# lukors/kanter_core

Measured on AMD Instinct MI355X. Metric: node-Mpix/s on 4096x4096 f32x4, 32-node graph, higher is better.
Workload: dtype f32

## Files before the change

### bindings/rust/kanter_core_amd_sys.rs

```rust
#![allow(non_camel_case_types, dead_code)]
use std::os::raw::{c_char, c_void};

#[repr(C)] pub struct KcPlane { _private: [u8; 0] }
#[repr(C)] pub struct KcImage { _private: [u8; 0] }
#[repr(C)] pub struct KcNodeGraph { _private: [u8; 0] }
#[repr(C)] pub struct KcLiveGraph { _private: [u8; 0] }
#[repr(C)] pub struct KcTexPro { _private: [u8; 0] }
#[repr(C)] pub struct KcPartition { _private: [u8; 0] }
#[repr(C)] pub struct KcU8Pipe { _private: [u8; 0] }

#[repr(C)] #[derive(Clone, Copy, Debug, PartialEq, Eq)]
pub struct KcPlacement { pub node_id: u32, pub rank: i32, pub component: i32, pub kind: i32 }

#[repr(C)] #[derive(Clone, Copy, Debug, PartialEq, Eq)]
pub struct KcBandRows { pub node_id: u32, pub y0: i32, pub y1: i32, pub width: u32, pub height: u32 }

#[repr(C)] #[derive(Clone, Copy, Debug, PartialEq, Eq)]
pub struct KcBandRange { pub y0: i32, pub y1: i32 }

#[repr(C)] #[derive(Clone, Copy, Debug, PartialEq, Eq)]
pub struct KcTransfer { pub node_id: u32, pub slot_id: u32, pub src_rank: i32, pub dst_rank: i32, pub level: i32 }

#[repr(C)] #[derive(Clone, Copy, Debug)]
pub struct KcDeviceImage {
// ... 13 lines not shown
pub struct KcChannelStats {
    pub channels: u32,
    pub flags: u32,
    pub pixels: u64,
    pub min: [f32; 4],
    pub max: [f32; 4],
    pub nan_count: [u64; 4],
    pub histogram: [[u64; 256]; 4],
}
pub const KC_STATS_HISTOGRAM: u32 = 1;
pub const KC_STATS_SRGB: u32 = 2;

#[repr(C)] #[derive(Clone, Copy, Debug)]
pub struct KcBcImage {
    pub ptr: *mut c_void,
    pub width: u32,
    pub height: u32,
    pub format: i32,
    pub row_pitch_bytes: usize,
}
pub const KC_BC1: i32 = 1;
pub const KC_BC3: i32 = 3;
pub const KC_BC4: i32 = 4;
pub const KC_BC5: i32 = 5;
pub const KC_BC_SRGB: u32 = 1;

#[repr(C)] #[derive(Clone, Copy, Debug, PartialEq, Eq)]
pub struct KcSize { pub width: u32, pub height: u32 }

#[repr(C)] #[derive(Clone, Copy, Debug, PartialEq, Eq)]
pub struct KcEdge { pub output_id: u32, pub input_id: u32, pub output_slot: u32, pub input_slot: u32 }

#[repr(C)]
pub struct KcNodeDesc {
    pub node_id: u32,
    pub node_type: i32,
    pub mix_type: i32,
    pub value: f32,
    pub embed_id: u32,
    pub text: *const c_char,
    pub graph: *const KcNodeGraph,
    pub resize_policy: i32,
    pub policy_slot: u32,
    pub policy_size: KcSize,
    pub resize_filter: i32,
}

pub const KC_OK: i32 = 0;
pub const KC_ERR_CANCELED: i32 = 2;
pub const KC_ERR_NO_DEVICE: i32 = 101;

#[link(name = "kanter_core_amd")]
extern "C" {
    pub fn kc_init(device_ordinal: i32) -> i32;
    pub fn kc_shutdown() -> i32;
    pub fn kc_is_initialized() -> i32;
    pub fn kc_set_stream(hip_stream: *mut c_void) -> i32;
    pub fn kc_get_stream() -> *mut c_void;
    pub fn kc_sync() -> i32;
    pub fn kc_last_error() -> *const c_char;
    pub fn kc_status_string(status: i32) -> *const c_char;
    pub fn kc_set_fusion(enabled: i32) -> i32;
    pub fn kc_get_fusion() -> i32;
    pub fn kc_set_resize_mode(mode: i32) -> i32;
    pub fn kc_get_resize_mode() -> i32;
    pub fn kc_set_cache_policy(mode: i32) -> i32;
    pub fn kc_get_cache_policy() -> i32;
    pub fn kc_set_option(name: *const c_char, value: i32) -> i32;
    pub fn kc_get_option(name: *const c_char, value: *mut i32) -> i32;
    pub fn kc_resize_upsample_plan(in_n: u32, out_n: u32, filter: i32, eligible: *mut i32, info: *mut i32, rows: *mut f32, cap: usize) -> i32;
    pub fn kc_resize_down2_plan(in_n: u32, out_n: u32, filter: i32, info: *mut i32, left_count: *mut u32, w: *mut f32, wcap: usize, vrec: *mut u32, vcap: usize, hw: *mut f32, hcap: usize) -> i32;
    pub fn kc_stats(bytes_in_use: *mut u64, bytes_cached: *mut u64, kernel_launches: *mut u64) -> i32;
    pub fn kc_stats_algorithmic_bytes(bytes: *mut u64) -> i32;
    pub fn kc_stats_counter(name: *const c_char, value: *mut u64) -> i32;
    pub fn kc_pool_trim() -> i32;
    pub fn kc_set_specialize(mode: i32, after: i32) -> i32;
    pub fn kc_get_specialize() -> i32;
    pub fn kc_specialize_wait() -> i32;
    pub fn kc_specialize_stats(kernels_compiled: *mut u64, compiles_failed: *mut u64, specialized_launches: *mut u64, compiles_pending: *mut u64) -> i32;
    pub fn kc_specialize_compile_check(words: *const u32, n_ops: u32, n_in: u32, start_src: i32, flat: i32, source: *mut c_char, cap: usize) -> i32;
    pub fn kc_specialize_compile_check_mask(words: *const u32, n_ops: u32, n_in: u32, start_src: i32, flat: i32, nt_mask: u32, source: *mut c_char, cap: usize) -> i32;
    pub fn kc_set_chain_quads(quads: i32) -> i32;
    pub fn kc_get_chain_quads() -> i32;
    pub fn kc_specialize_compile_check_upsample(words: *const u32, n_ops: u32, n_in: u32, start_src: i32, taps: u32, wide: i32, source: *mut c_char, cap: usize) -> i32;
    pub fn kc_kernel_cache_set_dir(dir: *const c_char) -> i32;
    pub fn kc_kernel_cache_stats(files_accepted: *mut u64, files_refused: *mut u64, files_written: *mut u64, kernels_loaded: *mut u64) -> i32;
    pub fn kc_kernel_cache_precompile(words: *const u32, n_ops: u32, n_in: u32, start_src: i32, flat: i32, nt_mask: u32, up_taps: u32, up_wide: i32, dir: *const c_char) -> i32;
    pub fn kc_specialize_reset() -> i32;
    pub fn kc_plane_alloc(width: u32, height: u32, out: *mut *mut KcPlane) -> i32;
    pub fn kc_plane_const(width: u32, height: u32, value: f32, out: *mut *mut KcPlane) -> i32;
    pub fn kc_plane_wrap(device_ptr: *mut c_void, width: u32, height: u32, pitch_bytes: usize, out: *mut *mut KcPlane) -> i32;
    pub fn kc_plane_retain(p: *mut KcPlane) -> i32;
    pub fn kc_plane_release(p: *mut KcPlane) -> i32;
    pub fn kc_plane_size(p: *const KcPlane, width: *mut u32, height: *mut u32) -> i32;
    pub fn kc_plane_is_const(p: *const KcPlane, is_const: *mut i32, value: *mut f32) -> i32;
    pub fn kc_plane_materialize(p: *mut KcPlane) -> i32;
    pub fn kc_plane_device_ptr(p: *mut KcPlane, device_ptr: *mut *mut c_void, pitch_bytes: *mut usize) -> i32;
    pub fn kc_plane_upload_f32(p: *mut KcPlane, host: *const f32, host_pitch_bytes: usize) -> i32;
    pub fn kc_plane_download_f32(p: *mut KcPlane, host: *mut f32, host_pitch_bytes: usize) -> i32;
    pub fn kc_image_gray(p: *mut KcPlane, out: *mut *mut KcImage) -> i32;
    pub fn kc_image_rgba(planes: *const *mut KcPlane, out: *mut *mut KcImage) -> i32;
    pub fn kc_image_retain(img: *mut KcImage) -> i32;
    pub fn kc_image_release(img: *mut KcImage) -> i32;
    pub fn kc_image_is_rgba(img: *const KcImage, is_rgba: *mut i32) -> i32;
    pub fn kc_image_size(img: *const KcImage, size: *mut KcSize) -> i32;
    pub fn kc_image_plane(img: *const KcImage, channel: i32, out: *mut *mut KcPlane) -> i32;
    pub fn kc_image_from_value(size: KcSize, value: f32, rgba: i32, out: *mut *mut KcImage) -> i32;
    pub fn kc_image_as_type(img: *const KcImage, rgba: i32, out: *mut *mut KcImage) -> i32;
    pub fn kc_image_materialize(img: *mut KcImage) -> i32;
    pub fn kc_image_from_u8(host: *const u8, width: u32, height: u32, channels: i32, out: *mut *mut KcImage) -> i32;
    pub fn kc_image_to_u8(img: *mut KcImage, srgb: i32, host_rgba8: *mut u8) -> i32;
    pub fn kc_u8_pipe_create(width: u32, height: u32, channels: i32, depth: i32, out: *mut *mut KcU8Pipe) -> i32;
    pub fn kc_u8_pipe_free(pipe: *mut KcU8Pipe) -> i32;
    pub fn kc_u8_pipe_buffers(pipe: *mut KcU8Pipe, slot: i32, host_in: *mut *mut u8, host_out: *mut *const u8) -> i32;
    pub fn kc_u8_pipe_upload(pipe: *mut KcU8Pipe, slot: i32, out: *mut *mut KcImage) -> i32;
    pub fn kc_u8_pipe_download(pipe: *mut KcU8Pipe, slot: i32, img: *mut KcImage, srgb: i32) -> i32;
    pub fn kc_u8_pipe_wait_download(pipe: *mut KcU8Pipe, slot: i32) -> i32;
    pub fn kc_image_from_f32(host_planes: *const *const f32, n_planes: i32, width: u32, height: u32, out: *mut *mut KcImage) -> i32;
    pub fn kc_image_to_f32(img: *mut KcImage, host_planes: *const *mut f32, n_planes: i32) -> i32;
    pub fn kc_device_image_validate(d: *const KcDeviceImage, extent_bytes: *mut usize) -> i32;
    pub fn kc_image_from_device(src: *const KcDeviceImage, flags: u32, hip_stream: *mut c_void, out: *mut *mut KcImage) -> i32;
    pub fn kc_image_to_device(img: *mut KcImage, dst: *const KcDeviceImage, flags: u32, hip_stream: *mut c_void) -> i32;
    pub fn kc_image_channel_stats(img: *mut KcImage, flags: u32, out: *mut KcChannelStats) -> i32;
    pub fn kc_bc_image_validate(d: *const KcBcImage, extent_bytes: *mut usize) -> i32;
    pub fn kc_image_to_bc(img: *mut KcImage, format: i32, flags: u32, host: *mut u8, host_bytes: usize) -> i32;
    pub fn kc_image_to_bc_device(img: *mut KcImage, dst: *const KcBcImage, flags: u32, hip_stream: *mut c_void) -> i32;
    pub fn kc_mip_level_count(width: u32, height: u32, levels: *mut u32) -> i32;
    pub fn kc_image_build_mips(img: *mut KcImage, flags: u32, levels: *mut *mut KcImage, cap: u32, count: *mut u32) -> i32;
    pub fn kc_bc_mip_layout(width: u32, height: u32, format: i32, levels: *mut u32, offsets: *mut usize, cap: u32, total_bytes: *mut usize) -> i32;
    pub fn kc_image_to_bc_mips(img: *mut KcImage, format: i32, flags: u32, host: *mut u8, host_bytes: usize) -> i32;
    pub fn kc_image_to_bc_mips_device(img: *mut KcImage, format: i32, flags: u32, device_ptr: *mut c_void, bytes: usize, hip_stream: *mut c_void) -> i32;
    pub fn kc_dds_header(width: u32, height: u32, format: i32, flags: u32, levels: u32, out: *mut u8, bytes: *mut usize) -> i32;
    pub fn kc_image_write_dds(img: *mut KcImage, path: *const c_char, format: i32, flags: u32, with_mips: i32) -> i32;
    pub fn kc_image_read_png(path: *const c_char, out: *mut *mut KcImage) -> i32;
    pub fn kc_image_write_png(img: *mut KcImage, path: *const c_char) -> i32;
    pub fn kc_calculate_size(policy: i32, sizes: *const KcSize, n: i32, slot_index: i32, specific: KcSize, out: *mut KcSize) -> i32;
    pub fn kc_resize_image(src: *mut KcImage, size: KcSize, filter: i32, out: *mut *mut KcImage) -> i32;
    pub fn kc_resize_buffers(images: *const *mut KcImage, keys: *const KcEdge, n: i32, edges_sorted: *const KcEdge, n_edges: i32, policy: i32, policy_slot: u32, policy_size: KcSize, filter: i32, out: *mut *mut KcImage) -> i32;
    pub fn kc_mix_process(left: *mut KcImage, right: *mut KcImage, mix_type: i32, out: *mut *mut KcImage) -> i32;
    pub fn kc_separate_rgba_process(input: *mut KcImage, out: *mut *mut KcImage) -> i32;
    pub fn kc_combine_rgba_process(inputs: *const *mut KcImage, out: *mut *mut KcImage) -> i32;
    pub fn kc_value_process(value: f32, out: *mut *mut KcImage) -> i32;
    pub fn kc_height_to_normal_process(input: *mut KcImage, out: *mut *mut KcImage) -> i32;
    pub fn kc_node_graph_new(out: *mut *mut KcNodeGraph) -> i32;
    pub fn kc_node_graph_clone(g: *const KcNodeGraph, out: *mut *mut KcNodeGraph) -> i32;
    pub fn kc_node_graph_free(g: *mut KcNodeGraph) -> i32;
    pub fn kc_node_graph_from_path(path: *const c_char, out: *mut *mut KcNodeGraph) -> i32;
    pub fn kc_node_graph_from_json(json: *const c_char, out: *mut *mut KcNodeGraph) -> i32;
    pub fn kc_node_graph_export_json(g: *const KcNodeGraph, path: *const c_char) -> i32;
    pub fn kc_node_graph_to_json(g: *const KcNodeGraph, buf: *mut c_char, cap: usize, needed: *mut usize) -> i32;
    pub fn kc_node_graph_add_node(g: *mut KcNodeGraph, node: *const KcNodeDesc, node_id: *mut u32) -> i32;
    pub fn kc_node_graph_add_node_with_id(g: *mut KcNodeGraph, node: *const KcNodeDesc) -> i32;
    pub fn kc_node_graph_connect(g: *mut KcNodeGraph, output_node: u32, input_node: u32, output_slot: u32, input_slot: u32) -> i32;
    pub fn kc_node_graph_try_connect(g: *mut KcNodeGraph, output_node: u32, input_node: u32, output_slot: u32, input_slot: u32) -> i32;
    pub fn kc_node_graph_remove_node(g: *mut KcNodeGraph, node_id: u32) -> i32;
    pub fn kc_node_graph_remove_edge(g: *mut KcNodeGraph, edge: KcEdge) -> i32;
    pub fn kc_node_graph_disconnect_slot(g: *mut KcNodeGraph, node_id: u32, side: i32, slot_id: u32) -> i32;
    pub fn kc_node_graph_node_count(g: *const KcNodeGraph, count: *mut u32) -> i32;
    pub fn kc_node_graph_node_ids(g: *const KcNodeGraph, ids: *mut u32, cap: u32, count: *mut u32) -> i32;
    pub fn kc_node_graph_edges(g: *const KcNodeGraph, edges: *mut KcEdge, cap: u32, count: *mut u32) -> i32;
    pub fn kc_node_graph_input_slot_id_with_name(g: *const KcNodeGraph, name: *const c_char, slot_id: *mut u32) -> i32;
    pub fn kc_node_graph_output_slot_id_with_name(g: *const KcNodeGraph, name: *const c_char, slot_id: *mut u32) -> i32;
    pub fn kc_node_graph_set_mix_type(g: *mut KcNodeGraph, node_id: u32, mix_type: i32) -> i32;
    pub fn kc_node_graph_set_image_node_path(g: *mut KcNodeGraph, node_id: u32, path: *const c_char) -> i32;
    pub fn kc_node_graph_rename_output_node(g: *mut KcNodeGraph, node_id: u32, new_name: *const c_char, old_name: *mut c_char, cap: usize) -> i32;
    pub fn kc_tex_pro_new(memory_threshold: u64, out: *mut *mut KcTexPro) -> i32;
    pub fn kc_tex_pro_free(tp: *mut KcTexPro) -> i32;
    pub fn kc_tex_pro_new_live_graph(tp: *mut KcTexPro, out: *mut *mut KcLiveGraph) -> i32;
    pub fn kc_live_graph_free(lg: *mut KcLiveGraph) -> i32;
    pub fn kc_live_graph_set_flags(lg: *mut KcLiveGraph, auto_update: i32, use_cache: i32) -> i32;
// ... 56 lines not shown
```

### include/kanter_core_amd.h

```cpp
#ifndef KANTER_CORE_AMD_H
#define KANTER_CORE_AMD_H

#include <stddef.h>
#include <stdint.h>

#ifdef __cplusplus
extern "C" {
#endif

#define KC_API __attribute__((visibility("default")))

typedef enum kc_status {
    KC_OK = 0,
    KC_ERR_GENERIC = 1,
    KC_ERR_CANCELED = 2,
    KC_ERR_IMAGE = 3,
    KC_ERR_INVALID_BUFFER_COUNT = 4,
    KC_ERR_INVALID_NODE_ID = 5,
    KC_ERR_INVALID_NODE_TYPE = 6,
    KC_ERR_INVALID_SLOT_ID = 7,
    KC_ERR_INVALID_SLOT_TYPE = 8,
    KC_ERR_INVALID_EDGE = 9,
    KC_ERR_NO_SLOT_DATA = 10,
    KC_ERR_SLOT_OCCUPIED = 11,
// ... 3 lines not shown
    KC_ERR_POISON = 15,
    KC_ERR_TRY_LOCK = 16,
    KC_ERR_NODE_DIRTY = 17,
    KC_ERR_IO = 18,
    KC_ERR_INVALID_NAME = 19,
    KC_ERR_HIP = 100,
    KC_ERR_NO_DEVICE = 101,
    KC_ERR_INVALID_ARG = 102,
    KC_ERR_OUT_OF_MEMORY = 103,
    KC_ERR_UNSUPPORTED = 104
} kc_status;

typedef enum kc_mix_type { KC_MIX_ADD = 0, KC_MIX_SUBTRACT = 1, KC_MIX_MULTIPLY = 2, KC_MIX_DIVIDE = 3, KC_MIX_POW = 4 } kc_mix_type;
typedef enum kc_resize_filter { KC_FILTER_NEAREST = 0, KC_FILTER_TRIANGLE = 1, KC_FILTER_CATMULLROM = 2, KC_FILTER_GAUSSIAN = 3, KC_FILTER_LANCZOS3 = 4 } kc_resize_filter;
typedef enum kc_resize_policy { KC_POLICY_MOST_PIXELS = 0, KC_POLICY_LEAST_PIXELS = 1, KC_POLICY_LARGEST_AXES = 2, KC_POLICY_SMALLEST_AXES = 3, KC_POLICY_SPECIFIC_SLOT = 4, KC_POLICY_SPECIFIC_SIZE = 5 } kc_resize_policy;
typedef enum kc_node_type {
    KC_NODE_INPUT_GRAY = 0, KC_NODE_INPUT_RGBA = 1, KC_NODE_OUTPUT_GRAY = 2, KC_NODE_OUTPUT_RGBA = 3,
    KC_NODE_GRAPH = 4, KC_NODE_IMAGE = 5, KC_NODE_EMBED = 6, KC_NODE_WRITE = 7, KC_NODE_VALUE = 8,
    KC_NODE_MIX = 9, KC_NODE_HEIGHT_TO_NORMAL = 10, KC_NODE_SEPARATE_RGBA = 11, KC_NODE_COMBINE_RGBA = 12
} kc_node_type;
typedef enum kc_node_state { KC_STATE_CLEAN = 0, KC_STATE_DIRTY = 1, KC_STATE_REQUESTED = 2, KC_STATE_PRIORITISED = 3, KC_STATE_PROCESSING = 4, KC_STATE_PROCESSING_DIRTY = 5 } kc_node_state;
typedef enum kc_side { KC_SIDE_INPUT = 0, KC_SIDE_OUTPUT = 1 } kc_side;

typedef struct kc_plane kc_plane;
typedef struct kc_image kc_image;
typedef struct kc_node_graph kc_node_graph;
typedef struct kc_live_graph kc_live_graph;
typedef struct kc_tex_pro kc_tex_pro;
typedef struct kc_partition kc_partition;
typedef struct kc_u8_pipe kc_u8_pipe;

typedef struct kc_size { uint32_t width, height; } kc_size;
typedef struct kc_edge { uint32_t output_id, input_id, output_slot, input_slot; } kc_edge;

typedef struct kc_node_desc {
    uint32_t node_id;
    int32_t node_type;
    int32_t mix_type;
    float value;
    uint32_t embed_id;
    const char *text;
    const kc_node_graph *graph;
    int32_t resize_policy;
    uint32_t policy_slot;
    kc_size policy_size;
    int32_t resize_filter;
} kc_node_desc;

KC_API int kc_init(int device_ordinal);
KC_API int kc_shutdown(void);
KC_API int kc_is_initialized(void);
KC_API int kc_set_stream(void *hip_stream);
KC_API void *kc_get_stream(void);
KC_API int kc_sync(void);
KC_API const char *kc_last_error(void);
KC_API const char *kc_status_string(int status);
KC_API int kc_set_fusion(int enabled);
KC_API int kc_get_fusion(void);
KC_API int kc_set_resize_mode(int mode);
KC_API int kc_get_resize_mode(void);
KC_API int kc_set_cache_policy(int mode);
KC_API int kc_get_cache_policy(void);
KC_API int kc_set_option(const char *name, int value);
KC_API int kc_get_option(const char *name, int *value);
KC_API int kc_resize_upsample_plan(uint32_t in_n, uint32_t out_n, int filter, int *eligible, int32_t info[5], float *rows,
                                   size_t cap);
KC_API int kc_resize_down2_plan(uint32_t in_n, uint32_t out_n, int filter, int32_t info[5], uint32_t *left_count, float *w, size_t wcap,
                                uint32_t *vrec, size_t vcap, float *hw, size_t hcap);
KC_API int kc_stats(uint64_t *bytes_in_use, uint64_t *bytes_cached, uint64_t *kernel_launches);
KC_API int kc_stats_algorithmic_bytes(uint64_t *bytes);
KC_API int kc_stats_counter(const char *name, uint64_t *value);
KC_API int kc_pool_trim(void);
KC_API int kc_set_specialize(int mode, int after);
KC_API int kc_get_specialize(void);
KC_API int kc_specialize_wait(void);
KC_API int kc_specialize_stats(uint64_t *kernels_compiled, uint64_t *compiles_failed, uint64_t *specialized_launches,
                               uint64_t *compiles_pending);
KC_API int kc_specialize_compile_check(const uint32_t *words, uint32_t n_ops, uint32_t n_in, int start_src, int flat,
                                       char *source, size_t cap);
KC_API int kc_specialize_compile_check_mask(const uint32_t *words, uint32_t n_ops, uint32_t n_in, int start_src, int flat,
                                            uint32_t nt_mask, char *source, size_t cap);
KC_API int kc_set_chain_quads(int quads);
KC_API int kc_get_chain_quads(void);
KC_API int kc_specialize_compile_check_upsample(const uint32_t *words, uint32_t n_ops, uint32_t n_in, int start_src, uint32_t taps,
                                                int wide, char *source, size_t cap);
KC_API int kc_kernel_cache_set_dir(const char *dir);
KC_API int kc_kernel_cache_stats(uint64_t *files_accepted, uint64_t *files_refused, uint64_t *files_written, uint64_t *kernels_loaded);
KC_API int kc_kernel_cache_precompile(const uint32_t *words, uint32_t n_ops, uint32_t n_in, int start_src, int flat, uint32_t nt_mask,
                                      uint32_t up_taps, int up_wide, const char *dir);
KC_API int kc_specialize_reset(void);

KC_API int kc_plane_alloc(uint32_t width, uint32_t height, kc_plane **out);
KC_API int kc_plane_const(uint32_t width, uint32_t height, float value, kc_plane **out);
KC_API int kc_plane_wrap(void *device_ptr, uint32_t width, uint32_t height, size_t pitch_bytes, kc_plane **out);
KC_API int kc_plane_retain(kc_plane *p);
KC_API int kc_plane_release(kc_plane *p);
KC_API int kc_plane_size(const kc_plane *p, uint32_t *width, uint32_t *height);
KC_API int kc_plane_is_const(const kc_plane *p, int *is_const, float *value);
KC_API int kc_plane_materialize(kc_plane *p);
KC_API int kc_plane_device_ptr(kc_plane *p, void **device_ptr, size_t *pitch_bytes);
KC_API int kc_plane_upload_f32(kc_plane *p, const float *host, size_t host_pitch_bytes);
KC_API int kc_plane_download_f32(kc_plane *p, float *host, size_t host_pitch_bytes);

KC_API int kc_image_gray(kc_plane *p, kc_image **out);
KC_API int kc_image_rgba(kc_plane *const planes[4], kc_image **out);
KC_API int kc_image_retain(kc_image *img);
KC_API int kc_image_release(kc_image *img);
KC_API int kc_image_is_rgba(const kc_image *img, int *is_rgba);
KC_API int kc_image_size(const kc_image *img, kc_size *size);
KC_API int kc_image_plane(const kc_image *img, int channel, kc_plane **out);
KC_API int kc_image_from_value(kc_size size, float value, int rgba, kc_image **out);
KC_API int kc_image_as_type(const kc_image *img, int rgba, kc_image **out);
KC_API int kc_image_materialize(kc_image *img);
KC_API int kc_image_from_u8(const uint8_t *host, uint32_t width, uint32_t height, int channels, kc_image **out);
KC_API int kc_image_to_u8(kc_image *img, int srgb, uint8_t *host_rgba8);
KC_API int kc_u8_pipe_create(uint32_t width, uint32_t height, int channels, int depth, kc_u8_pipe **out);
KC_API int kc_u8_pipe_free(kc_u8_pipe *pipe);
KC_API int kc_u8_pipe_buffers(kc_u8_pipe *pipe, int slot, uint8_t **host_in, const uint8_t **host_out);
KC_API int kc_u8_pipe_upload(kc_u8_pipe *pipe, int slot, kc_image **out);
KC_API int kc_u8_pipe_download(kc_u8_pipe *pipe, int slot, kc_image *img, int srgb);
KC_API int kc_u8_pipe_wait_download(kc_u8_pipe *pipe, int slot);
KC_API int kc_image_from_f32(const float *const host_planes[], int n_planes, uint32_t width, uint32_t height, kc_image **out);
KC_API int kc_image_to_f32(kc_image *img, float *const host_planes[], int n_planes);
typedef enum kc_dtype { KC_DTYPE_U8 = 0, KC_DTYPE_U16 = 1, KC_DTYPE_F16 = 2, KC_DTYPE_BF16 = 3, KC_DTYPE_F32 = 4 } kc_dtype;
typedef enum kc_layout { KC_LAYOUT_INTERLEAVED = 0 , KC_LAYOUT_PLANAR = 1  } kc_layout;
typedef struct kc_device_image {
    void *ptr;
    uint32_t width, height;
    int32_t channels;
    int32_t dtype, layout;
    size_t row_pitch_bytes;
    size_t channel_pitch_bytes;
} kc_device_image;
#define KC_DEVICE_SRGB 1u
#define KC_DEVICE_GRAY 2u
KC_API int kc_device_image_validate(const kc_device_image *d, size_t *extent_bytes);
KC_API int kc_image_from_device(const kc_device_image *src, uint32_t flags, void *hip_stream, kc_image **out);
KC_API int kc_image_to_device(kc_image *img, const kc_device_image *dst, uint32_t flags, void *hip_stream);
#define KC_STATS_HISTOGRAM 1u
#define KC_STATS_SRGB 2u
typedef struct kc_channel_stats {
    uint32_t channels;
    uint32_t flags;
    uint64_t pixels;
    float min[4], max[4];
    uint64_t nan_count[4];
    uint64_t histogram[4][256];
} kc_channel_stats;
KC_API int kc_image_channel_stats(kc_image *img, uint32_t flags, kc_channel_stats *out);
typedef enum kc_bc_format { KC_BC1 = 1, KC_BC3 = 3, KC_BC4 = 4, KC_BC5 = 5 } kc_bc_format;
typedef struct kc_bc_image {
    void *ptr;
    uint32_t width, height;
    int32_t format;
    size_t row_pitch_bytes;
} kc_bc_image;
#define KC_BC_SRGB 1u
KC_API int kc_bc_image_validate(const kc_bc_image *d, size_t *extent_bytes);
KC_API int kc_image_to_bc(kc_image *img, int format, uint32_t flags, uint8_t *host, size_t host_bytes);
KC_API int kc_image_to_bc_device(kc_image *img, const kc_bc_image *dst, uint32_t flags, void *hip_stream);
#define KC_MIP_PER_LEVEL 2u
KC_API int kc_mip_level_count(uint32_t width, uint32_t height, uint32_t *levels);
KC_API int kc_image_build_mips(kc_image *img, uint32_t flags, kc_image **levels, uint32_t cap, uint32_t *count);
KC_API int kc_bc_mip_layout(uint32_t width, uint32_t height, int format, uint32_t *levels, size_t *offsets, uint32_t cap,
                            size_t *total_bytes);
KC_API int kc_image_to_bc_mips(kc_image *img, int format, uint32_t flags, uint8_t *host, size_t host_bytes);
KC_API int kc_image_to_bc_mips_device(kc_image *img, int format, uint32_t flags, void *device_ptr, size_t bytes, void *hip_stream);
KC_API int kc_dds_header(uint32_t width, uint32_t height, int format, uint32_t flags, uint32_t levels, uint8_t out[148], size_t *bytes);
KC_API int kc_image_write_dds(kc_image *img, const char *path, int format, uint32_t flags, int with_mips);
KC_API int kc_image_read_png(const char *path, kc_image **out);
KC_API int kc_image_write_png(kc_image *img, const char *path);

// ... 126 lines not shown
```

### kanter_core_amd/__init__.py

```python
from .api import (Edge, EmbeddedSlotDataId, LiveGraph, MixType, Node, NodeGraph, NodeId, NodeState, NodeType,
                  ResizeFilter, ResizePolicy, Side, Size, SlotData, SlotId, SlotImage, TexProError,
                  TextureProcessor, calculate_size, combine_rgba_process, get_stream, height_to_normal_process,
                  init, is_initialized, mix_process, resize_image, separate_rgba_process, set_fusion, set_stream,
                  shutdown, stats, sync, value_process, set_specialize, get_specialize, specialize_wait,
                  specialize_stats, specialize_compile_check, Partition, PartitionPolicy, NodeKind, set_resize_mode,
                  get_resize_mode, resize_upsample_plan, resize_down2_plan, stats_counter, specialize_compile_check_upsample, specialize_compile_check_mask, set_chain_quads, get_chain_quads, set_cache_policy, get_cache_policy, set_option, get_option, comm_unique_id, comm_init,
                  comm_destroy, comm_info, comm_stats, comm_transport, comm_gather_bands, PlanKind, pool_trim, kernel_cache_set_dir, kernel_cache_stats,
                  kernel_cache_precompile, specialize_reset, U8Pipe, device_image_desc, DEVICE_SRGB, DEVICE_GRAY,
                  ChannelStats, STATS_HISTOGRAM, STATS_SRGB, BC_SRGB, BC_BLOCK_BYTES,
                  MIP_PER_LEVEL, mip_level_count, bc_mip_layout, dds_header)

__all__ = [n for n in dir() if not n.startswith("_")]
```

### kanter_core_amd/_lib.py

```python
import ctypes as C
import os

_HERE = os.path.dirname(os.path.abspath(__file__))
LIB_PATH = os.path.join(_HERE, "libkanter_core_amd.so")

c_u8p = C.POINTER(C.c_uint8)
c_u32p = C.POINTER(C.c_uint32)
c_fp = C.POINTER(C.c_float)
c_vp = C.c_void_p


class kc_size(C.Structure):
    _fields_ = [("width", C.c_uint32), ("height", C.c_uint32)]


class kc_edge(C.Structure):
    _fields_ = [("output_id", C.c_uint32), ("input_id", C.c_uint32), ("output_slot", C.c_uint32),
                ("input_slot", C.c_uint32)]


class kc_node_desc(C.Structure):
    _fields_ = [("node_id", C.c_uint32), ("node_type", C.c_int32), ("mix_type", C.c_int32), ("value", C.c_float),
                ("embed_id", C.c_uint32), ("text", C.c_char_p), ("graph", c_vp), ("resize_policy", C.c_int32),
                ("policy_slot", C.c_uint32), ("policy_size", kc_size), ("resize_filter", C.c_int32)]


class kc_placement(C.Structure):
    _fields_ = [("node_id", C.c_uint32), ("rank", C.c_int32), ("component", C.c_int32), ("kind", C.c_int32)]


class kc_transfer(C.Structure):
    _fields_ = [("node_id", C.c_uint32), ("slot_id", C.c_uint32), ("src_rank", C.c_int32), ("dst_rank", C.c_int32),
                ("level", C.c_int32)]


class kc_band_range(C.Structure):
    _fields_ = [("y0", C.c_int32), ("y1", C.c_int32)]


class kc_band_rows(C.Structure):
    _fields_ = [("node_id", C.c_uint32), ("y0", C.c_int32), ("y1", C.c_int32), ("width", C.c_uint32), ("height", C.c_uint32)]


class kc_device_image(C.Structure):
    _fields_ = [("ptr", c_vp), ("width", C.c_uint32), ("height", C.c_uint32), ("channels", C.c_int32), ("dtype", C.c_int32),
                ("layout", C.c_int32), ("row_pitch_bytes", C.c_size_t), ("channel_pitch_bytes", C.c_size_t)]


class kc_channel_stats(C.Structure):
    _fields_ = [("channels", C.c_uint32), ("flags", C.c_uint32), ("pixels", C.c_uint64), ("min", C.c_float * 4), ("max", C.c_float * 4),
                ("nan_count", C.c_uint64 * 4), ("histogram", (C.c_uint64 * 256) * 4)]


class kc_bc_image(C.Structure):
    _fields_ = [("ptr", c_vp), ("width", C.c_uint32), ("height", C.c_uint32), ("format", C.c_int32), ("row_pitch_bytes", C.c_size_t)]


SIGNATURES = {
    "kc_init": (C.c_int, [C.c_int]),
    "kc_shutdown": (C.c_int, []),
    "kc_is_initialized": (C.c_int, []),
    "kc_set_stream": (C.c_int, [c_vp]),
    "kc_get_stream": (c_vp, []),
    "kc_sync": (C.c_int, []),
    "kc_last_error": (C.c_char_p, []),
    "kc_status_string": (C.c_char_p, [C.c_int]),
    "kc_set_fusion": (C.c_int, [C.c_int]),
    "kc_set_resize_mode": (C.c_int, [C.c_int]),
    "kc_get_resize_mode": (C.c_int, []),
    "kc_set_cache_policy": (C.c_int, [C.c_int]),
    "kc_comm_unique_id": (C.c_int, [C.c_void_p]),
    "kc_comm_init": (C.c_int, [C.c_int, C.c_int, C.c_void_p]),
    "kc_comm_destroy": (C.c_int, []),
    "kc_comm_info": (C.c_int, [C.POINTER(C.c_int), C.POINTER(C.c_int)]),
    "kc_comm_stats": (C.c_int, [C.POINTER(C.c_uint64), C.POINTER(C.c_uint64), C.POINTER(C.c_uint64)]),
    "kc_live_graph_exchange": (C.c_int, [C.c_void_p, C.c_void_p, C.c_uint32]),
    "kc_comm_transport": (C.c_int, [C.c_char_p, C.c_size_t]),
    "kc_u8_pipe_create": (C.c_int, [C.c_uint32, C.c_uint32, C.c_int, C.c_int, C.POINTER(C.c_void_p)]),
    "kc_u8_pipe_free": (C.c_int, [C.c_void_p]),
    "kc_u8_pipe_buffers": (C.c_int, [C.c_void_p, C.c_int, C.POINTER(C.c_void_p), C.POINTER(C.c_void_p)]),
    "kc_u8_pipe_upload": (C.c_int, [C.c_void_p, C.c_int, C.POINTER(C.c_void_p)]),
    "kc_u8_pipe_download": (C.c_int, [C.c_void_p, C.c_int, C.c_void_p, C.c_int]),
    "kc_u8_pipe_wait_download": (C.c_int, [C.c_void_p, C.c_int]),
    "kc_kernel_cache_set_dir": (C.c_int, [C.c_char_p]),
    "kc_kernel_cache_stats": (C.c_int, [C.POINTER(C.c_uint64)] * 4),
    "kc_kernel_cache_precompile": (C.c_int, [C.POINTER(C.c_uint32), C.c_uint32, C.c_uint32, C.c_int, C.c_int, C.c_uint32, C.c_uint32, C.c_int, C.c_char_p]),
    "kc_specialize_reset": (C.c_int, []),
    "kc_comm_gather_bands": (C.c_int, [C.c_void_p, C.c_int32, C.c_uint32, C.c_int, C.POINTER(C.c_void_p)]),
    "kc_live_graph_evaluate_partitioned": (C.c_int, [C.c_void_p, C.c_void_p, C.c_uint32, C.POINTER(C.c_void_p)]),
    "kc_set_option": (C.c_int, [C.c_char_p, C.c_int]),
    "kc_get_option": (C.c_int, [C.c_char_p, C.POINTER(C.c_int)]),
    "kc_get_cache_policy": (C.c_int, []),
    "kc_stats_counter": (C.c_int, [C.c_char_p, C.POINTER(C.c_uint64)]),
    "kc_resize_down2_plan": (C.c_int, [C.c_uint32, C.c_uint32, C.c_int, C.POINTER(C.c_int32), C.POINTER(C.c_uint32), C.POINTER(C.c_float),
                                       C.c_size_t, C.POINTER(C.c_uint32), C.c_size_t, C.POINTER(C.c_float), C.c_size_t]),
    "kc_resize_upsample_plan": (C.c_int, [C.c_uint32, C.c_uint32, C.c_int, C.POINTER(C.c_int), C.POINTER(C.c_int32),
                                          C.POINTER(C.c_float), C.c_size_t]),
    "kc_get_fusion": (C.c_int, []),
    "kc_stats": (C.c_int, [C.POINTER(C.c_uint64)] * 3),
    "kc_set_specialize": (C.c_int, [C.c_int, C.c_int]),
    "kc_get_specialize": (C.c_int, []),
    "kc_specialize_wait": (C.c_int, []),
    "kc_specialize_stats": (C.c_int, [C.POINTER(C.c_uint64)] * 4),
    "kc_specialize_compile_check": (C.c_int, [c_u32p, C.c_uint32, C.c_uint32, C.c_int, C.c_int, C.c_char_p, C.c_size_t]),
    "kc_specialize_compile_check_mask": (C.c_int, [c_u32p, C.c_uint32, C.c_uint32, C.c_int, C.c_int, C.c_uint32, C.c_char_p, C.c_size_t]),
    "kc_set_chain_quads": (C.c_int, [C.c_int]),
    "kc_get_chain_quads": (C.c_int, []),
    "kc_specialize_compile_check_upsample": (C.c_int, [c_u32p, C.c_uint32, C.c_uint32, C.c_int, C.c_uint32, C.c_int, C.c_char_p,
                                                       C.c_size_t]),
    "kc_stats_algorithmic_bytes": (C.c_int, [C.POINTER(C.c_uint64)]),
    "kc_pool_trim": (C.c_int, []),
    "kc_live_graph_partition": (C.c_int, [c_vp, C.c_uint32, C.c_int, C.c_int, C.POINTER(c_vp)]),
    "kc_partition_free": (C.c_int, [c_vp]),
    "kc_partition_info": (C.c_int, [c_vp, C.POINTER(C.c_int), C.POINTER(C.c_int), C.POINTER(C.c_int)]),
    "kc_partition_nodes": (C.c_int, [c_vp, C.POINTER(kc_placement), C.c_uint32, c_u32p]),
    "kc_partition_transfers": (C.c_int, [c_vp, C.POINTER(kc_transfer), C.c_uint32, c_u32p]),
    "kc_partition_kind": (C.c_int, [c_vp, C.POINTER(C.c_int), C.POINTER(C.c_double), C.POINTER(C.c_double), C.POINTER(C.c_double)]),
    "kc_partition_bands": (C.c_int, [c_vp, C.POINTER(kc_band_range), C.c_uint32, c_u32p, c_u32p, c_u32p]),
    "kc_partition_set_gather": (C.c_int, [c_vp, C.c_int]),
    "kc_live_graph_import_slot_data": (C.c_int, [c_vp, C.c_uint32, C.c_uint32, c_vp]),
    "kc_live_graph_evaluate_band": (C.c_int, [c_vp, C.c_uint32, C.c_uint32, C.c_int32, C.c_int32, C.POINTER(c_vp)]),
    "kc_live_graph_band_source_rows": (C.c_int, [c_vp, C.c_uint32, C.c_int32, C.c_int32, C.POINTER(kc_band_rows), C.c_uint32, c_u32p]),
    "kc_live_graph_embed_slot_data_band": (C.c_int, [c_vp, c_vp, C.c_uint32, C.c_uint32, C.c_int32, C.c_uint32]),
    "kc_plane_alloc": (C.c_int, [C.c_uint32, C.c_uint32, C.POINTER(c_vp)]),
    "kc_plane_const": (C.c_int, [C.c_uint32, C.c_uint32, C.c_float, C.POINTER(c_vp)]),
    "kc_plane_wrap": (C.c_int, [c_vp, C.c_uint32, C.c_uint32, C.c_size_t, C.POINTER(c_vp)]),
    "kc_plane_retain": (C.c_int, [c_vp]),
    "kc_plane_release": (C.c_int, [c_vp]),
    "kc_plane_size": (C.c_int, [c_vp, c_u32p, c_u32p]),
    "kc_plane_is_const": (C.c_int, [c_vp, C.POINTER(C.c_int), c_fp]),
    "kc_plane_materialize": (C.c_int, [c_vp]),
    "kc_plane_device_ptr": (C.c_int, [c_vp, C.POINTER(c_vp), C.POINTER(C.c_size_t)]),
    "kc_plane_upload_f32": (C.c_int, [c_vp, c_vp, C.c_size_t]),
    "kc_plane_download_f32": (C.c_int, [c_vp, c_vp, C.c_size_t]),
    "kc_image_gray": (C.c_int, [c_vp, C.POINTER(c_vp)]),
    "kc_image_rgba": (C.c_int, [C.POINTER(c_vp), C.POINTER(c_vp)]),
    "kc_image_retain": (C.c_int, [c_vp]),
    "kc_image_release": (C.c_int, [c_vp]),
    "kc_image_is_rgba": (C.c_int, [c_vp, C.POINTER(C.c_int)]),
    "kc_image_size": (C.c_int, [c_vp, C.POINTER(kc_size)]),
    "kc_image_plane": (C.c_int, [c_vp, C.c_int, C.POINTER(c_vp)]),
    "kc_image_from_value": (C.c_int, [kc_size, C.c_float, C.c_int, C.POINTER(c_vp)]),
    "kc_image_as_type": (C.c_int, [c_vp, C.c_int, C.POINTER(c_vp)]),
    "kc_image_materialize": (C.c_int, [c_vp]),
    "kc_image_from_u8": (C.c_int, [c_vp, C.c_uint32, C.c_uint32, C.c_int, C.POINTER(c_vp)]),
    "kc_image_to_u8": (C.c_int, [c_vp, C.c_int, c_vp]),
    "kc_device_image_validate": (C.c_int, [C.POINTER(kc_device_image), C.POINTER(C.c_size_t)]),
    "kc_image_from_device": (C.c_int, [C.POINTER(kc_device_image), C.c_uint32, c_vp, C.POINTER(c_vp)]),
    "kc_image_to_device": (C.c_int, [c_vp, C.POINTER(kc_device_image), C.c_uint32, c_vp]),
    "kc_image_channel_stats": (C.c_int, [c_vp, C.c_uint32, C.POINTER(kc_channel_stats)]),
    "kc_bc_image_validate": (C.c_int, [C.POINTER(kc_bc_image), C.POINTER(C.c_size_t)]),
    "kc_image_to_bc": (C.c_int, [c_vp, C.c_int, C.c_uint32, c_vp, C.c_size_t]),
    "kc_image_to_bc_device": (C.c_int, [c_vp, C.POINTER(kc_bc_image), C.c_uint32, c_vp]),
    "kc_mip_level_count": (C.c_int, [C.c_uint32, C.c_uint32, C.POINTER(C.c_uint32)]),
    "kc_image_build_mips": (C.c_int, [c_vp, C.c_uint32, C.POINTER(c_vp), C.c_uint32, C.POINTER(C.c_uint32)]),
    "kc_bc_mip_layout": (C.c_int, [C.c_uint32, C.c_uint32, C.c_int, C.POINTER(C.c_uint32), C.POINTER(C.c_size_t), C.c_uint32,
                                   C.POINTER(C.c_size_t)]),
    "kc_image_to_bc_mips": (C.c_int, [c_vp, C.c_int, C.c_uint32, c_vp, C.c_size_t]),
    "kc_image_to_bc_mips_device": (C.c_int, [c_vp, C.c_int, C.c_uint32, c_vp, C.c_size_t, c_vp]),
    "kc_dds_header": (C.c_int, [C.c_uint32, C.c_uint32, C.c_int, C.c_uint32, C.c_uint32, c_vp, C.POINTER(C.c_size_t)]),
    "kc_image_write_dds": (C.c_int, [c_vp, C.c_char_p, C.c_int, C.c_uint32, C.c_int]),
    "kc_image_from_f32": (C.c_int, [C.POINTER(c_vp), C.c_int, C.c_uint32, C.c_uint32, C.POINTER(c_vp)]),
    "kc_image_to_f32": (C.c_int, [c_vp, C.POINTER(c_vp), C.c_int]),
    "kc_image_read_png": (C.c_int, [C.c_char_p, C.POINTER(c_vp)]),
    "kc_image_write_png": (C.c_int, [c_vp, C.c_char_p]),
    "kc_calculate_size": (C.c_int, [C.c_int, C.POINTER(kc_size), C.c_int, C.c_int, kc_size, C.POINTER(kc_size)]),
    "kc_resize_image": (C.c_int, [c_vp, kc_size, C.c_int, C.POINTER(c_vp)]),
    "kc_resize_buffers": (C.c_int, [C.POINTER(c_vp), C.POINTER(kc_edge), C.c_int, C.POINTER(kc_edge), C.c_int, C.c_int,
                                    C.c_uint32, kc_size, C.c_int, C.POINTER(c_vp)]),
    "kc_mix_process": (C.c_int, [c_vp, c_vp, C.c_int, C.POINTER(c_vp)]),
    "kc_separate_rgba_process": (C.c_int, [c_vp, C.POINTER(c_vp)]),
    "kc_combine_rgba_process": (C.c_int, [C.POINTER(c_vp), C.POINTER(c_vp)]),
    "kc_value_process": (C.c_int, [C.c_float, C.POINTER(c_vp)]),
    "kc_height_to_normal_process": (C.c_int, [c_vp, C.POINTER(c_vp)]),
    "kc_node_graph_new": (C.c_int, [C.POINTER(c_vp)]),
    "kc_node_graph_clone": (C.c_int, [c_vp, C.POINTER(c_vp)]),
    "kc_node_graph_free": (C.c_int, [c_vp]),
    "kc_node_graph_from_path": (C.c_int, [C.c_char_p, C.POINTER(c_vp)]),
    "kc_node_graph_from_json": (C.c_int, [C.c_char_p, C.POINTER(c_vp)]),
    "kc_node_graph_export_json": (C.c_int, [c_vp, C.c_char_p]),
    "kc_node_graph_to_json": (C.c_int, [c_vp, C.c_char_p, C.c_size_t, C.POINTER(C.c_size_t)]),
    "kc_node_graph_add_node": (C.c_int, [c_vp, C.POINTER(kc_node_desc), c_u32p]),
    "kc_node_graph_add_node_with_id": (C.c_int, [c_vp, C.POINTER(kc_node_desc)]),
    "kc_node_graph_connect": (C.c_int, [c_vp] + [C.c_uint32] * 4),
    "kc_node_graph_try_connect": (C.c_int, [c_vp] + [C.c_uint32] * 4),
    "kc_node_graph_remove_node": (C.c_int, [c_vp, C.c_uint32]),
    "kc_node_graph_remove_edge": (C.c_int, [c_vp, kc_edge]),
    "kc_node_graph_disconnect_slot": (C.c_int, [c_vp, C.c_uint32, C.c_int, C.c_uint32]),
    "kc_node_graph_node_count": (C.c_int, [c_vp, c_u32p]),
    "kc_node_graph_node_ids": (C.c_int, [c_vp, c_u32p, C.c_uint32, c_u32p]),
# ... 87 lines not shown
```

### kanter_core_amd/api.py

```python
import collections
import ctypes as C
import os

import numpy as np

from . import _lib
from ._lib import kc_edge, kc_node_desc, kc_size

_ERROR_NAMES = {
    1: "Generic", 2: "Canceled", 3: "Image", 4: "InvalidBufferCount", 5: "InvalidNodeId", 6: "InvalidNodeType",
    7: "InvalidSlotId", 8: "InvalidSlotType", 9: "InvalidEdge", 10: "NoSlotData", 11: "SlotOccupied",
    12: "SlotNotOccupied", 13: "UnableToLock", 14: "NodeProcessing", 15: "PoisonError", 16: "TryLockError",
    17: "NodeDirty", 18: "Io", 19: "InvalidName", 100: "Hip", 101: "NoDevice", 102: "InvalidArgument",
    103: "OutOfMemory", 104: "Unsupported",
}


class TexProError(Exception):

    def __init__(self, code, detail=""):
        self.code = code
        self.kind = _ERROR_NAMES.get(code, "Unknown")
        L = _lib.load()
        msg = L.kc_status_string(code).decode()
# ... 107 lines not shown


def get_option(name):
    v = C.c_int()
    _check(_lib.load().kc_get_option(name.encode(), C.byref(v)))
    return v.value


def resize_upsample_plan(in_n, out_n, filter=None):
    import numpy as np
    L = _lib.load()
    f = ResizeFilter.default() if filter is None else filter
    ok = C.c_int(0)
    info = (C.c_int32 * 5)()
    _check(L.kc_resize_upsample_plan(int(in_n), int(out_n), int(f), C.byref(ok), info, None, 0))
    if not ok.value:
        return None
    ratio, taps, off, b_lo, b_hi = (int(v) for v in info)
    rows = np.zeros(((ratio + b_lo + b_hi), taps), np.float32)
    _check(L.kc_resize_upsample_plan(int(in_n), int(out_n), int(f), C.byref(ok), info,
                                     rows.ctypes.data_as(C.POINTER(C.c_float)), rows.size))
    return dict(ratio=ratio, taps=taps, off=off, b_lo=b_lo, b_hi=b_hi, rows=rows)


def resize_down2_plan(in_n, out_n, filter=None):
    import numpy as np
    L = _lib.load()
    f = ResizeFilter.default() if filter is None else filter
    info = (C.c_int32 * 5)()
    _check(L.kc_resize_down2_plan(int(in_n), int(out_n), int(f), info, None, None, 0, None, 0, None, 0))
    stride, nc, hstride, tile_w, min_count = (int(v) for v in info)
    groups = (out_n + 3) // 4
    lc = np.zeros(2 * out_n, np.uint32)
    w = np.zeros((out_n, stride), np.float32)
    vrec = np.zeros((groups, max(nc, 1), 72), np.uint32)
    hw = np.zeros((out_n, max(hstride, 1)), np.float32)
    _check(L.kc_resize_down2_plan(int(in_n), int(out_n), int(f), info, lc.ctypes.data_as(C.POINTER(C.c_uint32)),
                                  w.ctypes.data_as(C.POINTER(C.c_float)), w.size,
                                  vrec.ctypes.data_as(C.POINTER(C.c_uint32)), vrec.size if nc else 0,
                                  hw.ctypes.data_as(C.POINTER(C.c_float)), hw.size if hstride else 0))
    return dict(stride=stride, nc=nc, hstride=hstride, tile_w=tile_w, min_count=min_count, left=lc[:out_n].copy(),
                count=lc[out_n:].copy(), w=w, vrec=vrec if nc else None, hw=hw if hstride else None)


def set_specialize(mode, after=0):
    _check(_lib.load().kc_set_specialize(int(mode), int(after)))


def get_specialize():
    return _lib.load().kc_get_specialize()


def specialize_wait():
    _check(_lib.load().kc_specialize_wait())


def specialize_stats():
    v = [C.c_uint64() for _ in range(4)]
    _check(_lib.load().kc_specialize_stats(*[C.byref(x) for x in v]))
    return dict(zip(("kernels_compiled", "compiles_failed", "specialized_launches", "compiles_pending"), [x.value for x in v]))


def specialize_compile_check(words, n_in, start_src=0, flat=True):
    arr = (C.c_uint32 * len(words))(*words)
    buf = C.create_string_buffer(1 << 16)
    _check(_lib.load().kc_specialize_compile_check(arr, len(words), int(n_in), int(start_src), int(bool(flat)), buf, len(buf)))
    return buf.value.decode()


def specialize_compile_check_mask(words, n_in, nt_mask, start_src=0, flat=True):
    arr = (C.c_uint32 * len(words))(*words)
    buf = C.create_string_buffer(1 << 17)
    _check(_lib.load().kc_specialize_compile_check_mask(arr, len(words), int(n_in), int(start_src), int(bool(flat)), int(nt_mask),
                                                        buf, len(buf)))
    return buf.value.decode()


def set_chain_quads(quads):
    _check(_lib.load().kc_set_chain_quads(int(quads)))


def get_chain_quads():
    return _lib.load().kc_get_chain_quads()


def specialize_compile_check_upsample(words, n_in, start_src=0, taps=3, wide=True):
    arr = (C.c_uint32 * len(words))(*words)
    buf = C.create_string_buffer(1 << 17)
    _check(_lib.load().kc_specialize_compile_check_upsample(arr, len(words), int(n_in), int(start_src), int(taps), int(bool(wide)),
                                                            buf, len(buf)))
    return buf.value.decode()


def stats():
    a, b, c = C.c_uint64(), C.c_uint64(), C.c_uint64()
    _check(_lib.load().kc_stats(C.byref(a), C.byref(b), C.byref(c)))
    d = C.c_uint64()
    _check(_lib.load().kc_stats_algorithmic_bytes(C.byref(d)))
    return {"bytes_in_use": a.value, "bytes_cached": b.value, "kernel_launches": c.value, "algorithmic_bytes": d.value}


def kernel_cache_set_dir(path):
    _check(_lib.load().kc_kernel_cache_set_dir(None if path is None else str(path).encode()))


def kernel_cache_stats():
    v = [C.c_uint64() for _ in range(4)]
    _check(_lib.load().kc_kernel_cache_stats(*[C.byref(x) for x in v]))
    return dict(zip(("files_accepted", "files_refused", "files_written", "kernels_loaded"), (x.value for x in v)))


def kernel_cache_precompile(words, n_in, start_src, flat, nt_mask, directory, up_taps=0, up_wide=False):
    arr = (C.c_uint32 * len(words))(*words)
    _check(_lib.load().kc_kernel_cache_precompile(arr, len(words), int(n_in), int(start_src), int(bool(flat)), int(nt_mask),
                                                  int(up_taps), int(bool(up_wide)), str(directory).encode()))


def specialize_reset():
    _check(_lib.load().kc_specialize_reset())


def pool_trim():
    _check(_lib.load().kc_pool_trim())


def stats_counter(name):
    v = C.c_uint64()
    _check(_lib.load().kc_stats_counter(name.encode(), C.byref(v)))
    return v.value


class NodeId(int):
    """NodeId(u32), src/node_graph.rs:592-607"""


class SlotId(int):
    """SlotId(u32), src/node_graph.rs:609-624"""


class EmbeddedSlotDataId(int):
    """src/node/embed.rs:13-14"""


class Size:

    def __init__(self, width, height):
        self.width, self.height = int(width), int(height)

    def pixel_count(self):
        return (self.width * self.height) & 0xFFFFFFFF

    def __eq__(self, o):
        if isinstance(o, tuple):
            return (self.width, self.height) == o
        return isinstance(o, Size) and (self.width, self.height) == (o.width, o.height)

    def __hash__(self):
        return hash((self.width, self.height))

    def __iter__(self):
        return iter((self.width, self.height))

    def __repr__(self):
        return "%dx%d" % (self.width, self.height)

    def _c(self):
# ... 1040 lines not shown
```

### kanter_core_amd/build.py

```python
import os
import subprocess
import sys
from concurrent.futures import ThreadPoolExecutor

HERE = os.path.dirname(os.path.abspath(__file__))
CSRC = os.path.join(HERE, "csrc")
OBJ = os.path.join(HERE, "csrc", "build")
LIB = os.path.join(HERE, "libkanter_core_amd.so")
SOURCES = ["chain.hip", "upsample.hip", "resize_tile.hip", "resize_down.hip", "h2n.hip", "u8.hip", "chain1.hip", "down2.hip", "runtime.cpp",
           "ops.cpp", "resize.cpp", "graph.cpp", "json.cpp", "png.cpp", "specialize.cpp", "partition.cpp", "bands.cpp", "comm.cpp", "replay.cpp",
           "u8pipe.cpp", "devimage.hip", "devimage.cpp", "stats.hip", "stats.cpp", "bc.hip", "bc.cpp", "mip.hip", "mip.cpp",
           "c_api.cpp"]
HEADERS = ["kc_internal.hpp", "kc_runtime.hpp", "chain_program.h", os.path.join("..", "..", "include", "kanter_core_amd.h"), "pow_positive.inc",
           "srgb_thresholds.inc", "streaming.h", "upsample.h", "upsample_chain.inc", "chain_apply.inc", "chain_interp.inc", "resample.inc"]
JIT_TEXTS = [("kJitChainProgramH", "chain_program.h"), ("kJitPowPositiveInc", "pow_positive.inc"), ("kJitUpsampleH", "upsample.h"),
             ("kJitUpsampleChainInc", "upsample_chain.inc")]

FLAGS = ["--offload-arch=gfx950", "-O3", "-std=c++17", "-fPIC", "-fvisibility=hidden", "-fno-fast-math",
         "-ffp-contract=off", "-fhip-fp32-correctly-rounded-divide-sqrt", "-Wall", "-Wno-unused-result"]
DEVICE_FLAGS = ["-mllvm", "-structurizecfg-skip-uniform-regions=1"]
if os.environ.get("KC_HOST_PROFILE"):
    FLAGS = FLAGS + ["-DKC_HOST_PROFILE"]
if os.environ.get("KC_HOST_SAMPLE"):
    FLAGS = FLAGS + ["-DKC_HOST_SAMPLE", "-fno-omit-frame-pointer"]


def _hipcc():
    for cand in (os.environ.get("HIPCC"), "/opt/rocm/bin/hipcc", "hipcc"):
        if cand and (os.path.isabs(cand) and os.path.exists(cand) or not os.path.isabs(cand)):
            return cand
    return "hipcc"


def _stale(target, deps):
    if not os.path.exists(target):
        return True
    t = os.path.getmtime(target)
    return any(os.path.getmtime(d) > t for d in deps)


def object_name(src):
    stem = os.path.splitext(src)[0]
    if src.endswith(".hip") and stem + ".cpp" in SOURCES:
        stem += "_kernels"
    return stem + ".o"


def _write_jit_texts():
    out = os.path.join(OBJ, "jit_texts.cpp")
    parts = ["// generated by kanter_core_amd/build.py from csrc/chain_program.h and csrc/pow_positive.inc -- do not edit\n",
             "namespace kc {\n"]
    for name, fn in JIT_TEXTS:
        with open(os.path.join(CSRC, fn)) as f:
            text = f.read()
        assert ')KCJIT"' not in text
        parts.append('extern const char %s[];\nconst char %s[] = R"KCJIT(\n%s)KCJIT";\n' % (name, name, text))
    parts.append("}  // namespace kc\n")
    new = "".join(parts)
    old = open(out).read() if os.path.exists(out) else None
    if new != old:
        with open(out, "w") as f:
            f.write(new)
    return out


def build(force=False, verbose=False):
    os.makedirs(OBJ, exist_ok=True)
    hipcc = _hipcc()
    hdrs = [os.path.join(CSRC, h) for h in HEADERS]
    jobs = []
    objs = []
    jit = _write_jit_texts()
    jit_o = os.path.join(OBJ, "jit_texts.o")
    objs.append(jit_o)
    if force or _stale(jit_o, [jit]):
        jobs.append([hipcc] + FLAGS + ["-c", jit, "-o", jit_o])
    for src in SOURCES:
        s = os.path.join(CSRC, src)
        o = os.path.join(OBJ, object_name(src))
        objs.append(o)
        if force or _stale(o, [s] + hdrs):
            cmd = [hipcc] + FLAGS + (DEVICE_FLAGS + ["-x", "hip"] if src.endswith(".hip") else []) + ["-c", s, "-o", o]
            jobs.append(cmd)

    def run(cmd):
        if verbose:
            print(" ".join(cmd), flush=True)
        r = subprocess.run(cmd, stdout=subprocess.PIPE, stderr=subprocess.STDOUT, text=True)
        if r.returncode != 0:
            raise RuntimeError("hipcc failed:\n%s\n%s" % (" ".join(cmd), r.stdout))
        return r.stdout

    with ThreadPoolExecutor(max_workers=4) as ex:
        for out in ex.map(run, jobs):
            if verbose and out.strip():
                print(out)
    if force or jobs or _stale(LIB, objs):
        run([hipcc, "--offload-arch=gfx950", "-shared", "-fPIC", "-o", LIB] + objs + ["-lz", "-ldl"])
    populate_kernel_cache(verbose=verbose)
    return LIB


MANIFEST = os.path.join(HERE, "baseline_programs.jsonl")
KERNEL_CACHE = os.path.join(HERE, "kernel_cache")


def populate_kernel_cache(force=False, verbose=False):
    import ctypes as C
    import hashlib
    import json
    if not os.path.exists(MANIFEST) or not os.path.exists(LIB):
        return 0
    with open(MANIFEST) as f:
        text = f.read()
    entries = [json.loads(line) for line in text.splitlines() if line.strip()]
    st = os.stat(LIB)
    stamp = hashlib.sha256(("%s|%d|%d" % (text, st.st_mtime_ns, st.st_size)).encode()).hexdigest()
    stamp_file = os.path.join(KERNEL_CACHE, ".stamp")
    if not force and os.path.exists(stamp_file) and open(stamp_file).read() == stamp:
        return len(entries)
    os.makedirs(KERNEL_CACHE, exist_ok=True)
    for old in os.listdir(KERNEL_CACHE):
        if old.endswith(".kcco"):
            os.remove(os.path.join(KERNEL_CACHE, old))
    L = C.CDLL(LIB)
    L.kc_kernel_cache_precompile.argtypes = [C.POINTER(C.c_uint32), C.c_uint32, C.c_uint32, C.c_int, C.c_int, C.c_uint32, C.c_uint32,
                                             C.c_int, C.c_char_p]
    L.kc_kernel_cache_precompile.restype = C.c_int
    L.kc_last_error.restype = C.c_char_p

    def one(e):
        words = (C.c_uint32 * len(e["words"]))(*e["words"])
        rc = L.kc_kernel_cache_precompile(words, len(e["words"]), e["n_in"], e["start_src"], e["flat"], e["nt_mask"], e["up_taps"],
                                          e["up_wide"], KERNEL_CACHE.encode())
        if rc != 0:
            raise RuntimeError("pre-compiling %s failed (%d): %s" % (e.get("name"), rc, (L.kc_last_error() or b"").decode(errors="replace")))
        if verbose:
            print("pre-compiled", e.get("name"), flush=True)

    with ThreadPoolExecutor(max_workers=4) as ex:
        list(ex.map(one, entries))
    with open(stamp_file, "w") as f:
        f.write(stamp)
    return len(entries)


if __name__ == "__main__":
    print(build(force="--force" in sys.argv, verbose=True))
```

### kanter_core_amd/csrc/c_api.cpp

```cpp
#include <algorithm>
#include <cctype>
#include <climits>
#include <cstdio>
#include <cstdlib>
#include <cstring>
#include <fstream>
#include <sstream>

#include "kc_runtime.hpp"

namespace kc {
const std::string &last_error();
}
using namespace kc;

#define KC_ARG(cond)                                         \
    do {                                                     \
        if (!(cond)) {                                       \
            set_error("invalid argument: " #cond);           \
            return KC_ERR_INVALID_ARG;                       \
        }                                                    \
    } while (0)

typedef std::lock_guard<std::recursive_mutex> Lock;
// ... 310 lines not shown

int kc_specialize_stats(uint64_t *compiled, uint64_t *failed, uint64_t *launches, uint64_t *pending)
try {
    specialize_stats(compiled, failed, launches, pending);
    return KC_OK;
}
KC_CATCH

int kc_specialize_compile_check(const uint32_t *words, uint32_t n_ops, uint32_t n_in, int start_src, int flat, char *source,
                                size_t cap)
try {
    KC_ARG(words && n_ops >= 1 && n_ops <= (uint32_t)KC_CHAIN_MAX_OPS && n_in <= (uint32_t)KC_CHAIN_MAX_IN);
    KC_ARG(start_src >= -1 && start_src < (int)n_in);
    ChainProgram P;
    std::memset(&P, 0, sizeof P);
    P.n_ops = n_ops;
    P.n_in = n_in;
    P.start_src = start_src;
    P.rows = flat ? 1u : 2u;
    P.row_units = 1;
    for (uint32_t i = 0; i < n_ops; ++i) {
        const uint32_t from = (words[i] >> 8) & 0xffu, level = words[i] >> 16;
        KC_ARG((words[i] & 0xffu) <= CH_SAVE_LOAD && (from <= n_in || (from == (uint32_t)KC_CHAIN_SRC_SAVED && (words[i] & 0xffu) != CH_SAVE_LOAD)));
        KC_ARG(level < (uint32_t)KC_CHAIN_MAX_SAVED && (level == 0 || from == (uint32_t)KC_CHAIN_SRC_SAVED || (words[i] & 0xffu) == CH_SAVE_LOAD));
        ((i & 1u) ? P.step[0][i / 2].b : P.step[0][i / 2].a).word = words[i];
    }
    if (source && cap) {
        const std::string src = specialize_source(P);
        std::snprintf(source, cap, "%s", src.c_str());
    }
    std::string log;
    int s = specialize_compile_only(P, &log);
    if (s != KC_OK) set_error("specialised chain kernel did not compile: " + log);
    return s;
}
KC_CATCH

int kc_specialize_compile_check_mask(const uint32_t *words, uint32_t n_ops, uint32_t n_in, int start_src, int flat, uint32_t nt_mask,
                                     char *source, size_t cap)
try {
    KC_ARG(words && n_ops >= 1 && n_ops <= (uint32_t)KC_CHAIN_MAX_OPS && n_in <= (uint32_t)KC_CHAIN_MAX_IN);
    KC_ARG(start_src >= -1 && start_src < (int)n_in);
    ChainProgram P;
    std::memset(&P, 0, sizeof P);
    P.n_ops = n_ops;
    P.n_in = n_in;
    P.start_src = start_src;
    P.rows = flat ? 1u : 2u;
    P.row_units = 1;
    P.nt_mask = nt_mask;
    for (uint32_t i = 0; i < n_ops; ++i) {
        const uint32_t from = (words[i] >> 8) & 0xffu, level = words[i] >> 16;
        KC_ARG((words[i] & 0xffu) <= CH_SAVE_LOAD && (from <= n_in || (from == (uint32_t)KC_CHAIN_SRC_SAVED && (words[i] & 0xffu) != CH_SAVE_LOAD)));
        KC_ARG(level < (uint32_t)KC_CHAIN_MAX_SAVED && (level == 0 || from == (uint32_t)KC_CHAIN_SRC_SAVED || (words[i] & 0xffu) == CH_SAVE_LOAD));
        ((i & 1u) ? P.step[0][i / 2].b : P.step[0][i / 2].a).word = words[i];
    }
    if (source && cap) {
        const std::string src = specialize_source(P);
        std::snprintf(source, cap, "%s", src.c_str());
    }
    std::string log;
    int s = specialize_compile_only(P, &log);
    if (s != KC_OK) set_error("specialised chain kernel did not compile: " + log);
    return s;
}
KC_CATCH

int kc_set_chain_quads(int quads)
try {
    const int s = specialize_set_chain_quads(quads);
    if (s != KC_OK) set_error("kc_set_chain_quads accepts 0, 1, 2 or 4");
    return s;
}
KC_CATCH

int kc_get_chain_quads(void)
try {
    return specialize_get_chain_quads();
}
catch (...) {
    return 0;
}

int kc_kernel_cache_set_dir(const char *dir)
try {
    Lock lk(ctx().mu);
    return kernel_cache_set_dir(dir);
}
KC_CATCH

int kc_kernel_cache_stats(uint64_t *hits, uint64_t *rejected, uint64_t *written, uint64_t *kernels_loaded)
try {
    kernel_cache_stats(hits, rejected, written, kernels_loaded);
    return KC_OK;
}
KC_CATCH

int kc_kernel_cache_precompile(const uint32_t *words, uint32_t n_ops, uint32_t n_in, int start_src, int flat, uint32_t nt_mask,
                               uint32_t up_taps, int up_wide, const char *dir)
try {
    KC_ARG(words && dir);
    std::string log;
    const int s = kernel_cache_precompile(words, n_ops, n_in, start_src, flat != 0, nt_mask, up_taps, up_wide != 0, dir, &log);
    if (s != KC_OK) set_error("kernel cache: " + log);
    return s;
}
KC_CATCH

int kc_specialize_reset(void)
try {
    Lock lk(ctx().mu);
    if (ctx().stream) (void)hipStreamSynchronize(ctx().stream);
    const int mode = specialize_get_mode();
    specialize_shutdown();
    (void)mode;
    return KC_OK;
}
KC_CATCH

int kc_specialize_compile_check_upsample(const uint32_t *words, uint32_t n_ops, uint32_t n_in, int start_src, uint32_t taps, int wide,
                                         char *source, size_t cap)
try {
    KC_ARG(words && n_ops >= 1 && n_ops <= (uint32_t)KC_CHAIN_MAX_OPS && n_in >= 1 && n_in <= (uint32_t)KC_CHAIN_INTERP_IN);
    KC_ARG(start_src >= -1 && start_src < (int)n_in && (taps == 1 || taps == 3));
    ChainProgram P;
    std::memset(&P, 0, sizeof P);
    P.n_ops = n_ops;
    P.n_in = n_in;
    P.start_src = start_src;
    for (uint32_t i = 0; i < n_ops; ++i) {
        const uint32_t from = words[i] >> 8, code = words[i] & 0xffu;
        KC_ARG(code <= CH_MUL_INV && from <= n_in && code != CH_DIV_L && code != CH_DIV_R && code != CH_POW_L && code != CH_POW_R);
        ((i & 1u) ? P.step[0][i / 2].b : P.step[0][i / 2].a).word = words[i];
    }
    UpsampleArgs U{};
    U.H.taps = U.V.taps = taps;
    U.tile_w = wide ? 1024u : 256u;
    if (source && cap) {
        const std::string src = specialize_source(P, &U);
        std::snprintf(source, cap, "%s", src.c_str());
    }
    std::string log;
    int s = specialize_compile_only(P, &log, &U);
    if (s != KC_OK) set_error("specialised up-sampling kernel did not compile: " + log);
    return s;
}
KC_CATCH

int kc_stats(uint64_t *in_use, uint64_t *cached, uint64_t *launches)
try {
    Context &c = ctx();
    Lock lk(c.mu);
    if (in_use) *in_use = c.bytes_in_use;
    if (cached) *cached = c.bytes_cached;
    if (launches) *launches = c.launches;
    return KC_OK;
}
KC_CATCH

int kc_stats_counter(const char *name, uint64_t *value)
try {
    KC_ARG(name && value);
    Context &c = ctx();
    Lock lk(c.mu);
    auto it = c.counters.find(name);
    *value = it == c.counters.end() ? 0 : it->second;
// ... 1307 lines not shown
```

### kanter_core_amd/csrc/kc_runtime.hpp

```cpp
#pragma once

#include <cstring>
#include <deque>
#include <set>
#include <tuple>
#include <type_traits>
#include <unordered_map>
#include <unordered_set>

#include "kc_internal.hpp"

namespace kc {
struct Chain;
struct ChainLink;
}

namespace kc {
#if defined(__SANITIZE_ADDRESS__) || defined(__SANITIZE_THREAD__)
#define KC_NO_OBJECT_POOL 1
#elif defined(__has_feature)
#if __has_feature(address_sanitizer) || __has_feature(thread_sanitizer)
#define KC_NO_OBJECT_POOL 1
#endif
#endif
template <class T> struct Pooled {
#ifndef KC_NO_OBJECT_POOL
    struct FreeList {
        struct Block { Block *next; };
        static constexpr size_t kMaxFree = 1u << 14;
        Block *head = nullptr;
        size_t n = 0;
        bool closed = false;
        ~FreeList()
        {
            closed = true;
            while (head) {
                Block *b = head;
                head = b->next;
                ::operator delete(b);
            }
            n = 0;
        }
    };
    static FreeList &list()
    {
        static FreeList fl;
        return fl;
    }
    static void *operator new(size_t bytes)
    {
        FreeList &fl = list();
        if (bytes == sizeof(T) && fl.head) {
            typename FreeList::Block *b = fl.head;
            fl.head = b->next;
            --fl.n;
            return b;
        }
        return ::operator new(bytes < sizeof(typename FreeList::Block) ? sizeof(typename FreeList::Block) : bytes);
    }
    static void operator delete(void *q, size_t bytes)
    {
        FreeList &fl = list();
        if (bytes == sizeof(T) && fl.n < FreeList::kMaxFree && !fl.closed) {
            typename FreeList::Block *b = static_cast<typename FreeList::Block *>(q);
            b->next = fl.head;
            fl.head = b;
            ++fl.n;
            return;
        }
        ::operator delete(q);
    }
#endif
};
}

struct kc_plane : kc::Pooled<kc_plane> {
    enum Kind { MEM = 0, CONST = 1, LAZY = 2, RESIZE = 3 };
    int refs = 1;
    uint32_t w = 0, h = 0;
    Kind kind = MEM;
    float *dptr = nullptr;
    size_t pitch = 0;
    size_t bytes = 0;
    bool owned = false;
    float cval = 0.0f;
    kc::ChainLink *link = nullptr;
    kc::Chain *chain = nullptr;
    kc_plane *view_of = nullptr;
    kc_plane *rz_src = nullptr;
    int rz_filter = 0;
};

struct kc_image : kc::Pooled<kc_image> {
    int refs = 1;
    int n = 0;
    kc_plane *planes[4] = { nullptr, nullptr, nullptr, nullptr };
    bool is_rgba() const { return n == 4; }
    uint32_t w() const { return planes[0]->w; }
    uint32_t h() const { return planes[0]->h; }
};

namespace kc {

struct ChainStep {
    uint8_t code;
    kc_plane *operand;
    uint8_t level = 0;
};
kc_plane *saved_value_marker();

struct Chain : Pooled<Chain> {
    kc_plane *start = nullptr;
    std::vector<ChainStep> steps;
    std::vector<kc_plane *> joined;
    ~Chain();
};

struct ChainLink : Pooled<ChainLink> {
    kc_plane *prev = nullptr;
    kc_plane *start = nullptr;
    ChainStep step{};
    uint32_t length = 1;
    bool fused = false;
    uint8_t saved = 0;
    int n_in = 0;
    struct InKey {
        const void *p = nullptr;
        size_t q = 0;
        bool operator==(const InKey &o) const { return p == o.p && q == o.q; }
    };
    InKey ins[KC_CHAIN_MAX_IN + 1];
    ~ChainLink();
};

struct TapsHost {
    std::vector<uint32_t> left, count;
    std::vector<float> w;
    uint32_t stride = 1;
    uint32_t min_count = 1;
    uint32_t reg_a = 0, reg_b = 0, reg_ages = 0, reg_ratio = 0;
    bool up_ok = false;
    UpAxis up{};
    std::vector<float> up_rows, up_qrows;
    std::vector<uint32_t> d2_vrec, d2_strips;
    std::vector<float> d2_hw;
    bool d2_want = false;
    uint32_t d2_nc = 0, d2_hstride = 0, d2_tile_w = 0;
    uint32_t p2_tile_w = 0;
    const uint32_t *d2_vrec_dev = nullptr, *d2_strips_dev = nullptr;
    const float *d2_hw_dev = nullptr;
};

struct TapsEntry {
    uint64_t last_use = 0;
    TapsHost host;
    void *dev_block = nullptr;
    size_t dev_bytes = 0;
    TapsDev dev{};
};

struct ReplayLaunch {
    ChainProgram prog;
    int batch = 0, mode = 0;
    uint32_t in_refs[KC_CHAIN_MAX_IN] = {};
    uint32_t w = 0, h = 0;
    kc_plane *planes[KC_CHAIN_MAX_BATCH] = { nullptr, nullptr, nullptr, nullptr };
    int in_from[KC_CHAIN_MAX_BATCH][KC_CHAIN_MAX_IN];
    int in_ch[KC_CHAIN_MAX_BATCH][KC_CHAIN_MAX_IN];
};
struct ReplayCapture {
    bool ok = true;
    std::vector<ReplayLaunch> launches;
};
// ... 65 lines not shown
#endif

#define KC_HIP(call)                                           \
    do {                                                       \
        hipError_t _e = (call);                                \
        if (_e != hipSuccess) return kc::hip_fail(_e, #call);  \
    } while (0)
#define KC_TRY(expr)                   \
    do {                               \
        int _s = (expr);               \
        if (_s != KC_OK) return _s;    \
    } while (0)

int pool_alloc(size_t bytes, void **out);
void pool_free(void *p, size_t bytes);
int pool_trim();

int plane_new_mem(uint32_t w, uint32_t h, kc_plane **out);
kc_plane *plane_new_const(uint32_t w, uint32_t h, float v);
inline void plane_retain(kc_plane *p)
{
    if (p) ++p->refs;
}
void plane_release(kc_plane *p);
int plane_force(kc_plane *p);
int planes_force(kc_plane *const *planes, int n);
int plane_materialize(kc_plane *p);
int plane_mix(int mix_type, kc_plane *l, kc_plane *r, kc_plane **out);
int planes_mix_prepare(kc_plane *const *ls, kc_plane *const *rs, int n);
Operand plane_operand(const kc_plane *p);

kc_image *image_new(int n, kc_plane *const *planes);
inline void image_retain(kc_image *img)
{
    if (img) ++img->refs;
}
void image_release(kc_image *img);
int image_force(kc_image *img);

int image_from_value(kc_size size, float v, bool rgba, kc_image **out);
int image_as_type(kc_image *img, bool rgba, kc_image **out);
int image_from_u8(const uint8_t *host, uint32_t w, uint32_t h, int channels, kc_image **out);
int image_to_u8(kc_image *img, bool srgb, uint8_t *host);
int device_image_validate(const kc_device_image *d, size_t *extent_bytes);
int image_from_device(const kc_device_image *src, uint32_t flags, void *hip_stream, kc_image **out);
int image_to_device(kc_image *img, const kc_device_image *dst, uint32_t flags, void *hip_stream);
int device_extent_check(const void *ptr, size_t ext, const char *who);
int stream_edge(hipStream_t from, hipStream_t to);
int bc_image_validate(const kc_bc_image *d, size_t *extent_bytes);
int image_to_bc(kc_image *img, int format, uint32_t flags, uint8_t *host, size_t host_bytes);
int image_to_bc_device(kc_image *img, const kc_bc_image *dst, uint32_t flags, void *hip_stream);
size_t bc_block_bytes(int format);
int bc_encode(kc_image *img, int format, bool srgb, char *dst, size_t row_pitch, hipStream_t s);
int mip_level_count(uint32_t w, uint32_t h, uint32_t *levels);
float mip_const_fold(float c);
int image_build_mips(kc_image *img, uint32_t flags, kc_image **levels, uint32_t cap, uint32_t *count);
int bc_mip_layout(uint32_t w, uint32_t h, int format, uint32_t *levels, size_t *offsets, uint32_t cap, size_t *total_bytes);
int image_to_bc_mips(kc_image *img, int format, uint32_t flags, uint8_t *host, size_t host_bytes);
int image_to_bc_mips_device(kc_image *img, int format, uint32_t flags, void *device_ptr, size_t bytes, void *hip_stream);
int dds_header(uint32_t w, uint32_t h, int format, uint32_t flags, uint32_t levels, uint8_t *out, size_t *bytes);
int image_write_dds(kc_image *img, const char *path, int format, uint32_t flags, int with_mips);
int image_channel_stats(kc_image *img, uint32_t flags, kc_channel_stats *out);
void channel_stats_release();
int calculate_size(int policy, const kc_size *sizes, int n, int slot_index, kc_size specific, kc_size *out);
int mix_process(kc_image *left, kc_image *right, int mix_type, kc_image **out);
int separate_process(kc_image *in, kc_image *out[4]);
int combine_process(kc_image *const in[4], kc_image **out);
int value_process(float v, kc_image **out);
int height_to_normal_process(kc_image *in, kc_image **out);
int height_to_normal_band(kc_image *in_with_halo, uint32_t full_h, kc_image **out);

int build_taps_host(uint32_t in_n, uint32_t out_n, int filter, TapsHost &t);
int resize_image(kc_image *src, kc_size size, int filter, kc_image **out);
int resize_force(kc_plane *p);
int resize_planes_band(kc_plane *const *srcs, int n, int32_t src_y0, uint32_t src_h_full, kc_size dst_full, int32_t a, int32_t b,
                       int filter, kc_plane **outs);
int resize_force_many(kc_plane *const *planes, int n);
int chain_resize_launch(const ChainProgram &P, int batch, int mode, kc_plane *const *sampled, bool *launched);

hipError_t launch_chain_specialized(const ChainProgram &P, int batch, hipStream_t s, bool *launched, uint32_t *nt_mask, uint32_t *quads = nullptr);
uint32_t cache_policy_mask(uint64_t in_bytes, uint64_t out_bytes, uint32_t n_resident, const Options &o = options());
uint32_t chain_cache_policy(const uint32_t *refs, uint32_t n, uint64_t stream_bytes, uint64_t out_bytes);
hipError_t chain_dispatch(ChainProgram &P, int batch, int mode, uint32_t w, uint32_t h, size_t out_pitch_bytes);
hipError_t launch_upsample_chain_specialized(const ChainProgram &P, int batch, const UpsampleArgs &U, hipStream_t s, bool *launched);
int specialize_set_mode(int mode, int after);
int specialize_get_mode();
int specialize_set_chain_quads(int quads);
int specialize_get_chain_quads();
void specialize_wait();
void specialize_stats(uint64_t *compiled, uint64_t *failed, uint64_t *launches, uint64_t *pending);
std::string specialize_last_log();
void specialize_shutdown();
std::string specialize_source(const ChainProgram &P, const UpsampleArgs *U = nullptr);
int specialize_compile_only(const ChainProgram &P, std::string *log, const UpsampleArgs *U = nullptr);
int kernel_cache_set_dir(const char *dir);
void kernel_cache_stats(uint64_t *hits, uint64_t *rejected, uint64_t *written, uint64_t *kernels_loaded);
bool kernel_cache_populated();
int kernel_cache_precompile(const uint32_t *words, uint32_t n_ops, uint32_t n_in, int32_t start_src, bool flat, uint32_t nt_mask,
                            uint32_t up_taps, bool up_wide, const char *dir, std::string *log);

int u8_pipe_create(uint32_t w, uint32_t h, int channels, int depth, kc_u8_pipe **out);
int u8_pipe_free(kc_u8_pipe *p);
int u8_pipe_buffers(kc_u8_pipe *p, int slot, uint8_t **host_in, const uint8_t **host_out);
int u8_pipe_upload(kc_u8_pipe *p, int slot, kc_image **out);
int u8_pipe_download(kc_u8_pipe *p, int slot, kc_image *img, bool srgb);
int u8_pipe_wait_download(kc_u8_pipe *p, int slot);

int png_read(const std::string &path, std::vector<uint8_t> &px, uint32_t &w, uint32_t &h, int &channels);
int png_write_rgba8(const std::string &path, const uint8_t *px, uint32_t w, uint32_t h);

struct NodeGraph;

struct Node {
    uint32_t node_id = 0;
    int type = KC_NODE_VALUE;
    int mix_type = KC_MIX_ADD;
    float value = 0.0f;
    uint32_t embed_id = 0;
    std::string text;
    std::shared_ptr<NodeGraph> graph;
    int policy = KC_POLICY_MOST_PIXELS;
    uint32_t policy_slot = 0;
    kc_size policy_size{ 0, 0 };
    int filter = KC_FILTER_TRIANGLE;

    bool is_input() const { return type == KC_NODE_INPUT_GRAY || type == KC_NODE_INPUT_RGBA; }
    bool is_output() const { return type == KC_NODE_OUTPUT_GRAY || type == KC_NODE_OUTPUT_RGBA; }
    bool is_source() const { return type == KC_NODE_EMBED || type == KC_NODE_IMAGE || is_input(); }
};

enum SlotType { SLOT_GRAY = 0, SLOT_RGBA = 1, SLOT_GRAY_OR_RGBA = 2 };
struct Slot {
    std::string name;
    uint32_t slot_id;
    int slot_type;
};

struct GraphIndex {
    uint64_t version = ~0ull;
    size_t n_nodes = 0, n_edges = 0;
    std::unordered_map<uint32_t, uint32_t> node_pos;
    std::unordered_map<uint32_t, std::vector<kc_edge>> in_edges;
    std::unordered_map<uint32_t, std::vector<kc_edge>> out_edges;
};

struct NodeGraph {
    std::vector<Node> nodes;
    std::vector<kc_edge> edges;
    uint32_t node_id_counter = 0;
    uint64_t version = 0;
    mutable GraphIndex idx;

    void touch() { ++version; }
    const GraphIndex &index() const;
    bool index_is_current() const;
    void appended_node(bool index_was_current);
    void appended_edge(bool index_was_current);
    void erased_edge(const kc_edge &e, bool index_was_current);
    const std::vector<kc_edge> &edges_into(uint32_t id) const;
    const std::vector<kc_edge> &edges_out_of(uint32_t id) const;

    const Node *find(uint32_t id) const;
    Node *find(uint32_t id);
    uint32_t new_id();
    int add_node(Node n, uint32_t *id);
    int add_node_with_id(Node n);
    int connect(uint32_t on, uint32_t in, uint32_t os, uint32_t is);
    int try_connect(uint32_t on, uint32_t in, uint32_t os, uint32_t is);
    int remove_edge(kc_edge e);
    int remove_node(uint32_t id, std::vector<kc_edge> *removed);
    int disconnect_slot(uint32_t id, int side, uint32_t slot, std::vector<kc_edge> *removed);
    std::vector<uint32_t> get_children(uint32_t id) const;
    std::vector<uint32_t> get_children_recursive(uint32_t id) const;
    std::vector<uint32_t> get_parents(uint32_t id) const;
    std::vector<uint32_t> output_ids() const;
    int rename_output_node(uint32_t id, const std::string &new_name, std::string *old_name);
    std::vector<Slot> input_slots_of_graph() const;
    std::vector<Slot> output_slots_of_graph() const;
};

std::vector<Slot> node_input_slots(const Node &n, bool *unimplemented = nullptr);
std::vector<Slot> node_output_slots(const Node &n, bool *unimplemented = nullptr);
Node node_from_desc(const kc_node_desc &d);
int ancestors_topological(const NodeGraph &g, uint32_t root, std::vector<uint32_t> &topo);
int root_output_slot(const NodeGraph &g, uint32_t root, uint32_t *slot);

int graph_from_json(const std::string &text, NodeGraph &g);
std::string graph_to_json(const NodeGraph &g);

// ... 175 lines not shown
```

### kanter_core_amd/csrc/runtime.cpp

```cpp
#include <cmath>
#include <cstdlib>
#include <cstdio>
#include <cstring>

#include <algorithm>

#ifdef KC_HOST_SAMPLE
#include <dlfcn.h>
#include <new>
#include <signal.h>
#include <sys/time.h>
#include <ucontext.h>
#endif

#include "kc_runtime.hpp"

namespace kc {

static const int KC_RETRY_CHAIN = -1000;

static thread_local std::string g_last_error;

Context &ctx()
{
// ... 130 lines not shown
        e = hipMalloc(out, bytes);
    }
    if (e == hipErrorOutOfMemory) {
        (void)hipGetLastError();
        set_error("out of HBM");
        return KC_ERR_OUT_OF_MEMORY;
    }
    if (e != hipSuccess) return hip_fail(e, "hipMalloc");
    c.bytes_in_use += bytes;
    return KC_OK;
}

void pool_free(void *p, size_t bytes)
{
    if (!p) return;
    Context &c = ctx();
    std::lock_guard<std::recursive_mutex> lk(c.mu);
    if (!c.inited) return;
    c.free_blocks.emplace(bytes, p);
    c.bytes_in_use -= bytes;
    c.bytes_cached += bytes;
}

int pool_trim()
{
    Context &c = ctx();
    std::lock_guard<std::recursive_mutex> lk(c.mu);
    if (c.stream) (void)hipStreamSynchronize(c.stream);
    for (auto &kv : c.free_blocks) (void)hipFree(kv.second);
    if (!c.free_blocks.empty()) comm_blocks_freed();
    c.free_blocks.clear();
    c.bytes_cached = 0;
    return KC_OK;
}

static size_t pitch_for(uint32_t w)
{
    size_t row = (size_t)w * sizeof(float);
    return (row + 255) / 256 * 256;
}

int plane_new_mem(uint32_t w, uint32_t h, kc_plane **out)
{
    KC_TRY(need_init());
    if (w == 0 || h == 0) {
        set_error("plane with zero extent");
        return KC_ERR_INVALID_ARG;
    }
    kc_plane *p = new kc_plane();
    p->w = w;
    p->h = h;
    p->kind = kc_plane::MEM;
    p->pitch = pitch_for(w);
    p->bytes = p->pitch * h;
    p->owned = true;
    void *d = nullptr;
    int s = pool_alloc(p->bytes, &d);
    if (s != KC_OK) {
        delete p;
        return s;
    }
    p->dptr = (float *)d;
    *out = p;
    return KC_OK;
}

kc_plane *plane_new_const(uint32_t w, uint32_t h, float v)
{
    kc_plane *p = new kc_plane();
    p->w = w;
    p->h = h;
    p->kind = kc_plane::CONST;
    p->cval = v;
    return p;
}

void plane_release(kc_plane *p)
{
    if (!p) return;
    if (--p->refs == 0) {
        if (p->chain) delete p->chain;
        if (p->link) delete p->link;
        if (p->rz_src) plane_release(p->rz_src);
        if (p->view_of) plane_release(p->view_of);
        if (p->owned && p->dptr) pool_free(p->dptr, p->bytes);
        delete p;
    }
}

Chain::~Chain()
{
    plane_release(start);
    for (auto &s : steps) plane_release(s.operand);
    for (auto *j : joined) plane_release(j);
}

kc_plane *saved_value_marker()
{
    static kc_plane *m = [] {
        kc_plane *p = new kc_plane();
        p->kind = kc_plane::CONST;
        p->refs = 1 << 30;
        return p;
    }();
    return m;
}

ChainLink::~ChainLink()
{
    plane_release(start);
    plane_release(step.operand);
    kc_plane *q = prev;
    prev = nullptr;
    while (q) {
        if (--q->refs != 0) break;
        kc_plane *next = nullptr;
        if (q->link) {
            next = q->link->prev;
            q->link->prev = nullptr;
        }
        q->refs = 1;
        plane_release(q);
        q = next;
    }
}

static int chain_in_limit()
{
    const Context &c = ctx();
    return (c.opt.wide && c.opt.fusion && !c.plain_chains && specialize_get_mode() != 0) ? KC_CHAIN_MAX_IN : KC_CHAIN_INTERP_IN;
}

static void link_add_input(ChainLink &L, const kc_plane *q)
{
    ChainLink::InKey k;
    if (q->kind == kc_plane::MEM)
        k = { q->dptr, q->pitch };
    else if (q->kind == kc_plane::RESIZE)
        k = { q, ~(size_t)0 };
    else
        return;
    for (int i = 0; i < L.n_in && i <= KC_CHAIN_MAX_IN; ++i)
        if (L.ins[i] == k) return;
    if (L.n_in <= KC_CHAIN_MAX_IN) L.ins[L.n_in] = k;
    L.n_in++;
}

static int input_index(std::vector<const kc_plane *> &ins, const kc_plane *p);

static int chain_distinct_inputs(const Chain &ch)
{
    std::vector<const kc_plane *> ins;
    auto counts = [](const kc_plane *q) { return q->kind == kc_plane::MEM || q->kind == kc_plane::RESIZE; };
    if (counts(ch.start)) input_index(ins, ch.start);
    for (auto &s : ch.steps)
        if (counts(s.operand)) input_index(ins, s.operand);
    return (int)ins.size();
}

static size_t chain_record_count(const Chain &ch)
{
    size_t r = 0;
    for (size_t i = 0; i < ch.steps.size(); ++i, ++r) {
        const ChainStep &st = ch.steps[i];
        uint8_t code = st.code == CH_ADD_R ? (uint8_t)CH_ADD : st.code == CH_MUL_R ? (uint8_t)CH_MUL : st.code;
        const bool plane = st.operand == saved_value_marker() || st.operand->kind != kc_plane::CONST;
        if (plane && code <= CH_MUL && i + 1 < ch.steps.size() && ch.steps[i + 1].code == CH_SUB_R &&
            ch.steps[i + 1].operand->kind == kc_plane::CONST && ch.steps[i + 1].operand != saved_value_marker())
            ++i;
    }
    return r;
}

static void chain_flatten(kc_plane *p)
{
    KC_PROF("chain_flatten");
    if (p->chain) return;
    Chain *c = new Chain();
    c->steps.reserve(p->link->length);
    kc_plane *q = p;
    for (;;) {
        ChainLink *L = q->link;
        kc_plane *opnd = L->step.operand;
        if (opnd->kind == kc_plane::LAZY) {
            chain_flatten(opnd);
            const Chain &sub = *opnd->chain;
            uint8_t code = L->step.code;
            switch (code) {
            case CH_SUB_L: code = CH_SUB_R; break;
            case CH_SUB_R: code = CH_SUB_L; break;
            case CH_DIV_L: code = CH_DIV_R; break;
            case CH_DIV_R: code = CH_DIV_L; break;
            case CH_POW_L: code = CH_POW_R; break;
            case CH_POW_R: code = CH_POW_L; break;
            default: break;
            }
            c->steps.push_back({ code, saved_value_marker(), 0 });
            for (size_t i = sub.steps.size(); i-- > 0;) {
                ChainStep st = sub.steps[i];
                if (st.code == CH_SAVE_LOAD || st.operand == saved_value_marker()) st.level++;
                c->steps.push_back(st);
            }
            c->steps.push_back({ (uint8_t)CH_SAVE_LOAD, sub.start, 0 });
            c->joined.push_back(opnd);
            plane_retain(opnd);
        } else {
            c->steps.push_back(L->step);
        }
        if (L->prev && L->prev->kind == kc_plane::LAZY) {
            q = L->prev;
            continue;
        }
        c->start = L->prev ? L->prev : L->start;
        break;
    }
    std::reverse(c->steps.begin(), c->steps.end());
    plane_retain(c->start);
    for (auto &s : c->steps) plane_retain(s.operand);
    p->chain = c;
}

Operand plane_operand(const kc_plane *p)
{
    Operand o;
    if (p->kind == kc_plane::CONST) {
        o.ptr = nullptr;
        o.pitch = 0;
        o.c = p->cval;
    } else {
        o.ptr = p->dptr;
        o.pitch = (uint32_t)(p->pitch / sizeof(float));
        o.c = 0.0f;
    }
    return o;
}

struct BuiltChain {
    ChainProgram prog;
    uint32_t in_refs[KC_CHAIN_MAX_IN] = {};
    int mode = 0;
    kc_plane *sampled[KC_CHAIN_MAX_BATCH] = { nullptr, nullptr, nullptr, nullptr };
    bool joins = false;
};

static int input_index(std::vector<const kc_plane *> &ins, const kc_plane *p)
{
    for (size_t i = 0; i < ins.size(); ++i)
        if (ins[i] == p || (p->kind == kc_plane::MEM && ins[i]->kind == kc_plane::MEM && ins[i]->dptr == p->dptr &&
                            ins[i]->pitch == p->pitch))
            return (int)i;
    ins.push_back(p);
    return (int)ins.size() - 1;
}

static bool chain_fill(BuiltChain &bc, int b, const kc_plane *p)
{
    KC_PROF("chain_fill");
    const Chain &ch = *p->chain;
    ChainProgram &P = bc.prog;
    std::vector<const kc_plane *> ins;
    kc_plane *samp = nullptr;
    if (ch.start->kind == kc_plane::MEM) input_index(ins, ch.start);
    for (auto &st : ch.steps)
        if (st.operand->kind == kc_plane::MEM) input_index(ins, st.operand);
    auto slot = [&](kc_plane *q, float *c) -> int {
        if (q == saved_value_marker()) return KC_CHAIN_SRC_SAVED - 1;
        if (q->kind == kc_plane::MEM) return input_index(ins, q);
        if (q->kind == kc_plane::RESIZE) {
            samp = q;
            return -2;
        }
        *c = q->cval;
        return -1;
    };
    const int km = (int)ins.size();
    if (km > KC_CHAIN_MAX_IN) return false;
    float c0 = 0.0f;
    int start_src = slot(ch.start, &c0);
    if (start_src == -2) start_src = km;
    if (b == 0) {
        std::memset(&P, 0, sizeof(P));
        P.start_src = start_src;
    } else if (P.start_src != start_src) {
        return false;
    }
    P.start_c[b] = c0;
    size_t r = 0;
    for (size_t i = 0; i < ch.steps.size(); ++i, ++r) {
        const ChainStep &st = ch.steps[i];
        float c = 0.0f;
        int src = slot(st.operand, &c);
        if (src == -2) src = km;
        uint8_t code = st.code;
        if (code == CH_ADD_R) code = CH_ADD;
        if (code == CH_MUL_R) code = CH_MUL;
        if (code == CH_SAVE_LOAD) bc.joins = true;
        if (src >= 0 && code <= CH_MUL && i + 1 < ch.steps.size() && ch.steps[i + 1].code == CH_SUB_R &&
            ch.steps[i + 1].operand->kind == kc_plane::CONST && ch.steps[i + 1].operand != saved_value_marker()) {
            static const uint8_t inv[4] = { CH_ADD_INV, CH_SUBL_INV, CH_SUBR_INV, CH_MUL_INV };
            code = inv[code];
            c = ch.steps[i + 1].operand->cval;
            ++i;
        }
        uint32_t word = chain_op_word(code, src);
        if (st.code == CH_SAVE_LOAD || st.operand == saved_value_marker()) word |= (uint32_t)st.level << 16;
        auto rec = [&](int ch_) -> ChainStepRec & { return (r & 1) ? P.step[ch_][r / 2].b : P.step[ch_][r / 2].a; };
        if (b == 0) {
            rec(0).word = word;
            if (code == CH_DIV_L || code == CH_DIV_R) bc.mode = bc.mode < 1 ? 1 : bc.mode;
            if (code == CH_POW_L || code == CH_POW_R) bc.mode = 2;
        } else if (r >= P.n_ops || rec(0).word != word) {
            return false;
        }
        rec(b).word = word;
        rec(b).c = c;
    }
    if (b == 0)
        P.n_ops = (uint32_t)r;
    else if (P.n_ops != r)
        return false;
    const uint32_t n_in = (uint32_t)km + (samp ? 1u : 0u);
    if (b == 0)
        P.n_in = n_in;
    else if (P.n_in != n_in || (samp != nullptr) != (bc.sampled[0] != nullptr))
        return false;
    if (samp && b > 0) {
        const kc_plane *s0 = bc.sampled[0];
        if (samp->rz_filter != s0->rz_filter || samp->rz_src->w != s0->rz_src->w || samp->rz_src->h != s0->rz_src->h)
            return false;
    }
    bc.sampled[b] = samp;
    for (int k = 0; k < km; ++k) {
        P.in[b][k] = ins[k]->dptr;
        P.in_pitch[b][k] = (uint32_t)(ins[k]->pitch / 16);
        if (b == 0) bc.in_refs[k] = (uint32_t)ins[k]->refs;
    }
    if (samp) {
        P.samp_src[b] = samp->rz_src->dptr;
        P.samp_pitch[b] = (uint32_t)(samp->rz_src->pitch / 4);
    }
    return true;
}

static int chain_prepare(kc_plane *p)
{
    Chain &ch = *p->chain;
    kc_plane *first = nullptr;
    auto visit = [&](kc_plane *q) -> int {
        if (q->kind != kc_plane::RESIZE) return KC_OK;
        if (!first) {
            first = q;
            return KC_OK;
        }
        return q == first ? KC_OK : resize_force(q);
    };
    KC_TRY(visit(ch.start));
    for (auto &st : ch.steps) KC_TRY(visit(st.operand));
    return KC_OK;
}

uint32_t chain_cache_policy(const uint32_t *refs, uint32_t n, uint64_t stream_bytes, uint64_t out_bytes)
{
    const Options &o = options();
    if (!o.cache_policy) return 0;
    uint32_t all = 0;
    for (uint32_t k = 0; k < n; ++k) all |= KC_CHAIN_NT_BIT(k);
    if (o.nt_force >= 0) return (uint32_t)o.nt_force & (all | 0x100u);
    const uint64_t budget = (uint64_t)o.cache_budget_mb << 20;
    if (n * stream_bytes + out_bytes <= budget) return 0;
    uint32_t mask = all;
    uint64_t used = 0;
    for (;;) {
        int best = -1;
        for (uint32_t k = 0; k < n; ++k)
            if ((mask & KC_CHAIN_NT_BIT(k)) && refs[k] >= 2 && (best < 0 || refs[k] > refs[best])) best = (int)k;
        if (best < 0 || used + stream_bytes > budget) break;
        used += stream_bytes;
        mask &= ~KC_CHAIN_NT_BIT(best);
    }
    if (used + out_bytes > budget) mask |= 0x100u;
    return mask;
}

uint32_t cache_policy_mask(uint64_t in_bytes, uint64_t out_bytes, uint32_t n_resident, const Options &o)
{
    if (!o.cache_policy) return 0;
    if (o.nt_force >= 0) return (uint32_t)o.nt_force & (((1u << n_resident) - 1u) | 0x100u);
    const uint64_t budget = (uint64_t)o.cache_budget_mb << 20;
    if (in_bytes + out_bytes <= budget) return 0;
    uint32_t mask = (1u << n_resident) - 1u;
    if (out_bytes > budget) mask |= 0x100u;
    return mask;
}

namespace {
struct ChainCounterNames {
    std::string interp[5][9][3][2];
    std::string k0[3];
    std::string chain1[8];
    std::string spec[0x200], spec_q2[0x200], spec_q4[0x200];
    ChainCounterNames()
    {
        char buf[64];
        for (int k = 1; k <= 4; ++k)
            for (int u : { 1, 2, 4, 6, 8 })
                for (int m = 0; m < 3; ++m)
                    for (int nt = 0; nt < 2; ++nt) {
                        std::snprintf(buf, sizeof buf, "chain_interp_k%d_u%d_m%d%s", k, u, m, nt ? "_nt" : "");
                        interp[k][u][m][nt] = buf;
                    }
        for (int m = 0; m < 3; ++m) k0[m] = "chain_k0_m" + std::to_string(m);
        for (int b = 0; b < 8; ++b) chain1[b] = "chain1_nt" + std::to_string(b);
        for (int b = 0; b < 0x200; ++b) {
            std::snprintf(buf, sizeof buf, "specialized_nt_%03x", b);
            spec[b] = buf;
            spec_q2[b] = spec[b] + "_q2";
            spec_q4[b] = spec[b] + "_q4";
        }
    }
};
const ChainCounterNames &chain_counter_names()
{
    static const ChainCounterNames n;
    return n;
}
}

hipError_t chain_dispatch(ChainProgram &P, int batch, int mode, uint32_t w, uint32_t h, size_t out_pitch_bytes)
{
    Context &c = ctx();
    const uint32_t row_units = (w + 3) / 4;
    bool launched = false;
    bool dense = (size_t)row_units * 16 == out_pitch_bytes;
    for (int b = 0; b < batch && dense; ++b)
        for (uint32_t k = 0; k < P.n_in; ++k)
            if (P.in_pitch[b][k] != row_units) dense = false;
    if (dense) {
        P.rows = 1;
        P.row_units = row_units * h;
    } else {
// ... 104 lines not shown
        }
        if (e != hipSuccess) {
            for (auto *o : outs) plane_release(o);
            return hip_fail(e, "launch_chain");
        }
        if (bc.joins) c.counters["join_launches"]++;
        if (P.n_in > (uint32_t)KC_CHAIN_INTERP_IN) c.counters["wide_launches"]++;
    }
    c.launches++;
    {
        uint64_t px = (uint64_t)p0->w * p0->h, bytes = 0;
        for (int b = 0; b < batch; ++b) {
            const uint32_t resident = P.n_in - (bc.sampled[b] ? 1u : 0u);
            bytes += 4 * px * (resident + 1);
            if (bc.sampled[b]) bytes += 4 * (uint64_t)bc.sampled[b]->rz_src->w * bc.sampled[b]->rz_src->h;
        }
        c.alg_bytes += bytes;
    }
    if (c.capture) {
        ReplayCapture &cap = *c.capture;
        if (bc.sampled[0] || cap.launches.size() >= 32) cap.ok = false;
        else {
            cap.launches.emplace_back();
            ReplayLaunch &L = cap.launches.back();
            L.prog = P;
            L.batch = batch;
            L.mode = bc.mode;
            std::memcpy(L.in_refs, bc.in_refs, sizeof L.in_refs);
            L.w = p0->w;
            L.h = p0->h;
            for (int b = 0; b < batch; ++b) L.planes[b] = planes[b];
        }
    }
    for (int b = 0; b < batch; ++b) {
        kc_plane *p = planes[b];
        Chain *old = p->chain;
        ChainLink *old_link = p->link;
        p->chain = nullptr;
        p->link = nullptr;
        p->kind = kc_plane::MEM;
        p->dptr = outs[b]->dptr;
        p->pitch = outs[b]->pitch;
        p->bytes = outs[b]->bytes;
        p->owned = true;
        outs[b]->owned = false;
        outs[b]->dptr = nullptr;
        plane_release(outs[b]);
        delete old;
        delete old_link;
    }
    return KC_OK;
}

static int chain_flatten_to_fit(kc_plane *p, int limit)
{
    chain_flatten(p);
    while (chain_distinct_inputs(*p->chain) > limit || chain_record_count(*p->chain) > (size_t)KC_CHAIN_MAX_OPS) {
        if (!p->chain->joined.empty()) {
            std::vector<kc_plane *> subs(p->chain->joined);
            for (auto *q : subs) plane_retain(q);
            const int fs = planes_force(subs.data(), (int)subs.size());
            for (auto *q : subs) plane_release(q);
            KC_TRY(fs);
            if (p->kind != kc_plane::LAZY) return KC_OK;
            delete p->chain;
            p->chain = nullptr;
            chain_flatten(p);
            continue;
        }
        kc_plane *prev = p->link->prev;
        if (!prev || prev->kind != kc_plane::LAZY) {
            set_error("chain with more inputs than a program holds cannot be split");
            return KC_ERR_UNSUPPORTED;
        }
        {
            std::vector<kc_plane *> path;
            for (kc_plane *q = prev; q && q->kind == kc_plane::LAZY; q = q->link->prev) path.push_back(q);
            std::reverse(path.begin(), path.end());
            std::vector<ChainLink::InKey> keys;
            auto add = [&](const kc_plane *q) {
                ChainLink::InKey k;
                if (q->kind == kc_plane::MEM) k = { q->dptr, q->pitch };
                else if (q->kind == kc_plane::RESIZE) k = { q, ~(size_t)0 };
                else return;
                if (std::find(keys.begin(), keys.end(), k) == keys.end()) keys.push_back(k);
            };
            const ChainLink &first = *path[0]->link;
            add(first.prev ? first.prev : first.start);
            kc_plane *cut = nullptr;
            size_t steps = 0;
            for (kc_plane *q : path) {
                const kc_plane *o = q->link->step.operand;
                if (o->kind == kc_plane::LAZY) {
                    for (int i = 0; i < o->link->n_in && i <= KC_CHAIN_MAX_IN; ++i)
                        if (std::find(keys.begin(), keys.end(), o->link->ins[i]) == keys.end()) keys.push_back(o->link->ins[i]);
                    steps += o->link->length + 2u;
                    if (o->link->n_in > KC_CHAIN_MAX_IN) break;
                } else {
                    add(o);
                    ++steps;
                }
                if ((int)keys.size() > limit || steps > (size_t)KC_CHAIN_MAX_OPS) break;
                cut = q;
            }
            if (cut) prev = cut;
        }
        KC_TRY(plane_force(prev));
        delete p->chain;
        p->chain = nullptr;
        chain_flatten(p);
    }
    return KC_OK;
}

int planes_force(kc_plane *const *planes, int n)
{
    KC_PROF("planes_force");
    std::lock_guard<std::recursive_mutex> lk(ctx().mu);
    std::vector<kc_plane *> todo;
    KC_TRY(resize_force_many(planes, n));
    for (int i = 0; i < n; ++i) {
        kc_plane *p = planes[i];
        if (!p) continue;
        if (p->kind != kc_plane::LAZY) continue;
        bool dup = false;
        for (auto *q : todo) dup |= (q == p);
        if (!dup) todo.push_back(p);
    }
    if (todo.empty()) return KC_OK;
    KC_TRY(need_init());
    for (auto *p : todo) {
        if (p->kind != kc_plane::LAZY) continue;
        KC_TRY(chain_flatten_to_fit(p, chain_in_limit()));
        if (p->kind != kc_plane::LAZY) continue;
        {
            bool resampled = p->chain->start->kind == kc_plane::RESIZE;
            for (auto &st : p->chain->steps) resampled |= st.operand->kind == kc_plane::RESIZE;
            if (resampled && chain_distinct_inputs(*p->chain) > KC_CHAIN_INTERP_IN) {
                delete p->chain;
                p->chain = nullptr;
                KC_TRY(chain_flatten_to_fit(p, KC_CHAIN_INTERP_IN));
                if (p->kind != kc_plane::LAZY) continue;
            }
        }
        KC_TRY(chain_prepare(p));
    }
    todo.erase(std::remove_if(todo.begin(), todo.end(), [](kc_plane *q) { return q->kind != kc_plane::LAZY; }), todo.end());
    size_t i = 0;
    while (i < todo.size()) {
        if (todo[i]->kind != kc_plane::LAZY) {
            ++i;
            continue;
        }
        if (!todo[i]->chain) {
            KC_TRY(chain_flatten_to_fit(todo[i], KC_CHAIN_INTERP_IN));
            if (todo[i]->kind != kc_plane::LAZY) continue;
        }
        BuiltChain bc;
        kc_plane *group[KC_CHAIN_MAX_BATCH];
        int batch = 0;
        if (!chain_fill(bc, 0, todo[i])) {
            set_error("internal: chain does not fit one program");
            return KC_ERR_UNSUPPORTED;
        }
        group[batch++] = todo[i];
        size_t j = i + 1;
        while (j < todo.size() && batch < KC_CHAIN_MAX_BATCH && todo[j]->kind == kc_plane::LAZY && todo[j]->chain &&
               todo[j]->w == todo[i]->w && todo[j]->h == todo[i]->h && chain_fill(bc, batch, todo[j])) {
            group[batch++] = todo[j];
            ++j;
        }
        int s = chain_launch(bc, group, batch);
        if (s == KC_RETRY_CHAIN) continue;
        KC_TRY(s);
        i = j;
    }
    return KC_OK;
}

int plane_force(kc_plane *p) { return planes_force(&p, 1); }

int plane_materialize(kc_plane *p)
{
    KC_TRY(need_init());
    std::lock_guard<std::recursive_mutex> lk(ctx().mu);
    if (p->kind == kc_plane::LAZY || p->kind == kc_plane::RESIZE) return plane_force(p);
    if (p->kind == kc_plane::CONST) {
        kc_plane *m = nullptr;
        KC_TRY(plane_new_mem(p->w, p->h, &m));
        hipError_t e = launch_fill(m->dptr, (uint32_t)(m->pitch / 4), p->w, p->h, p->cval, ctx().stream);
        if (e != hipSuccess) {
            plane_release(m);
            return hip_fail(e, "launch_fill");
        }
        ctx().launches++;
        ctx().alg_bytes += (uint64_t)p->w * p->h * 4;
        p->kind = kc_plane::MEM;
        p->dptr = m->dptr;
        p->pitch = m->pitch;
        p->bytes = m->bytes;
        p->owned = true;
        m->owned = false;
        m->dptr = nullptr;
        plane_release(m);
    }
    return KC_OK;
}

static float fold_const(int mix, float l, float r)
{
    switch (mix) {
    case KC_MIX_ADD: return l + r;
    case KC_MIX_SUBTRACT: return l - r;
    case KC_MIX_MULTIPLY: return l * r;
    default: return l / r;
    }
}

static uint8_t code_for(int mix, bool acc_is_left)
{
    switch (mix) {
    case KC_MIX_ADD: return acc_is_left ? CH_ADD : CH_ADD_R;
    case KC_MIX_SUBTRACT: return acc_is_left ? CH_SUB_L : CH_SUB_R;
    case KC_MIX_MULTIPLY: return acc_is_left ? CH_MUL : CH_MUL_R;
    case KC_MIX_DIVIDE: return acc_is_left ? CH_DIV_L : CH_DIV_R;
    default: return acc_is_left ? CH_POW_L : CH_POW_R;
    }
}

static bool chain_full_with(const kc_plane *acc, const kc_plane *opnd)
{
    if (acc->link->length >= (uint32_t)KC_CHAIN_MAX_OPS) return true;
    int limit = chain_in_limit();
    if (opnd->kind == kc_plane::RESIZE) limit = KC_CHAIN_INTERP_IN;
    for (int i = 0; i < acc->link->n_in && i <= KC_CHAIN_MAX_IN; ++i)
        if (acc->link->ins[i].q == ~(size_t)0) limit = KC_CHAIN_INTERP_IN;
    if (acc->link->n_in < limit) return false;
    ChainLink probe;
    probe.n_in = acc->link->n_in;
    for (int i = 0; i < probe.n_in && i <= KC_CHAIN_MAX_IN; ++i) probe.ins[i] = acc->link->ins[i];
    link_add_input(probe, opnd);
    return probe.n_in > limit;
}

static kc_plane *lazy_pair_victim(kc_plane *l, kc_plane *r)
{
    return (l != r && l->link->length >= r->link->length) ? r : l;
}

static bool join_ok(const kc_plane *acc, const kc_plane *sub)
{
    Context &c = ctx();
    if (!c.opt.join || !c.opt.fusion || c.plain_chains || acc == sub || specialize_get_mode() == 0) return false;
    const ChainLink &A = *acc->link, &B = *sub->link;
    const int limit = chain_in_limit();
    if (std::max<int>(A.saved, B.saved + 1) > KC_CHAIN_MAX_SAVED || A.n_in > limit - 1 || B.n_in > limit) return false;
    if (A.length + B.length + 2u > (uint32_t)KC_CHAIN_MAX_OPS) return false;
    ChainLink probe;
    probe.n_in = A.n_in;
    for (int i = 0; i < A.n_in; ++i) {
        if (A.ins[i].q == ~(size_t)0) return false;
        probe.ins[i] = A.ins[i];
    }
    for (int i = 0; i < B.n_in; ++i) {
        if (B.ins[i].q == ~(size_t)0) return false;
        bool seen = false;
        for (int k = 0; k < probe.n_in && k <= KC_CHAIN_MAX_IN; ++k) seen |= probe.ins[k] == B.ins[i];
        if (!seen) {
            if (probe.n_in >= limit) return false;
// ... 143 lines not shown
```

### kanter_core_amd/csrc/specialize.cpp

```cpp
#include <dlfcn.h>
#include <sys/stat.h>
#include <unistd.h>

#include <condition_variable>
#include <cstdio>
#include <cstdlib>
#include <cstring>
#include <thread>

#include "kc_runtime.hpp"

namespace kc {

extern const char kJitChainProgramH[];
extern const char kJitPowPositiveInc[];
extern const char kJitUpsampleH[];
extern const char kJitUpsampleChainInc[];

namespace {

typedef struct _hiprtcProgram *hiprtcProgram;
struct Rtc {
    void *lib = nullptr;
    int (*create)(hiprtcProgram *, const char *, const char *, int, const char **, const char **) = nullptr;
    int (*compile)(hiprtcProgram, int, const char **) = nullptr;
    int (*log_size)(hiprtcProgram, size_t *) = nullptr;
    int (*log)(hiprtcProgram, char *) = nullptr;
    int (*code_size)(hiprtcProgram, size_t *) = nullptr;
    int (*code)(hiprtcProgram, char *) = nullptr;
    int (*destroy)(hiprtcProgram *) = nullptr;
    int (*version)(int *, int *) = nullptr;
    bool ok = false;
    bool tried = false;
};

void specialize_stop_at_exit();

Rtc &rtc()
{
    static Rtc r;
    static std::once_flag once;
    std::call_once(once, [] {
        r.tried = true;
        for (const char *name : { "libhiprtc.so", "libhiprtc.so.7", "/opt/rocm/lib/libhiprtc.so" }) {
            r.lib = dlopen(name, RTLD_NOW | RTLD_LOCAL);
            if (r.lib) break;
        }
        if (!r.lib) return;
#define KC_RTC_SYM(field, sym) *(void **)(&r.field) = dlsym(r.lib, sym)
        KC_RTC_SYM(create, "hiprtcCreateProgram");
        KC_RTC_SYM(compile, "hiprtcCompileProgram");
        KC_RTC_SYM(log_size, "hiprtcGetProgramLogSize");
        KC_RTC_SYM(log, "hiprtcGetProgramLog");
        KC_RTC_SYM(code_size, "hiprtcGetCodeSize");
        KC_RTC_SYM(code, "hiprtcGetCode");
        KC_RTC_SYM(destroy, "hiprtcDestroyProgram");
        KC_RTC_SYM(version, "hiprtcVersion");
#undef KC_RTC_SYM
        r.ok = r.create && r.compile && r.log_size && r.log && r.code_size && r.code && r.destroy;
        if (r.ok) std::atexit(specialize_stop_at_exit);
    });
    return r;
}

struct Signature {
    uint32_t n_in = 0, n_ops = 0;
    int32_t start_src = 0;
    bool flat = false;
    uint32_t up_taps = 0;
    bool up_wide = false;
    uint32_t nt_mask = 0;
    uint32_t quads = 1;
    uint32_t word[KC_CHAIN_MAX_OPS] = {};

    std::string key() const
    {
        std::string k((const char *)&n_in, sizeof n_in);
        k.append((const char *)&n_ops, sizeof n_ops);
        k.append((const char *)&start_src, sizeof start_src);
        k.push_back(flat ? 'f' : 'p');
        k.push_back((char)('0' + up_taps));
        k.push_back(up_wide ? 'w' : 'n');
        k.append((const char *)&nt_mask, sizeof nt_mask);
        k.append((const char *)word, sizeof(uint32_t) * n_ops);
        if (quads > 1) {
            k.push_back('q');
            k.push_back((char)('0' + quads));
        }
        return k;
    }
};

constexpr uint32_t kQuadsWarm = 2, kQuadsMaxOps = 16;
std::atomic<int> g_chain_quads{ 0 };

uint32_t chain_quads_for(const Signature &s, uint64_t total_units)
{
    if (s.up_taps || !s.flat || s.n_in < 1 || s.n_ops > kQuadsMaxOps || total_units > 0xF0000000ull) return 1;
    bool plain = false;
    for (uint32_t k = 0; k < s.n_in; ++k) plain |= !(s.nt_mask & KC_CHAIN_NT_BIT(k));
    if (!plain || !s.nt_mask) return 1;
    for (uint32_t i = 0; i < s.n_ops; ++i) {
        const uint32_t code = s.word[i] & 0xffu;
        if (code == CH_DIV_L || code == CH_DIV_R || code == CH_POW_L || code == CH_POW_R) return 1;
    }
    const int forced = g_chain_quads.load(std::memory_order_relaxed);
    return forced ? (uint32_t)forced : kQuadsWarm;
}

Signature signature_of(const ChainProgram &P, const UpsampleArgs *U = nullptr)
{
    Signature s;
    s.n_in = P.n_in;
    s.n_ops = P.n_ops;
    s.start_src = P.start_src;
    s.flat = U ? false : P.rows == 1;
    {
        uint32_t valid = 0x100u;
        for (uint32_t k = 0; k < (U ? P.n_in - 1u : P.n_in); ++k) valid |= KC_CHAIN_NT_BIT(k);
        s.nt_mask = P.nt_mask & valid;
    }
    if (U) {
        s.up_taps = U->H.taps;
        s.up_wide = U->tile_w == 1024;
    }
    for (uint32_t i = 0; i < P.n_ops; ++i) s.word[i] = (i & 1u) ? P.step[0][i / 2].b.word : P.step[0][i / 2].a.word;
    s.quads = chain_quads_for(s, (uint64_t)P.rows * P.row_units);
    return s;
}

static int spec_wg()
{
    static int wg = [] {
        int v = 256;
        if (const char *e = std::getenv("KC_SPEC_WG")) {
            const int x = std::atoi(e);
            if (x == 64 || x == 128 || x == 256 || x == 512 || x == 1024) v = x;
        }
        return v;
    }();
    return wg;
}

std::string kernel_name(const Signature &s)
{
    uint32_t h = 2166136261u;
    for (unsigned char c : s.key()) h = (h ^ c) * 16777619u;
    char buf[32];
    std::snprintf(buf, sizeof buf, s.up_taps ? "kc_upchain_%08x" : "kc_chain_%08x", h);
    return buf;
}

static const char kPackedF4[] = R"KCF4(typedef float raw4 __attribute__((ext_vector_type(4)));
typedef float f2 __attribute__((ext_vector_type(2)));
typedef unsigned long long __attribute__((may_alias)) rec64;
static __device__ __forceinline__ f2 pk_sub(f2 a, f2 b)
{
    f2 d;
    asm("v_pk_add_f32 %0, %1, %2 neg_lo:[0,1] neg_hi:[0,1]" : "=v"(d) : "v"(a), "v"(b));
    return d;
}
struct kconst {
    rec64 rec;  // { word, c }
    __device__ __forceinline__ operator float() const { return __builtin_bit_cast(float, (unsigned int)(rec >> 32)); }
    __device__ __forceinline__ f2 minus(f2 b) const
    {
        f2 d;
        asm("v_pk_add_f32 %0, %1, %2 op_sel_hi:[0,1] neg_lo:[0,1] neg_hi:[0,1]" : "=v"(d) : "s"(rec >> 32), "v"(b));
        return d;
    }
};
struct f4 {
    f2 lo, hi;
    f4() = default;
    __device__ __forceinline__ f4(float x, float y, float z, float w) : lo{ x, y }, hi{ z, w } {}
    __device__ __forceinline__ f4(f2 l, f2 h) : lo(l), hi(h) {}
    __device__ __forceinline__ f4(raw4 v) : lo(v.xy), hi(v.zw) {}
    __device__ __forceinline__ raw4 raw() const { return raw4{ lo.x, lo.y, hi.x, hi.y }; }
};
static __device__ __forceinline__ f4 operator+(f4 a, f4 b) { return f4(a.lo + b.lo, a.hi + b.hi); }
static __device__ __forceinline__ f4 operator*(f4 a, f4 b) { return f4(a.lo * b.lo, a.hi * b.hi); }
static __device__ __forceinline__ f4 operator-(f4 a, f4 b) { return f4(pk_sub(a.lo, b.lo), pk_sub(a.hi, b.hi)); }
static __device__ __forceinline__ f4 operator-(kconst c, f4 b) { return f4(c.minus(b.lo), c.minus(b.hi)); }
static __device__ __forceinline__ f4 operator/(f4 a, f4 b) { return f4(a.raw() / b.raw()); }
struct StepRecView { kconst c; };
struct StepPairView { StepRecView a, b; };
struct StepTableView {
    const ChainStepPair *p;
    __device__ __forceinline__ StepPairView operator[](unsigned int i) const
    {
        const rec64 *q = reinterpret_cast<const rec64 *>(p + i);
        return StepPairView{ { { q[0] } }, { { q[1] } } };
    }
};
)KCF4";

static std::string step_expr(const Signature &s, uint32_t i, const char *in_prefix, const char *in_suffix)
{
    const uint32_t code = s.word[i] & 0xffu, from = (s.word[i] >> 8) & 0xffu, level = (s.word[i] >> 16) & 3u;
    char c[48], x[96];
    std::snprintf(c, sizeof c, "pp[%u].%c.c", i / 2, (i & 1u) ? 'b' : 'a');
    if (from == 0)
        std::snprintf(x, sizeof x, "f4{ %s, %s, %s, %s }", c, c, c, c);
    else if (from == (uint32_t)KC_CHAIN_SRC_SAVED)
        std::snprintf(x, sizeof x, "saved%u", level);
    else
        std::snprintf(x, sizeof x, "%s%u%s", in_prefix, from - 1, in_suffix);
    switch (code) {
    case CH_SAVE_LOAD: return "(saved" + std::to_string(level) + " = acc, " + x + ")";
    case CH_ADD: return std::string("acc + ") + x;
    case CH_SUB_L: return std::string("acc - ") + x;
    case CH_SUB_R: return std::string(x) + " - acc";
    case CH_MUL: return std::string("acc * ") + x;
    case CH_DIV_L: return std::string("acc / ") + x;
    case CH_DIV_R: return std::string(x) + " / acc";
    case CH_POW_L: return std::string("pow4(acc, ") + x + ", pow_tab)";
    case CH_POW_R: return std::string("pow4(") + x + ", acc, pow_tab)";
    case CH_ADD_INV: return std::string(c) + " - (acc + " + x + ")";
    case CH_SUBL_INV: return std::string(c) + " - (acc - " + x + ")";
    case CH_SUBR_INV: return std::string(c) + " - (" + x + " - acc)";
    case CH_MUL_INV: return std::string(c) + " - (acc * " + x + ")";
    default: return std::string();
    }
}

static std::string generate_up(const Signature &s)
{
    std::string src;
    src.reserve(32768);
    src += "namespace kc {\n";
    src += kJitChainProgramH;
    src += kJitUpsampleH;
// ... 8 lines not shown
                  s.n_in, KC_UPSAMPLE_ROWS, KC_UPSAMPLE_ROWS, KC_UPSAMPLE_ROWS);
    src += buf;
    if (s.start_src < 0)
        src += "            f4 acc = f4{ P.start_c[b], P.start_c[b], P.start_c[b], P.start_c[b] };\n";
    else {
        std::snprintf(buf, sizeof buf, "            f4 acc = in[%d][u];\n", s.start_src);
        src += buf;
    }
    for (uint32_t i = 0; i < s.n_ops; ++i) {
        const uint32_t code = s.word[i] & 0xffu;
        if (code == CH_DIV_L || code == CH_DIV_R || code == CH_POW_L || code == CH_POW_R || code == CH_SAVE_LOAD) return std::string();
        const std::string e = step_expr(s, i, "in[", "][u]");
        if (e.empty()) return std::string();
        src += "            acc = " + e + ";\n";
    }
    src += "            out[u] = acc;\n        }\n    }\n};\n}  // namespace kc\nusing namespace kc;\n";
    std::snprintf(buf, sizeof buf,
                  "extern \"C\" __global__ __launch_bounds__(256) void %s(const ChainProgram P, const UpsampleArgs U)\n{\n"
                  "    extern __shared__ __attribute__((aligned(16))) float lds[];\n"
                  "    upsample_chain_tile<%u, %u, %u, %s, 0x%xu>(P, U, lds, UpProg{ P });\n}\n",
                  kernel_name(s).c_str(), s.n_in, s.up_taps, KC_UPSAMPLE_ROWS, s.up_wide ? "true" : "false", s.nt_mask);
    src += buf;
    return src;
}

static std::string generate_quads(const Signature &s, int SPEC_WG)
{
    std::string src;
    char buf[320];
    std::snprintf(buf, sizeof buf,
                  "    const unsigned int n = P.rows * P.row_units;\n"
                  "    const unsigned int idx = blockIdx.x * %uu + threadIdx.x;\n    if (idx >= n) return;\n",
                  s.quads * (uint32_t)SPEC_WG);
    src += buf;
    for (uint32_t u = 0; u < s.quads; ++u) {
        if (u == 0)
            src += "    const unsigned int at0 = idx;\n";
        else {
            std::snprintf(buf, sizeof buf, "    const unsigned int at%u = idx + %uu < n ? idx + %uu : n - 1u;\n", u, u * SPEC_WG, u * SPEC_WG);
            src += buf;
        }
        for (uint32_t k = 0; k < s.n_in; ++k) {
            if (s.nt_mask & KC_CHAIN_NT_BIT(k))
                std::snprintf(buf, sizeof buf, "    const f4 in%u_%u = __builtin_nontemporal_load(&reinterpret_cast<const raw4 *>(P.in[b][%u])[at%u]);\n", k, u, k, u);
            else
                std::snprintf(buf, sizeof buf, "    const f4 in%u_%u = reinterpret_cast<const raw4 *>(P.in[b][%u])[at%u];\n", k, u, k, u);
            src += buf;
        }
    }
    src += "    const StepTableView pp{ P.step[b] };\n";
    for (uint32_t u = 0; u < s.quads; ++u) {
        char suffix[8];
        std::snprintf(suffix, sizeof suffix, "_%u", u);
        std::snprintf(buf, sizeof buf, "    f4 out%u;\n    {\n", u);
        src += buf;
        if (s.start_src < 0)
            src += "        f4 acc = f4{ P.start_c[b], P.start_c[b], P.start_c[b], P.start_c[b] };\n";
        else {
            std::snprintf(buf, sizeof buf, "        f4 acc = in%d%s;\n", s.start_src, suffix);
            src += buf;
        }
        src += "        f4 saved0 = acc, saved1 = acc, saved2 = acc;\n";
        for (uint32_t i = 0; i < s.n_ops; ++i) {
            const std::string e = step_expr(s, i, "in", suffix);
            if (e.empty()) return std::string();
            src += "        acc = " + e + ";\n";
        }
        std::snprintf(buf, sizeof buf, "        out%u = acc;\n    }\n", u);
        src += buf;
    }
    for (uint32_t u = 0; u < s.quads; ++u) {
        std::snprintf(buf, sizeof buf, "    if (idx + %uu < n) ", u * SPEC_WG);
        src += u ? buf : "    ";
        std::snprintf(buf, sizeof buf,
                      s.nt_mask & 0x100u ? "__builtin_nontemporal_store(out%u.raw(), &reinterpret_cast<raw4 *>(P.out[b])[idx + %uu]);\n"
                                         : "reinterpret_cast<raw4 *>(P.out[b])[idx + %uu] = out%u.raw();\n",
                      s.nt_mask & 0x100u ? u : u * SPEC_WG, s.nt_mask & 0x100u ? u * SPEC_WG : u);
        src += buf;
    }
    src += "}\n";
    return src;
}

std::string generate(const Signature &s)
{
    if (s.up_taps) return generate_up(s);
    const int SPEC_WG = spec_wg();
    bool pow = false;
    for (uint32_t i = 0; i < s.n_ops; ++i) pow |= (s.word[i] & 0xffu) == CH_POW_L || (s.word[i] & 0xffu) == CH_POW_R;
    std::string src;
    src.reserve(16384);
    src += "namespace kc {\n";
    src += kJitChainProgramH;
    src += kPackedF4;
    if (pow) {
        src += kJitPowPositiveInc;
        src += "static __device__ __noinline__ float pow_general(float a, float b) { return (float)pow((double)a, (double)b); }\n"
               "static __device__ __forceinline__ float kc_powf(float a, float b, const PowCtx &pw)\n"
               "{\n"
               "    if (a > 0.0f && a < __builtin_inff() && __builtin_fabsf(b) < __builtin_inff()) return pow_positive(a, b, pw);\n"
               "    return pow_general(a, b);\n"
               "}\n"
               "static __device__ __forceinline__ f4 pow4(f4 a, f4 b, const PowCtx &t) { return f4{ kc_powf(a.lo.x, b.lo.x, t), kc_powf(a.lo.y, b.lo.y, t), kc_powf(a.hi.x, b.hi.x, t), kc_powf(a.hi.y, b.hi.y, t) }; }\n";
    }
    src += "}  // namespace kc\nusing namespace kc;\n";
    char buf[256];
    std::snprintf(buf, sizeof buf, "extern \"C\" __global__ __launch_bounds__(%d) void %s(const ChainProgram P)\n{\n", SPEC_WG,
                  kernel_name(s).c_str());
    src += buf;
    if (pow) src += "    __shared__ double pow_lds[KC_POW_TABLE_DOUBLES];\n    const PowCtx pow_tab = pow_setup(pow_lds);\n";
    src += "    const unsigned int b = blockIdx.y;\n";
    if (s.quads > 1) {
        const std::string body = generate_quads(s, SPEC_WG);
        return body.empty() ? body : src + body;
    }
    std::snprintf(buf, sizeof buf, "    const unsigned int idx = blockIdx.x * %du + threadIdx.x;\n", SPEC_WG);
    src += buf;
    src += "    if (idx >= P.rows * P.row_units) return;\n";
    if (s.flat)
        src += "    const unsigned int row = 0u, col = idx;\n";
    else
        src += "    const unsigned int row = idx / P.row_units, col = idx - row * P.row_units;\n";
    for (uint32_t k = 0; k < s.n_in; ++k) {
        if (s.nt_mask & KC_CHAIN_NT_BIT(k))
            std::snprintf(buf, sizeof buf, "    const f4 in%u = __builtin_nontemporal_load(&reinterpret_cast<const raw4 *>(P.in[b][%u])[row * P.in_pitch[b][%u] + col]);\n", k, k, k);
        else
            std::snprintf(buf, sizeof buf, "    const f4 in%u = reinterpret_cast<const raw4 *>(P.in[b][%u])[row * P.in_pitch[b][%u] + col];\n", k, k, k);
        src += buf;
    }
    src += "    const StepTableView pp{ P.step[b] };\n";
    if (s.start_src < 0)
        src += "    f4 acc = f4{ P.start_c[b], P.start_c[b], P.start_c[b], P.start_c[b] };\n";
    else {
        std::snprintf(buf, sizeof buf, "    f4 acc = in%d;\n", s.start_src);
        src += buf;
    }
    src += "    f4 saved0 = acc, saved1 = acc, saved2 = acc;\n";
    for (uint32_t i = 0; i < s.n_ops; ++i) {
        const std::string e = step_expr(s, i, "in", "");
        if (e.empty()) return std::string();
        src += "    acc = " + e + ";\n";
    }
    if (s.nt_mask & 0x100u)
        src += "    __builtin_nontemporal_store(acc.raw(), &reinterpret_cast<raw4 *>(P.out[b])[row * P.out_pitch[b] + col]);\n}\n";
    else
        src += "    reinterpret_cast<raw4 *>(P.out[b])[row * P.out_pitch[b] + col] = acc.raw();\n}\n";
    return src;
}

static const char *const kCompileOpts[] = { "--gpu-architecture=gfx950", "-O3", "-ffp-contract=off", "-fno-fast-math",
                                            "-fhip-fp32-correctly-rounded-divide-sqrt" };
constexpr int kNumCompileOpts = (int)(sizeof kCompileOpts / sizeof *kCompileOpts);

uint64_t fnv64(const void *data, size_t n, uint64_t h = 1469598103934665603ull)
{
    const unsigned char *p = (const unsigned char *)data;
    for (size_t i = 0; i < n; ++i) h = (h ^ p[i]) * 1099511628211ull;
    return h;
}

struct CacheHeader {
    char magic[8];
    uint64_t key_len, source_hash, code_len, code_hash;
};

struct DiskCache {
    std::mutex mu;
    bool resolved = false;
    std::string write_dir;
// ... 189 lines not shown
    return true;
}

struct Entry {
    enum State { COUNTING, QUEUED, READY, FAILED } state = COUNTING;
    uint32_t sightings = 0;
    Signature sig;
    hipModule_t module = nullptr;
    hipFunction_t fn = nullptr;
};

struct Spec {
    std::mutex mu;
    std::condition_variable cv, idle_cv;
    std::map<std::string, Entry> cache;
    std::unordered_map<uint64_t, std::pair<std::string, Entry *>> by_hash;
    std::deque<std::string> queue;
    std::thread worker;
    bool worker_running = false, stopping = false;
    int busy = 0;
    std::atomic<int> mode{ 1 };
    uint32_t after = 2;
    int device = -1;
    uint64_t compiled = 0, failed = 0, launches = 0, loaded_from_disk = 0;
    std::string last_log;

    void stop()
    {
        {
            std::lock_guard<std::mutex> lk(mu);
            stopping = true;
            for (auto &key : queue) {
                auto it = cache.find(key);
                if (it != cache.end() && it->second.state == Entry::QUEUED) {
                    it->second.state = Entry::COUNTING;
                    it->second.sightings = 0;
                }
            }
            queue.clear();
        }
        cv.notify_all();
        idle_cv.notify_all();
        if (worker.joinable()) worker.join();
        std::lock_guard<std::mutex> lk(mu);
        worker_running = false;
        stopping = false;
    }
};

Spec &spec()
{
    static Spec *s = new Spec();
    return *s;
}

void specialize_stop_at_exit() { spec().stop(); }

bool compile_entry(const Signature &sig, hipModule_t *module, hipFunction_t *fn, std::string *log, bool disk_only = false)
{
    const std::string src = generate(sig);
    if (src.empty()) {
        *log = "unknown step code";
        return false;
    }
    std::vector<char> code;
    if (disk_load(sig, src, code)) {
        if (load_code(sig, code, module, fn, log)) return true;
        std::lock_guard<std::mutex> lk(disk().mu);
        disk().hits--;
        disk().rejected++;
    }
    if (disk_only) {
        *log = "not in the kernel cache";
        return false;
    }
    if (!rtc_compile(src, code, log)) return false;
    if (!load_code(sig, code, module, fn, log)) return false;
    disk_store(sig, src, code);
    if (const char *m = std::getenv("KC_KERNEL_CACHE_MANIFEST")) {
        if (FILE *f = std::fopen(m, "a")) {
            std::fprintf(f, "{\"name\": \"%s\", \"n_in\": %u, \"start_src\": %d, \"flat\": %d, \"nt_mask\": %u, \"up_taps\": %u, \"up_wide\": %d, \"words\": [",
                         kernel_name(sig).c_str(), sig.n_in, sig.start_src, sig.flat ? 1 : 0, sig.nt_mask, sig.up_taps, sig.up_wide ? 1 : 0);
            for (uint32_t k = 0; k < sig.n_ops; ++k) std::fprintf(f, "%s%u", k ? ", " : "", sig.word[k]);
            std::fprintf(f, "]}\n");
            std::fclose(f);
        }
    }
    return true;
}

void finish(Spec &S, const std::string &key, bool ok, hipModule_t m, hipFunction_t f, const std::string &log, bool from_disk = false)
{
    auto it = S.cache.find(key);
    if (it == S.cache.end()) {
        if (ok) (void)hipModuleUnload(m);
        return;
    }
    if (ok) {
        it->second.module = m;
        it->second.fn = f;
        it->second.state = Entry::READY;
        if (from_disk) S.loaded_from_disk++;
        else S.compiled++;
    } else {
        it->second.state = Entry::FAILED;
        S.failed++;
        S.last_log = log;
    }
}

void worker_main()
{
    Spec &S = spec();
    if (S.device >= 0) (void)hipSetDevice(S.device);
    std::unique_lock<std::mutex> lk(S.mu);
    for (;;) {
        S.cv.wait(lk, [&] { return S.stopping || !S.queue.empty(); });
        if (S.stopping) return;
        const std::string key = S.queue.front();
        S.queue.pop_front();
        auto it = S.cache.find(key);
        if (it == S.cache.end()) continue;
        const Signature sig = it->second.sig;
        S.busy++;
        lk.unlock();
        hipModule_t m = nullptr;
        hipFunction_t f = nullptr;
        std::string log;
        const uint64_t hits0 = disk_hits();
        const bool ok = compile_entry(sig, &m, &f, &log);
        const bool from_disk = ok && disk_hits() != hits0;
        lk.lock();
        S.busy--;
        finish(S, key, ok, m, f, log, from_disk);
        S.idle_cv.notify_all();
    }
}

}

static uint64_t signature_hash(const Signature &s)
{
    uint64_t h = 1469598103934665603ull;
    auto mix = [&](uint64_t v) { h = (h ^ v) * 1099511628211ull; };
    mix(s.n_in);
    mix(s.n_ops);
    mix((uint64_t)(int64_t)s.start_src);
    mix(s.flat ? 1 : 0);
    mix(s.up_taps);
    mix(s.up_wide ? 1 : 0);
    mix(s.nt_mask);
    mix(s.quads);
    for (uint32_t i = 0; i < s.n_ops; ++i) mix(s.word[i]);
    return h;
}

static bool same_signature(const Signature &a, const Signature &b)
{
    return a.n_in == b.n_in && a.n_ops == b.n_ops && a.start_src == b.start_src && a.flat == b.flat && a.up_taps == b.up_taps &&
           a.up_wide == b.up_wide && a.nt_mask == b.nt_mask && a.quads == b.quads &&
           std::memcmp(a.word, b.word, sizeof(uint32_t) * a.n_ops) == 0;
}

static hipFunction_t spec_lookup(const Signature &sig)
{
    Spec &S = spec();
    if (S.mode.load(std::memory_order_relaxed) == 0) return nullptr;
    const uint64_t h = signature_hash(sig);
    {
        std::lock_guard<std::mutex> fast(S.mu);
        auto it = S.by_hash.find(h);
        if (it != S.by_hash.end() && it->second.second->state == Entry::READY && same_signature(it->second.second->sig, sig))
            return it->second.second->fn;
    }
    const std::string key = sig.key();
    std::unique_lock<std::mutex> lk(S.mu);
    if (S.mode == 2) {
        auto it = S.cache.find(key);
        if (it != S.cache.end() && it->second.state == Entry::QUEUED)
            S.idle_cv.wait(lk, [&] { return S.cache[key].state != Entry::QUEUED || !S.worker_running; });
    }
    Entry &e = S.cache[key];
    if (e.state == Entry::READY) {
        e.sig = sig;
        S.by_hash[h] = { key, &e };
        return e.fn;
    }
    if (e.state != Entry::COUNTING) return nullptr;
    e.sightings++;
    if (e.sightings == 1 && S.mode == 1) {
        hipModule_t m = nullptr;
        hipFunction_t f = nullptr;
        std::string log;
        e.sig = sig;
        if (compile_entry(sig, &m, &f, &log, true)) {
            e.module = m;
            e.fn = f;
            e.state = Entry::READY;
            S.loaded_from_disk++;
            S.by_hash[h] = { key, &e };
            return f;
        }
    }
    if (S.mode == 1 && e.sightings < S.after) return nullptr;
    e.sig = sig;
    if (S.mode == 2) {
        e.state = Entry::QUEUED;
        lk.unlock();
        hipModule_t m = nullptr;
        hipFunction_t f = nullptr;
        std::string log;
        const uint64_t hits0 = disk_hits();
        const bool ok = compile_entry(sig, &m, &f, &log);
        const bool from_disk = ok && disk_hits() != hits0;
        lk.lock();
        finish(S, key, ok, m, f, log, from_disk);
        return ok ? f : nullptr;
    }
    e.state = Entry::QUEUED;
    S.queue.push_back(key);
    if (!S.worker_running) {
        S.device = ctx().device;
        S.stopping = false;
        S.worker = std::thread(worker_main);
        S.worker_running = true;
    }
    lk.unlock();
    S.cv.notify_one();
    return nullptr;
}

hipError_t launch_chain_specialized(const ChainProgram &P, int batch, hipStream_t s, bool *launched, uint32_t *nt_mask, uint32_t *quads)
{
    *launched = false;
    if (P.n_ops < 1 || P.n_ops > (uint32_t)KC_CHAIN_MAX_OPS || P.n_in > (uint32_t)KC_CHAIN_MAX_IN) return hipSuccess;
    const uint64_t total = (uint64_t)P.rows * P.row_units;
    if (total == 0 || total > 0xFFFFFFFFull) return hipSuccess;
    const Signature sig = signature_of(P);
    hipFunction_t fn = spec_lookup(sig);
    if (!fn) return hipSuccess;
    size_t size = sizeof(ChainProgram);
    const int SPEC_WG = spec_wg();
    void *extra[] = { HIP_LAUNCH_PARAM_BUFFER_POINTER, (void *)&P, HIP_LAUNCH_PARAM_BUFFER_SIZE, &size, HIP_LAUNCH_PARAM_END };
    const uint64_t per_block = (uint64_t)SPEC_WG * sig.quads;
    const unsigned gx = (unsigned)((total + per_block - 1) / per_block);
    hipError_t e = hipModuleLaunchKernel(fn, gx, (unsigned)batch, 1, SPEC_WG, 1, 1, 0, s, nullptr, extra);
    if (e == hipSuccess) {
        *launched = true;
        if (nt_mask) *nt_mask = sig.nt_mask;
        if (quads) *quads = sig.quads;
        std::lock_guard<std::mutex> lk(spec().mu);
        spec().launches++;
    }
    return e;
}

hipError_t launch_upsample_chain_specialized(const ChainProgram &P, int batch, const UpsampleArgs &U, hipStream_t s, bool *launched)
{
    *launched = false;
    if (P.n_ops < 1 || P.n_ops > (uint32_t)KC_CHAIN_MAX_OPS || P.n_in < 1 || P.n_in > (uint32_t)KC_CHAIN_INTERP_IN) return hipSuccess;
    if (!upsample_args_ok(U, batch) || (U.H.taps != 1 && U.H.taps != 3)) return hipSuccess;
    if (U.H.ratio == 2) return hipSuccess;
    hipFunction_t fn = spec_lookup(signature_of(P, &U));
    if (!fn) return hipSuccess;
    struct alignas(16) Params {
        ChainProgram P;
        UpsampleArgs U;
    };
    static_assert(sizeof(ChainProgram) % alignof(UpsampleArgs) == 0, "the second kernel argument follows the first without padding");
    static thread_local Params params;
    params.P = P;
    params.U = U;
    size_t size = sizeof(Params);
    void *extra[] = { HIP_LAUNCH_PARAM_BUFFER_POINTER, (void *)&params, HIP_LAUNCH_PARAM_BUFFER_SIZE, &size, HIP_LAUNCH_PARAM_END };
    const dim3 grid = upsample_grid(U, batch);
    hipError_t e = hipModuleLaunchKernel(fn, grid.x, grid.y, grid.z, 256, 1, 1, (unsigned)upsample_lds_bytes(U), s, nullptr, extra);
    if (e == hipSuccess) {
        *launched = true;
        std::lock_guard<std::mutex> lk(spec().mu);
        spec().launches++;
    }
    return e;
}

int specialize_set_mode(int mode, int after)
{
    Spec &S = spec();
    if (mode < 0 || mode > 2) return KC_ERR_INVALID_ARG;
    {
        std::lock_guard<std::mutex> lk(S.mu);
        S.mode.store(mode);
        if (after >= 1) S.after = (uint32_t)after;
    }
    if (mode == 0) S.stop();
    return KC_OK;
}

int specialize_get_mode()
{
    Spec &S = spec();
    return S.mode.load();
}

void specialize_wait()
{
    Spec &S = spec();
    std::unique_lock<std::mutex> lk(S.mu);
    S.idle_cv.wait(lk, [&] { return S.stopping || (S.queue.empty() && S.busy == 0); });
}

void specialize_stats(uint64_t *compiled, uint64_t *failed, uint64_t *launches, uint64_t *pending)
{
    Spec &S = spec();
    std::lock_guard<std::mutex> lk(S.mu);
    if (compiled) *compiled = S.compiled;
    if (failed) *failed = S.failed;
    if (launches) *launches = S.launches;
    if (pending) *pending = S.queue.size() + (uint64_t)S.busy;
}

std::string specialize_last_log()
{
    Spec &S = spec();
    std::lock_guard<std::mutex> lk(S.mu);
    return S.last_log;
}

void specialize_shutdown()
{
    Spec &S = spec();
    S.stop();
    std::lock_guard<std::mutex> lk(S.mu);
    for (auto &kv : S.cache)
        if (kv.second.module) (void)hipModuleUnload(kv.second.module);
    S.by_hash.clear();
    S.cache.clear();
}

int specialize_set_chain_quads(int quads)
{
    if (quads != 0 && quads != 1 && quads != 2 && quads != 4) return KC_ERR_INVALID_ARG;
    g_chain_quads.store(quads);
    return KC_OK;
}

int specialize_get_chain_quads() { return g_chain_quads.load(); }

std::string specialize_source(const ChainProgram &P, const UpsampleArgs *U) { return generate(signature_of(P, U)); }

int specialize_compile_only(const ChainProgram &P, std::string *log, const UpsampleArgs *U)
{
    if (!rtc().ok) {
        *log = "libhiprtc not available";
        return KC_ERR_UNSUPPORTED;
    }
    const std::string src = generate(signature_of(P, U));
    if (src.empty()) return KC_ERR_GENERIC;
    std::vector<char> code;
    return rtc_compile(src, code, log) ? KC_OK : KC_ERR_GENERIC;
}

int kernel_cache_set_dir(const char *dir)
{
    DiskCache &d = disk();
    std::lock_guard<std::mutex> lk(d.mu);
    resolve_dirs_locked(d, dir && *dir ? dir : nullptr);
    return KC_OK;
}

void kernel_cache_stats(uint64_t *hits, uint64_t *rejected, uint64_t *written, uint64_t *kernels_loaded)
{
    {
        DiskCache &d = disk();
        std::lock_guard<std::mutex> lk(d.mu);
        if (hits) *hits = d.hits;
        if (rejected) *rejected = d.rejected;
        if (written) *written = d.written;
    }
    Spec &S = spec();
    std::lock_guard<std::mutex> lk(S.mu);
    if (kernels_loaded) *kernels_loaded = S.loaded_from_disk;
}

bool kernel_cache_populated()
{
    DiskCache &d = disk();
    std::vector<std::string> dirs;
    {
        std::lock_guard<std::mutex> lk(d.mu);
        if (!d.resolved) resolve_dirs_locked(d, nullptr);
        dirs = d.read_dirs;
        if (dirs.empty()) return false;
        if (d.hits) return true;
    }
    static std::map<std::string, bool> seen;
    for (auto &dir : dirs) {
        auto it = seen.find(dir);
        if (it == seen.end()) {
            bool any = false;
            std::string probe = dir + "/.populated";
            any = access(probe.c_str(), R_OK) == 0;
            it = seen.emplace(dir, any).first;
        }
        if (it->second) return true;
    }
    return false;
}

int kernel_cache_precompile(const uint32_t *words, uint32_t n_ops, uint32_t n_in, int32_t start_src, bool flat, uint32_t nt_mask,
                            uint32_t up_taps, bool up_wide, const char *dir, std::string *log)
{
    if (!words || n_ops < 1 || n_ops > (uint32_t)KC_CHAIN_MAX_OPS || n_in > (uint32_t)KC_CHAIN_MAX_IN || !dir || !*dir) return KC_ERR_INVALID_ARG;
    Signature sig;
    sig.n_in = n_in;
    sig.n_ops = n_ops;
    sig.start_src = start_src;
    sig.flat = flat;
    sig.nt_mask = nt_mask;
    sig.up_taps = up_taps;
    sig.up_wide = up_wide;
    for (uint32_t i = 0; i < n_ops; ++i) sig.word[i] = words[i];
    sig.quads = chain_quads_for(sig, 0);
    const std::string src = generate(sig);
    if (src.empty()) {
        *log = "unknown step code";
        return KC_ERR_INVALID_ARG;
    }
    std::vector<char> code;
    if (!rtc_compile(src, code, log)) return rtc().ok ? KC_ERR_GENERIC : KC_ERR_UNSUPPORTED;
    if (!make_dirs(dir) || !disk_store_in(dir, sig, src, code)) {
        *log = std::string("cannot write into ") + dir;
        return KC_ERR_IO;
    }
    if (FILE *f = std::fopen((std::string(dir) + "/.populated").c_str(), "w")) std::fclose(f);
    return KC_OK;
}

}
```

### kanter_core_amd/csrc/streaming.h

```cpp
#pragma once

[[maybe_unused]] static uint64_t grid_cap(uint64_t dflt)
{
    const int cap = options().tune_cap;
    return cap > 0 ? (uint64_t)cap : dflt;
}

template <bool NT, class V>
static __device__ __forceinline__ V ld_policy(const V *p)
{
    if constexpr (NT) return __builtin_nontemporal_load(p);
    else return *p;
}
template <bool NT, class V>
static __device__ __forceinline__ void st_policy(V *p, V v)
{
    if constexpr (NT) __builtin_nontemporal_store(v, p);
    else *p = v;
}

static __device__ __forceinline__ uint32_t quant_u8(float v)
{
    float x = v;
    if (x < 0.0f) x = 0.0f;
    if (x > 1.0f) x = 1.0f;
    x = x * 255.0f;
    if (!(x <= 255.0f)) x = 255.0f;
    return (uint32_t)x;
}

#include "srgb_thresholds.inc"

static __device__ __forceinline__ uint32_t quant_u8_srgb(float v, const uint32_t *T)
{
    float x = v;
    if (x < 0.0f) x = 0.0f;
    if (x > 1.0f) x = 1.0f;
    if (x != x) return 255u;
    const uint32_t xb = __float_as_uint(x);
    if ((int32_t)xb <= 0) return 0u;
    const float est = 255.0f * __builtin_amdgcn_exp2f(2.4f * __builtin_amdgcn_logf((x + 0.055f) * (1.0f / 1.055f)));
    const uint32_t q = xb < T[1] ? 0u : (uint32_t)fminf(est, 255.0f);
    return q + (xb >= T[q + 1u] ? 1u : 0u) - (xb < T[q] ? 1u : 0u);
}
```

### kanter_core_amd/csrc/u8pipe.cpp

```cpp
#include "kc_runtime.hpp"

struct kc_u8_pipe {
    uint32_t w = 0, h = 0;
    int channels = 4, depth = 0;
    size_t in_bytes = 0, out_bytes = 0;
    hipStream_t up = nullptr, down = nullptr;
    struct Slot {
        uint8_t *host_in = nullptr, *host_out = nullptr;
        uint8_t *dev_in = nullptr, *dev_out = nullptr;
        hipEvent_t copied_in = nullptr;
        hipEvent_t converted = nullptr;
        hipEvent_t packed = nullptr;
        hipEvent_t copied_out = nullptr;
        bool in_used = false, out_used = false;
    };
    std::vector<Slot> slots;
};

namespace kc {

int u8_pipe_free(kc_u8_pipe *p)
{
    if (!p) return KC_OK;
    if (p->up) (void)hipStreamSynchronize(p->up);
    if (p->down) (void)hipStreamSynchronize(p->down);
    if (ctx().stream) (void)hipStreamSynchronize(ctx().stream);
    for (auto &s : p->slots) {
        if (s.host_in) (void)hipHostFree(s.host_in);
        if (s.host_out) (void)hipHostFree(s.host_out);
        if (s.dev_in) (void)hipFree(s.dev_in);
        if (s.dev_out) (void)hipFree(s.dev_out);
        for (hipEvent_t e : { s.copied_in, s.converted, s.packed, s.copied_out })
            if (e) (void)hipEventDestroy(e);
    }
    if (p->up) (void)hipStreamDestroy(p->up);
    if (p->down) (void)hipStreamDestroy(p->down);
    delete p;
    return KC_OK;
}

int u8_pipe_create(uint32_t w, uint32_t h, int channels, int depth, kc_u8_pipe **out)
{
    KC_TRY(need_init());
    if (w == 0 || h == 0 || channels < 1 || channels > 4 || depth < 1 || depth > 16 || !out) {
        set_error("kc_u8_pipe_create: width and height > 0, 1..4 channels, 1..16 slots");
        return KC_ERR_INVALID_ARG;
    }
    kc_u8_pipe *p = new kc_u8_pipe();
    p->w = w;
    p->h = h;
    p->channels = channels;
    p->depth = depth;
    p->in_bytes = (size_t)w * h * channels;
    p->out_bytes = (size_t)w * h * 4;
    p->slots.resize((size_t)depth);
    hipError_t e = hipStreamCreateWithFlags(&p->up, hipStreamNonBlocking);
    if (e == hipSuccess) e = hipStreamCreateWithFlags(&p->down, hipStreamNonBlocking);
    for (auto &s : p->slots) {
        if (e == hipSuccess) e = hipHostMalloc((void **)&s.host_in, p->in_bytes, hipHostMallocDefault);
        if (e == hipSuccess) e = hipHostMalloc((void **)&s.host_out, p->out_bytes, hipHostMallocDefault);
        if (e == hipSuccess) e = hipMalloc((void **)&s.dev_in, (p->in_bytes + 255) / 256 * 256);
        if (e == hipSuccess) e = hipMalloc((void **)&s.dev_out, (p->out_bytes + 255) / 256 * 256);
        for (hipEvent_t *ev : { &s.copied_in, &s.converted, &s.packed, &s.copied_out })
            if (e == hipSuccess) e = hipEventCreateWithFlags(ev, hipEventDisableTiming);
    }
    if (e != hipSuccess) {
        const int st = e == hipErrorOutOfMemory ? KC_ERR_OUT_OF_MEMORY : hip_fail(e, "kc_u8_pipe_create");
        if (st == KC_ERR_OUT_OF_MEMORY) set_error("kc_u8_pipe_create: out of (pinned or device) memory");
        (void)hipGetLastError();
        (void)u8_pipe_free(p);
        return st;
    }
    *out = p;
    return KC_OK;
}

static int slot_of(kc_u8_pipe *p, int slot, kc_u8_pipe::Slot **s)
{
    if (!p || slot < 0 || slot >= p->depth) {
        set_error("kc_u8_pipe: no such slot");
        return KC_ERR_INVALID_ARG;
    }
    *s = &p->slots[(size_t)slot];
    return KC_OK;
}

int u8_pipe_buffers(kc_u8_pipe *p, int slot, uint8_t **host_in, const uint8_t **host_out)
{
    kc_u8_pipe::Slot *s = nullptr;
    KC_TRY(slot_of(p, slot, &s));
    if (host_in) *host_in = s->host_in;
    if (host_out) *host_out = s->host_out;
    return KC_OK;
}

int u8_pipe_upload(kc_u8_pipe *p, int slot, kc_image **out)
{
    kc_u8_pipe::Slot *s = nullptr;
    KC_TRY(slot_of(p, slot, &s));
    Context &c = ctx();
    kc_plane *pl[4] = { nullptr, nullptr, nullptr, nullptr };
    float *dp[4] = { nullptr, nullptr, nullptr, nullptr };
    int st = KC_OK;
    for (int i = 0; i < 4 && st == KC_OK; ++i) {
        if (i < p->channels) {
            st = plane_new_mem(p->w, p->h, &pl[i]);
            if (st == KC_OK) dp[i] = pl[i]->dptr;
        } else {
            pl[i] = plane_new_const(p->w, p->h, i == 3 ? 1.0f : 0.0f);
        }
    }
    if (st == KC_OK) {
        hipError_t e = hipSuccess;
        if (s->in_used) e = hipStreamWaitEvent(p->up, s->converted, 0);
        if (e == hipSuccess) e = hipMemcpyAsync(s->dev_in, s->host_in, p->in_bytes, hipMemcpyHostToDevice, p->up);
        if (e == hipSuccess) e = hipEventRecord(s->copied_in, p->up);
        if (e == hipSuccess) e = hipStreamWaitEvent(c.stream, s->copied_in, 0);
        if (e == hipSuccess)
            e = launch_from_u8(s->dev_in, p->channels, p->w, p->h, dp, (uint32_t)(pl[0]->pitch / 4),
                               cache_policy_mask(p->in_bytes, (uint64_t)p->w * p->h * 4 * p->channels, 1), c.stream);
        if (e == hipSuccess) e = hipEventRecord(s->converted, c.stream);
        if (e != hipSuccess) st = hip_fail(e, "kc_u8_pipe_upload");
        else {
            s->in_used = true;
            c.launches++;
            c.alg_bytes += (uint64_t)p->w * p->h * p->channels * 5;
        }
    }
    if (st == KC_OK) *out = image_new(4, pl);
    for (int i = 0; i < 4; ++i) plane_release(pl[i]);
    return st;
}

int u8_pipe_download(kc_u8_pipe *p, int slot, kc_image *img, bool srgb)
{
    kc_u8_pipe::Slot *s = nullptr;
    KC_TRY(slot_of(p, slot, &s));
    if (!img || img->w() != p->w || img->h() != p->h) {
        set_error("kc_u8_pipe_download: the image has another size than the pipe's");
        return KC_ERR_INVALID_ARG;
    }
    Context &c = ctx();
    KC_TRY(image_force(img));
    Operand o[4];
    for (int i = 0; i < 4; ++i) o[i] = plane_operand(img->planes[img->is_rgba() ? i : 0]);
    uint32_t n_res = 0;
    for (int i = 0; i < (img->is_rgba() ? 4 : 1); ++i) n_res += o[i].ptr != nullptr;
    hipError_t e = hipSuccess;
    if (s->out_used) e = hipStreamWaitEvent(c.stream, s->copied_out, 0);
    if (e == hipSuccess)
        e = launch_to_u8(o[0], o[1], o[2], o[3], img->is_rgba() ? 0 : 1, srgb ? 1 : 0, p->w, p->h, s->dev_out,
                         cache_policy_mask((uint64_t)p->w * p->h * 4 * n_res, p->out_bytes, n_res ? n_res : 1), c.stream);
    if (e == hipSuccess) e = hipEventRecord(s->packed, c.stream);
    if (e == hipSuccess) e = hipStreamWaitEvent(p->down, s->packed, 0);
    if (e == hipSuccess) e = hipMemcpyAsync(s->host_out, s->dev_out, p->out_bytes, hipMemcpyDeviceToHost, p->down);
    if (e == hipSuccess) e = hipEventRecord(s->copied_out, p->down);
    if (e != hipSuccess) return hip_fail(e, "kc_u8_pipe_download");
    s->out_used = true;
    c.launches++;
    c.alg_bytes += (uint64_t)p->w * p->h * 4 * (n_res + 1);
    return KC_OK;
}

int u8_pipe_wait_download(kc_u8_pipe *p, int slot)
{
    kc_u8_pipe::Slot *s = nullptr;
    KC_TRY(slot_of(p, slot, &s));
    if (!s->out_used) return KC_OK;
    KC_HIP(hipEventSynchronize(s->copied_out));
    return KC_OK;
}

}
```

Baseline: 6.424 million.

## Fuse u8 unpack and pack into specialized chain kernels via deferred U8 source planes

Adds a lazy U8SRC plane kind so uploaded RGBA8 buffers are not expanded to f32 planes up front. Chain kernels read the u8 bytes directly, and the download path can run a specialized kernel that writes RGBA8 output, falling back to the old path when fusion is not possible. The goal is to drop the separate from_u8 and to_u8 passes and their f32 intermediate traffic. In exchange it adds reference-counted deferred-source lifetime management, new JIT signatures and fallbacks that force materialization.

Measured after the change: 6.415 million, median of 3. Within noise of the previous version (-0.1%).

```diff
diff --git a/bindings/rust/kanter_core_amd_sys.rs b/bindings/rust/kanter_core_amd_sys.rs
--- a/bindings/rust/kanter_core_amd_sys.rs
+++ b/bindings/rust/kanter_core_amd_sys.rs
@@ -119,10 +119,14 @@
     pub fn kc_specialize_compile_check_mask(words: *const u32, n_ops: u32, n_in: u32, start_src: i32, flat: i32, nt_mask: u32, source: *mut c_char, cap: usize) -> i32;
     pub fn kc_set_chain_quads(quads: i32) -> i32;
     pub fn kc_get_chain_quads() -> i32;
+    pub fn kc_set_u8_fuse(on: i32) -> i32;
+    pub fn kc_get_u8_fuse() -> i32;
+    pub fn kc_specialize_compile_check_u8(words: *const u32, n_ops: u32, n_in: u32, start_src: i32, flat: i32, nt_mask: u32, u8_mask: u32, sink: i32, source: *mut c_char, cap: usize) -> i32;
     pub fn kc_specialize_compile_check_upsample(words: *const u32, n_ops: u32, n_in: u32, start_src: i32, taps: u32, wide: i32, source: *mut c_char, cap: usize) -> i32;
     pub fn kc_kernel_cache_set_dir(dir: *const c_char) -> i32;
     pub fn kc_kernel_cache_stats(files_accepted: *mut u64, files_refused: *mut u64, files_written: *mut u64, kernels_loaded: *mut u64) -> i32;
     pub fn kc_kernel_cache_precompile(words: *const u32, n_ops: u32, n_in: u32, start_src: i32, flat: i32, nt_mask: u32, up_taps: u32, up_wide: i32, dir: *const c_char) -> i32;
+    pub fn kc_kernel_cache_precompile_u8(words: *const u32, n_ops: u32, n_in: u32, start_src: i32, flat: i32, nt_mask: u32, u8_mask: u32, sink: i32, dir: *const c_char) -> i32;
     pub fn kc_specialize_reset() -> i32;
     pub fn kc_plane_alloc(width: u32, height: u32, out: *mut *mut KcPlane) -> i32;
     pub fn kc_plane_const(width: u32, height: u32, value: f32, out: *mut *mut KcPlane) -> i32;
diff --git a/include/kanter_core_amd.h b/include/kanter_core_amd.h
--- a/include/kanter_core_amd.h
+++ b/include/kanter_core_amd.h
@@ -109,12 +109,18 @@
                                             uint32_t nt_mask, char *source, size_t cap);
 KC_API int kc_set_chain_quads(int quads);
 KC_API int kc_get_chain_quads(void);
+KC_API int kc_set_u8_fuse(int on);
+KC_API int kc_get_u8_fuse(void);
+KC_API int kc_specialize_compile_check_u8(const uint32_t *words, uint32_t n_ops, uint32_t n_in, int start_src, int flat,
+                                          uint32_t nt_mask, uint32_t u8_mask, int sink, char *source, size_t cap);
 KC_API int kc_specialize_compile_check_upsample(const uint32_t *words, uint32_t n_ops, uint32_t n_in, int start_src, uint32_t taps,
                                                 int wide, char *source, size_t cap);
 KC_API int kc_kernel_cache_set_dir(const char *dir);
 KC_API int kc_kernel_cache_stats(uint64_t *files_accepted, uint64_t *files_refused, uint64_t *files_written, uint64_t *kernels_loaded);
 KC_API int kc_kernel_cache_precompile(const uint32_t *words, uint32_t n_ops, uint32_t n_in, int start_src, int flat, uint32_t nt_mask,
                                       uint32_t up_taps, int up_wide, const char *dir);
+KC_API int kc_kernel_cache_precompile_u8(const uint32_t *words, uint32_t n_ops, uint32_t n_in, int start_src, int flat, uint32_t nt_mask,
+                                         uint32_t u8_mask, int sink, const char *dir);
 KC_API int kc_specialize_reset(void);
 
 KC_API int kc_plane_alloc(uint32_t width, uint32_t height, kc_plane **out);
diff --git a/kanter_core_amd/__init__.py b/kanter_core_amd/__init__.py
--- a/kanter_core_amd/__init__.py
+++ b/kanter_core_amd/__init__.py
@@ -4,7 +4,7 @@
                   init, is_initialized, mix_process, resize_image, separate_rgba_process, set_fusion, set_stream,
                   shutdown, stats, sync, value_process, set_specialize, get_specialize, specialize_wait,
                   specialize_stats, specialize_compile_check, Partition, PartitionPolicy, NodeKind, set_resize_mode,
-                  get_resize_mode, resize_upsample_plan, resize_down2_plan, stats_counter, specialize_compile_check_upsample, specialize_compile_check_mask, set_chain_quads, get_chain_quads, set_cache_policy, get_cache_policy, set_option, get_option, comm_unique_id, comm_init,
+                  get_resize_mode, resize_upsample_plan, resize_down2_plan, stats_counter, specialize_compile_check_upsample, specialize_compile_check_mask, set_chain_quads, get_chain_quads, set_u8_fuse, get_u8_fuse, specialize_compile_check_u8, set_cache_policy, get_cache_policy, set_option, get_option, comm_unique_id, comm_init,
                   comm_destroy, comm_info, comm_stats, comm_transport, comm_gather_bands, PlanKind, pool_trim, kernel_cache_set_dir, kernel_cache_stats,
                   kernel_cache_precompile, specialize_reset, U8Pipe, device_image_desc, DEVICE_SRGB, DEVICE_GRAY,
                   ChannelStats, STATS_HISTOGRAM, STATS_SRGB, BC_SRGB, BC_BLOCK_BYTES,
diff --git a/kanter_core_amd/_lib.py b/kanter_core_amd/_lib.py
--- a/kanter_core_amd/_lib.py
+++ b/kanter_core_amd/_lib.py
@@ -106,6 +106,12 @@
     "kc_specialize_compile_check_mask": (C.c_int, [c_u32p, C.c_uint32, C.c_uint32, C.c_int, C.c_int, C.c_uint32, C.c_char_p, C.c_size_t]),
     "kc_set_chain_quads": (C.c_int, [C.c_int]),
     "kc_get_chain_quads": (C.c_int, []),
+    "kc_set_u8_fuse": (C.c_int, [C.c_int]),
+    "kc_get_u8_fuse": (C.c_int, []),
+    "kc_specialize_compile_check_u8": (C.c_int, [c_u32p, C.c_uint32, C.c_uint32, C.c_int, C.c_int, C.c_uint32, C.c_uint32, C.c_int, C.c_char_p,
+                                                 C.c_size_t]),
+    "kc_kernel_cache_precompile_u8": (C.c_int, [C.POINTER(C.c_uint32), C.c_uint32, C.c_uint32, C.c_int, C.c_int, C.c_uint32, C.c_uint32, C.c_int,
+                                                C.c_char_p]),
     "kc_specialize_compile_check_upsample": (C.c_int, [c_u32p, C.c_uint32, C.c_uint32, C.c_int, C.c_uint32, C.c_int, C.c_char_p,
                                                        C.c_size_t]),
     "kc_stats_algorithmic_bytes": (C.c_int, [C.POINTER(C.c_uint64)]),
diff --git a/kanter_core_amd/api.py b/kanter_core_amd/api.py
--- a/kanter_core_amd/api.py
+++ b/kanter_core_amd/api.py
@@ -213,6 +213,22 @@
 
 def get_chain_quads():
     return _lib.load().kc_get_chain_quads()
+
+
+def set_u8_fuse(on):
+    _check(_lib.load().kc_set_u8_fuse(int(bool(on))))
+
+
+def get_u8_fuse():
+    return _lib.load().kc_get_u8_fuse()
+
+
+def specialize_compile_check_u8(words, n_in, nt_mask=0, u8_mask=0, sink=0, start_src=0, flat=True):
+    arr = (C.c_uint32 * len(words))(*words)
+    buf = C.create_string_buffer(1 << 17)
+    _check(_lib.load().kc_specialize_compile_check_u8(arr, len(words), int(n_in), int(start_src), int(bool(flat)), int(nt_mask),
+                                                      int(u8_mask), int(sink), buf, len(buf)))
+    return buf.value.decode()
 
 
 def specialize_compile_check_upsample(words, n_in, start_src=0, taps=3, wide=True):
diff --git a/kanter_core_amd/build.py b/kanter_core_amd/build.py
--- a/kanter_core_amd/build.py
+++ b/kanter_core_amd/build.py
@@ -12,7 +12,7 @@
            "u8pipe.cpp", "devimage.hip", "devimage.cpp", "stats.hip", "stats.cpp", "bc.hip", "bc.cpp", "mip.hip", "mip.cpp",
            "c_api.cpp"]
 HEADERS = ["kc_internal.hpp", "kc_runtime.hpp", "chain_program.h", os.path.join("..", "..", "include", "kanter_core_amd.h"), "pow_positive.inc",
-           "srgb_thresholds.inc", "streaming.h", "upsample.h", "upsample_chain.inc", "chain_apply.inc", "chain_interp.inc", "resample.inc"]
+           "srgb_thresholds.inc", "streaming.h", "quant_u8.inc", "u8source.h", "upsample.h", "upsample_chain.inc", "chain_apply.inc", "chain_interp.inc", "resample.inc"]
 JIT_TEXTS = [("kJitChainProgramH", "chain_program.h"), ("kJitPowPositiveInc", "pow_positive.inc"), ("kJitUpsampleH", "upsample.h"),
              ("kJitUpsampleChainInc", "upsample_chain.inc")]
 
@@ -127,12 +127,19 @@
     L.kc_kernel_cache_precompile.argtypes = [C.POINTER(C.c_uint32), C.c_uint32, C.c_uint32, C.c_int, C.c_int, C.c_uint32, C.c_uint32,
                                              C.c_int, C.c_char_p]
     L.kc_kernel_cache_precompile.restype = C.c_int
+    L.kc_kernel_cache_precompile_u8.argtypes = [C.POINTER(C.c_uint32), C.c_uint32, C.c_uint32, C.c_int, C.c_int, C.c_uint32, C.c_uint32,
+                                                C.c_int, C.c_char_p]
+    L.kc_kernel_cache_precompile_u8.restype = C.c_int
     L.kc_last_error.restype = C.c_char_p
 
     def one(e):
         words = (C.c_uint32 * len(e["words"]))(*e["words"])
-        rc = L.kc_kernel_cache_precompile(words, len(e["words"]), e["n_in"], e["start_src"], e["flat"], e["nt_mask"], e["up_taps"],
-                                          e["up_wide"], KERNEL_CACHE.encode())
+        if e.get("sink", 0):
+            rc = L.kc_kernel_cache_precompile_u8(words, len(e["words"]), e["n_in"], e["start_src"], e["flat"], e["nt_mask"], e["u8_mask"],
+                                                 e["sink"], KERNEL_CACHE.encode())
+        else:
+            rc = L.kc_kernel_cache_precompile(words, len(e["words"]), e["n_in"], e["start_src"], e["flat"], e["nt_mask"], e["up_taps"],
+                                              e["up_wide"], KERNEL_CACHE.encode())
         if rc != 0:
             raise RuntimeError("pre-compiling %s failed (%d): %s" % (e.get("name"), rc, (L.kc_last_error() or b"").decode(errors="replace")))
         if verbose:
diff --git a/kanter_core_amd/csrc/c_api.cpp b/kanter_core_amd/csrc/c_api.cpp
--- a/kanter_core_amd/csrc/c_api.cpp
+++ b/kanter_core_amd/csrc/c_api.cpp
@@ -416,6 +416,63 @@
     return 0;
 }
 
+int kc_set_u8_fuse(int on)
+try {
+    Lock lk(ctx().mu);
+    return u8_set_fuse(on);
+}
+KC_CATCH
+
+int kc_get_u8_fuse(void)
+try {
+    return u8_get_fuse();
+}
+catch (...) {
+    return 0;
+}
+
+int kc_specialize_compile_check_u8(const uint32_t *words, uint32_t n_ops, uint32_t n_in, int start_src, int flat, uint32_t nt_mask,
+                                   uint32_t u8_mask, int sink, char *source, size_t cap)
+try {
+    KC_ARG(words && n_ops >= 1 && n_ops <= (uint32_t)KC_CHAIN_MAX_OPS && n_in <= (uint32_t)KC_CHAIN_MAX_IN);
+    KC_ARG(start_src >= -1 && start_src < (int)n_in && sink >= 0 && sink <= 2 && (n_in >= 32 || (u8_mask >> n_in) == 0));
+    KC_ARG((sink == 0) == (u8_mask == 0));
+    ChainProgram P;
+    std::memset(&P, 0, sizeof P);
+    P.n_ops = n_ops;
+    P.n_in = n_in;
+    P.start_src = start_src;
+    P.rows = flat ? 1u : 2u;
+    P.row_units = 1;
+    P.nt_mask = nt_mask;
+    for (uint32_t i = 0; i < n_ops; ++i) {
+        const uint32_t from = (words[i] >> 8) & 0xffu, level = words[i] >> 16;
+        KC_ARG((words[i] & 0xffu) <= CH_SAVE_LOAD && (from <= n_in || (from == (uint32_t)KC_CHAIN_SRC_SAVED && (words[i] & 0xffu) != CH_SAVE_LOAD)));
+        KC_ARG(level < (uint32_t)KC_CHAIN_MAX_SAVED && (level == 0 || from == (uint32_t)KC_CHAIN_SRC_SAVED || (words[i] & 0xffu) == CH_SAVE_LOAD));
+        ((i & 1u) ? P.step[0][i / 2].b : P.step[0][i / 2].a).word = words[i];
+    }
+    if (source && cap) {
+        const std::string src = specialize_source_sig(P, u8_mask, sink);
+        std::snprintf(source, cap, "%s", src.c_str());
+    }
+    std::string log;
+    int s = specialize_compile_only_sig(P, u8_mask, sink, &log);
+    if (s != KC_OK) set_error("specialised chain kernel did not compile: " + log);
+    return s;
+}
+KC_CATCH
+
+int kc_kernel_cache_precompile_u8(const uint32_t *words, uint32_t n_ops, uint32_t n_in, int start_src, int flat, uint32_t nt_mask,
+                                  uint32_t u8_mask, int sink, const char *dir)
+try {
+    KC_ARG(words && dir && u8_mask && (sink == 1 || sink == 2));
+    std::string log;
+    const int s = kernel_cache_precompile(words, n_ops, n_in, start_src, flat != 0, nt_mask, 0, false, dir, &log, u8_mask, sink);
+    if (s != KC_OK) set_error("kernel cache: " + log);
+    return s;
+}
+KC_CATCH
+
 int kc_kernel_cache_set_dir(const char *dir)
 try {
     Lock lk(ctx().mu);
diff --git a/kanter_core_amd/csrc/kc_runtime.hpp b/kanter_core_amd/csrc/kc_runtime.hpp
--- a/kanter_core_amd/csrc/kc_runtime.hpp
+++ b/kanter_core_amd/csrc/kc_runtime.hpp
@@ -9,6 +9,7 @@
 #include <unordered_set>
 
 #include "kc_internal.hpp"
+#include "u8source.h"
 
 namespace kc {
 struct Chain;
@@ -75,7 +76,7 @@
 }
 
 struct kc_plane : kc::Pooled<kc_plane> {
-    enum Kind { MEM = 0, CONST = 1, LAZY = 2, RESIZE = 3 };
+    enum Kind { MEM = 0, CONST = 1, LAZY = 2, RESIZE = 3, U8SRC = 4 };
     int refs = 1;
     uint32_t w = 0, h = 0;
     Kind kind = MEM;
@@ -89,6 +90,8 @@
     kc_plane *view_of = nullptr;
     kc_plane *rz_src = nullptr;
     int rz_filter = 0;
+    kc::U8Source *u8 = nullptr;
+    int u8_ch = 0;
 };
 
 struct kc_image : kc::Pooled<kc_image> {
@@ -320,11 +323,15 @@
 uint32_t cache_policy_mask(uint64_t in_bytes, uint64_t out_bytes, uint32_t n_resident, const Options &o = options());
 uint32_t chain_cache_policy(const uint32_t *refs, uint32_t n, uint64_t stream_bytes, uint64_t out_bytes);
 hipError_t chain_dispatch(ChainProgram &P, int batch, int mode, uint32_t w, uint32_t h, size_t out_pitch_bytes);
+hipError_t launch_chain_rgba8_specialized(const ChainProgram &P, uint32_t u8_mask, int sink, hipStream_t s, bool *launched);
+int chain_launch_rgba8(kc_image *img, uint8_t *dst, bool *launched, U8Source **read);
 hipError_t launch_upsample_chain_specialized(const ChainProgram &P, int batch, const UpsampleArgs &U, hipStream_t s, bool *launched);
 int specialize_set_mode(int mode, int after);
 int specialize_get_mode();
 int specialize_set_chain_quads(int quads);
 int specialize_get_chain_quads();
+std::string specialize_source_sig(const ChainProgram &P, uint32_t u8_mask, int sink);
+int specialize_compile_only_sig(const ChainProgram &P, uint32_t u8_mask, int sink, std::string *log);
 void specialize_wait();
 void specialize_stats(uint64_t *compiled, uint64_t *failed, uint64_t *launches, uint64_t *pending);
 std::string specialize_last_log();
@@ -335,7 +342,7 @@
 void kernel_cache_stats(uint64_t *hits, uint64_t *rejected, uint64_t *written, uint64_t *kernels_loaded);
 bool kernel_cache_populated();
 int kernel_cache_precompile(const uint32_t *words, uint32_t n_ops, uint32_t n_in, int32_t start_src, bool flat, uint32_t nt_mask,
-                            uint32_t up_taps, bool up_wide, const char *dir, std::string *log);
+                            uint32_t up_taps, bool up_wide, const char *dir, std::string *log, uint32_t u8_mask = 0, int sink = 0);
 
 int u8_pipe_create(uint32_t w, uint32_t h, int channels, int depth, kc_u8_pipe **out);
 int u8_pipe_free(kc_u8_pipe *p);
@@ -343,6 +350,10 @@
 int u8_pipe_upload(kc_u8_pipe *p, int slot, kc_image **out);
 int u8_pipe_download(kc_u8_pipe *p, int slot, kc_image *img, bool srgb);
 int u8_pipe_wait_download(kc_u8_pipe *p, int slot);
+int u8_planes_force(kc_plane *const *planes, int n);
+int u8_source_force(U8Source *src);
+int u8_set_fuse(int on);
+int u8_get_fuse();
 
 int png_read(const std::string &path, std::vector<uint8_t> &px, uint32_t &w, uint32_t &h, int &channels);
 int png_write_rgba8(const std::string &path, const uint8_t *px, uint32_t w, uint32_t h);
diff --git a/kanter_core_amd/csrc/quant_u8.inc b/kanter_core_amd/csrc/quant_u8.inc
--- /dev/null
+++ b/kanter_core_amd/csrc/quant_u8.inc
@@ -0,0 +1,11 @@
+KC_QUANT_U8_TEXT(
+static __device__ __forceinline__ unsigned int quant_u8(float v)
+{
+    float x = v;
+    if (x < 0.0f) x = 0.0f;
+    if (x > 1.0f) x = 1.0f;
+    x = x * 255.0f;
+    if (!(x <= 255.0f)) x = 255.0f;
+    return (unsigned int)x;
+}
+)
diff --git a/kanter_core_amd/csrc/runtime.cpp b/kanter_core_amd/csrc/runtime.cpp
--- a/kanter_core_amd/csrc/runtime.cpp
+++ b/kanter_core_amd/csrc/runtime.cpp
@@ -236,6 +236,7 @@
         if (p->chain) delete p->chain;
         if (p->link) delete p->link;
         if (p->rz_src) plane_release(p->rz_src);
+        if (p->u8) u8source_detach_plane(p->u8, p->u8_ch, p);
         if (p->view_of) plane_release(p->view_of);
         if (p->owned && p->dptr) pool_free(p->dptr, p->bytes);
         delete p;
@@ -292,6 +293,8 @@
         k = { q->dptr, q->pitch };
     else if (q->kind == kc_plane::RESIZE)
         k = { q, ~(size_t)0 };
+    else if (q->kind == kc_plane::U8SRC)
+        k = { q, ~(size_t)1 };
     else
         return;
     for (int i = 0; i < L.n_in && i <= KC_CHAIN_MAX_IN; ++i)
@@ -305,7 +308,7 @@
 static int chain_distinct_inputs(const Chain &ch)
 {
     std::vector<const kc_plane *> ins;
-    auto counts = [](const kc_plane *q) { return q->kind == kc_plane::MEM || q->kind == kc_plane::RESIZE; };
+    auto counts = [](const kc_plane *q) { return q->kind == kc_plane::MEM || q->kind == kc_plane::RESIZE || q->kind == kc_plane::U8SRC; };
     if (counts(ch.start)) input_index(ins, ch.start);
     for (auto &s : ch.steps)
         if (counts(s.operand)) input_index(ins, s.operand);
@@ -395,6 +398,9 @@
     int mode = 0;
     kc_plane *sampled[KC_CHAIN_MAX_BATCH] = { nullptr, nullptr, nullptr, nullptr };
     bool joins = false;
+    bool allow_u8 = false;
+    uint32_t u8_mask = 0;
+    U8Source *u8_src = nullptr;
 };
 
 static int input_index(std::vector<const kc_plane *> &ins, const kc_plane *p)
@@ -414,12 +420,18 @@
     ChainProgram &P = bc.prog;
     std::vector<const kc_plane *> ins;
     kc_plane *samp = nullptr;
-    if (ch.start->kind == kc_plane::MEM) input_index(ins, ch.start);
+    bool stray_u8 = false;
+    auto takes_slot = [&](const kc_plane *q) {
+        if (q->kind == kc_plane::U8SRC && !bc.allow_u8) stray_u8 = true;
+        return q->kind == kc_plane::MEM || q->kind == kc_plane::U8SRC;
+    };
+    if (takes_slot(ch.start)) input_index(ins, ch.start);
     for (auto &st : ch.steps)
-        if (st.operand->kind == kc_plane::MEM) input_index(ins, st.operand);
+        if (st.operand != saved_value_marker() && takes_slot(st.operand)) input_index(ins, st.operand);
+    if (stray_u8) return false;
     auto slot = [&](kc_plane *q, float *c) -> int {
         if (q == saved_value_marker()) return KC_CHAIN_SRC_SAVED - 1;
-        if (q->kind == kc_plane::MEM) return input_index(ins, q);
+        if (q->kind == kc_plane::MEM || q->kind == kc_plane::U8SRC) return input_index(ins, q);
         if (q->kind == kc_plane::RESIZE) {
             samp = q;
             return -2;
@@ -484,11 +496,23 @@
             return false;
     }
     bc.sampled[b] = samp;
+    uint32_t u8_mask = 0;
     for (int k = 0; k < km; ++k) {
+        if (ins[k]->kind == kc_plane::U8SRC) {
+            if (!bc.u8_src) bc.u8_src = ins[k]->u8;
+            if (ins[k]->u8 != bc.u8_src || ins[k]->u8_ch != b || !ins[k]->u8->base) return false;
+            u8_mask |= 1u << k;
+            P.in[b][k] = nullptr;
+            P.in_pitch[b][k] = 0;
+            if (b == 0) bc.in_refs[k] = 1;
+            continue;
+        }
         P.in[b][k] = ins[k]->dptr;
         P.in_pitch[b][k] = (uint32_t)(ins[k]->pitch / 16);
         if (b == 0) bc.in_refs[k] = (uint32_t)ins[k]->refs;
     }
+    if (b == 0) bc.u8_mask = u8_mask;
+    else if (bc.u8_mask != u8_mask) return false;
     if (samp) {
         P.samp_src[b] = samp->rz_src->dptr;
         P.samp_pitch[b] = (uint32_t)(samp->rz_src->pitch / 4);
@@ -510,6 +534,15 @@
     };
     KC_TRY(visit(ch.start));
     for (auto &st : ch.steps) KC_TRY(visit(st.operand));
+    return KC_OK;
+}
+
+static int chain_force_u8(kc_plane *p)
+{
+    Chain &ch = *p->chain;
+    if (ch.start->kind == kc_plane::U8SRC) KC_TRY(u8_planes_force(&ch.start, 1));
+    for (auto &st : ch.steps)
+        if (st.operand->kind == kc_plane::U8SRC) KC_TRY(u8_planes_force(&st.operand, 1));
     return KC_OK;
 }
 
@@ -780,6 +813,7 @@
                 ChainLink::InKey k;
                 if (q->kind == kc_plane::MEM) k = { q->dptr, q->pitch };
                 else if (q->kind == kc_plane::RESIZE) k = { q, ~(size_t)0 };
+                else if (q->kind == kc_plane::U8SRC) k = { q, ~(size_t)1 };
                 else return;
                 if (std::find(keys.begin(), keys.end(), k) == keys.end()) keys.push_back(k);
             };
@@ -817,6 +851,7 @@
     std::lock_guard<std::recursive_mutex> lk(ctx().mu);
     std::vector<kc_plane *> todo;
     KC_TRY(resize_force_many(planes, n));
+    KC_TRY(u8_planes_force(planes, n));
     for (int i = 0; i < n; ++i) {
         kc_plane *p = planes[i];
         if (!p) continue;
@@ -842,6 +877,7 @@
             }
         }
         KC_TRY(chain_prepare(p));
+        KC_TRY(chain_force_u8(p));
     }
     todo.erase(std::remove_if(todo.begin(), todo.end(), [](kc_plane *q) { return q->kind != kc_plane::LAZY; }), todo.end());
     size_t i = 0;
@@ -853,6 +889,7 @@
         if (!todo[i]->chain) {
             KC_TRY(chain_flatten_to_fit(todo[i], KC_CHAIN_INTERP_IN));
             if (todo[i]->kind != kc_plane::LAZY) continue;
+            KC_TRY(chain_force_u8(todo[i]));
         }
         BuiltChain bc;
         kc_plane *group[KC_CHAIN_MAX_BATCH];
@@ -878,11 +915,91 @@
 
 int plane_force(kc_plane *p) { return planes_force(&p, 1); }
 
+static uint32_t quant_u8_host(float v)
+{
+    float x = v;
+    if (x < 0.0f) x = 0.0f;
+    if (x > 1.0f) x = 1.0f;
+    x = x * 255.0f;
+    if (!(x <= 255.0f)) x = 255.0f;
+    return (uint32_t)x;
+}
+
+int chain_launch_rgba8(kc_image *img, uint8_t *dst, bool *launched, U8Source **read)
+{
+    *launched = false;
+    *read = nullptr;
+    Context &c = ctx();
+    if (!img->is_rgba() || (img->w() & 3u) != 0) return KC_OK;
+    kc_plane *alpha = img->planes[3];
+    if (alpha->kind != kc_plane::CONST && alpha->kind != kc_plane::MEM) return KC_OK;
+    for (int b = 0; b < 3; ++b)
+        if (img->planes[b]->kind != kc_plane::LAZY) return KC_OK;
+    BuiltChain bc;
+    bc.allow_u8 = true;
+    bool ok = true;
+    for (int b = 0; b < 3 && ok; ++b) {
+        kc_plane *p = img->planes[b];
+        chain_flatten(p);
+        const Chain &ch = *p->chain;
+        ok = ch.joined.empty() && ch.start->kind != kc_plane::RESIZE && chain_distinct_inputs(ch) <= KC_CHAIN_MAX_IN &&
+             chain_record_count(ch) <= (size_t)KC_CHAIN_MAX_OPS;
+        for (auto &st : ch.steps) ok = ok && st.operand->kind != kc_plane::RESIZE && st.operand->kind != kc_plane::LAZY;
+        ok = ok && chain_fill(bc, b, p);
+    }
+    for (int b = 0; b < 3; ++b) {
+        delete img->planes[b]->chain;
+        img->planes[b]->chain = nullptr;
+    }
+    ChainProgram &P = bc.prog;
+    if (!ok || bc.joins || bc.mode == 2 || bc.sampled[0] || !bc.u8_mask || !bc.u8_src || P.n_ops < 1) return KC_OK;
+    const uint32_t w = img->w(), h = img->h(), row_units = w / 4;
+    if (bc.u8_src->w != w || bc.u8_src->h != h || bc.u8_src->channels != 4) return KC_OK;
+    bool dense = alpha->kind != kc_plane::MEM || alpha->pitch == (size_t)row_units * 16;
+    uint32_t n_f32 = 0, refs[KC_CHAIN_MAX_IN], at[KC_CHAIN_MAX_IN];
+    for (uint32_t k = 0; k < P.n_in; ++k) {
+        if (bc.u8_mask >> k & 1u) continue;
+        for (int b = 0; b < 3; ++b) dense = dense && P.in_pitch[b][k] == row_units;
+        refs[n_f32] = bc.in_refs[k];
+        at[n_f32++] = k;
+    }
+    P.rows = dense ? 1u : h;
+    P.row_units = dense ? row_units * h : row_units;
+    if ((uint64_t)row_units * h > 0xFFFFFFFFull) return KC_OK;
+    {
+        const uint64_t px = (uint64_t)w * h;
+        const uint32_t m = chain_cache_policy(refs, n_f32, 12 * px, 4 * px);
+        P.nt_mask = 0;
+        for (uint32_t i = 0; i < n_f32; ++i)
+            if (m & KC_CHAIN_NT_BIT(i)) P.nt_mask |= KC_CHAIN_NT_BIT(at[i]);
+    }
+    P.in[3][0] = reinterpret_cast<const float *>(bc.u8_src->base);
+    P.out[3] = reinterpret_cast<float *>(dst);
+    int sink = 1;
+    if (alpha->kind == kc_plane::MEM) {
+        sink = 2;
+        P.in[3][1] = alpha->dptr;
+        P.in_pitch[3][1] = (uint32_t)(alpha->pitch / 16);
+    } else {
+        const uint32_t a = quant_u8_host(alpha->cval);
+        std::memcpy(&P.start_c[3], &a, sizeof a);
+    }
+    hipError_t e = launch_chain_rgba8_specialized(P, bc.u8_mask, sink, c.stream, launched);
+    if (e != hipSuccess) return hip_fail(e, "launch_chain_rgba8");
+    if (!*launched) return KC_OK;
+    *read = bc.u8_src;
+    c.launches++;
+    c.counters["u8chain_launches"]++;
+    c.alg_bytes += (uint64_t)w * h * (4 + 4 + 12ull * n_f32 + (sink == 2 ? 4 : 0));
+    if (c.capture) c.capture->ok = false;
+    return KC_OK;
+}
+
 int plane_materialize(kc_plane *p)
 {
     KC_TRY(need_init());
     std::lock_guard<std::recursive_mutex> lk(ctx().mu);
-    if (p->kind == kc_plane::LAZY || p->kind == kc_plane::RESIZE) return plane_force(p);
+    if (p->kind == kc_plane::LAZY || p->kind == kc_plane::RESIZE || p->kind == kc_plane::U8SRC) return plane_force(p);
     if (p->kind == kc_plane::CONST) {
         kc_plane *m = nullptr;
         KC_TRY(plane_new_mem(p->w, p->h, &m));
diff --git a/kanter_core_amd/csrc/specialize.cpp b/kanter_core_amd/csrc/specialize.cpp
--- a/kanter_core_amd/csrc/specialize.cpp
+++ b/kanter_core_amd/csrc/specialize.cpp
@@ -18,6 +18,10 @@
 extern const char kJitUpsampleChainInc[];
 
 namespace {
+
+#define KC_QUANT_U8_TEXT(...) static const char kQuantU8Text[] = #__VA_ARGS__ "\n";
+#include "quant_u8.inc"
+#undef KC_QUANT_U8_TEXT
 
 typedef struct _hiprtcProgram *hiprtcProgram;
 struct Rtc {
@@ -71,7 +75,9 @@
     bool up_wide = false;
     uint32_t nt_mask = 0;
     uint32_t quads = 1;
+    uint32_t u8_mask = 0, sink = 0, lane_batch = 1;
     uint32_t word[KC_CHAIN_MAX_OPS] = {};
+    bool rgba8() const { return sink != 0; }
 
     std::string key() const
     {
@@ -87,6 +93,12 @@
             k.push_back('q');
             k.push_back((char)('0' + quads));
         }
+        if (u8_mask || sink || lane_batch != 1) {
+            k.push_back('u');
+            k.append((const char *)&u8_mask, sizeof u8_mask);
+            k.push_back((char)('0' + sink));
+            k.push_back((char)('0' + lane_batch));
+        }
         return k;
     }
 };
@@ -147,7 +159,7 @@
     uint32_t h = 2166136261u;
     for (unsigned char c : s.key()) h = (h ^ c) * 16777619u;
     char buf[32];
-    std::snprintf(buf, sizeof buf, s.up_taps ? "kc_upchain_%08x" : "kc_chain_%08x", h);
+    std::snprintf(buf, sizeof buf, s.up_taps ? "kc_upchain_%08x" : s.rgba8() ? "kc_u8chain_%08x" : "kc_chain_%08x", h);
     return buf;
 }
 
@@ -322,9 +334,90 @@
     return src;
 }
 
+static std::string generate_rgba8(const Signature &s)
+{
+    if (s.lane_batch != 3 || s.up_taps || s.quads != 1 || !s.u8_mask || (s.sink != 1 && s.sink != 2)) return std::string();
+    std::string src;
+    src.reserve(32768);
+    src += "namespace kc {\n";
+    src += kJitChainProgramH;
+    src += kPackedF4;
+    src += kQuantU8Text;
+    src += "typedef unsigned int u4 __attribute__((ext_vector_type(4)));\n";
+    src += "}  // namespace kc\nusing namespace kc;\n";
+    char buf[320];
+    std::snprintf(buf, sizeof buf, "extern \"C\" __global__ __launch_bounds__(256) void %s(const ChainProgram P)\n{\n", kernel_name(s).c_str());
+    src += buf;
+    src += "    __shared__ float u8_tab[256];\n"
+           "    const unsigned int n = P.rows * P.row_units;\n"
+           "    const unsigned int idx = blockIdx.x * 256u + threadIdx.x;\n"
+           "    const unsigned int at = idx < n ? idx : n - 1u;\n";
+    if (s.flat)
+        src += "    const unsigned int row = 0u, col = at;\n";
+    else
+        src += "    const unsigned int row = at / P.row_units, col = at - row * P.row_units;\n";
+    src += "    const u4 px = __builtin_nontemporal_load(&reinterpret_cast<const u4 *>(P.in[3][0])[at]);\n";
+    for (uint32_t b = 0; b < 3; ++b)
+        for (uint32_t k = 0; k < s.n_in; ++k) {
+            if (s.u8_mask >> k & 1u) continue;
+            if (s.nt_mask & KC_CHAIN_NT_BIT(k))
+                std::snprintf(buf, sizeof buf, "    const f4 in%u_%u = __builtin_nontemporal_load(&reinterpret_cast<const raw4 *>(P.in[%u][%u])[row * P.in_pitch[%u][%u] + col]);\n", k, b, b, k, b, k);
+            else
+                std::snprintf(buf, sizeof buf, "    const f4 in%u_%u = reinterpret_cast<const raw4 *>(P.in[%u][%u])[row * P.in_pitch[%u][%u] + col];\n", k, b, b, k, b, k);
+            src += buf;
+        }
+    if (s.sink == 2)
+        src += "    const raw4 alpha = reinterpret_cast<const raw4 *>(P.in[3][1])[row * P.in_pitch[3][1] + col];\n";
+    src += "    u8_tab[threadIdx.x] = (float)threadIdx.x / 255.0f;  // 256 threads\n"
+           "    __syncthreads();\n"
+           "    if (idx >= n) return;\n";
+    for (uint32_t b = 0; b < 3; ++b) {
+        std::snprintf(buf, sizeof buf, "    const f4 u8v_%u = f4{ u8_tab[(px.x >> %uu) & 255u], u8_tab[(px.y >> %uu) & 255u], u8_tab[(px.z >> %uu) & 255u], u8_tab[(px.w >> %uu) & 255u] };\n",
+                      b, 8 * b, 8 * b, 8 * b, 8 * b);
+        src += buf;
+        for (uint32_t k = 0; k < s.n_in; ++k)
+            if (s.u8_mask >> k & 1u) {
+                std::snprintf(buf, sizeof buf, "    const f4 in%u_%u = u8v_%u;\n", k, b, b);
+                src += buf;
+            }
+    }
+    for (uint32_t b = 0; b < 3; ++b) {
+        char suffix[8];
+        std::snprintf(suffix, sizeof suffix, "_%u", b);
+        std::snprintf(buf, sizeof buf, "    f4 out%u;\n    {\n        const StepTableView pp{ P.step[%u] };\n", b, b);
+        src += buf;
+        if (s.start_src < 0)
+            std::snprintf(buf, sizeof buf, "        f4 acc = f4{ P.start_c[%u], P.start_c[%u], P.start_c[%u], P.start_c[%u] };\n", b, b, b, b);
+        else
+            std::snprintf(buf, sizeof buf, "        f4 acc = in%d%s;\n", s.start_src, suffix);
+        src += buf;
+        for (uint32_t i = 0; i < s.n_ops; ++i) {
+            const uint32_t code = s.word[i] & 0xffu, from = (s.word[i] >> 8) & 0xffu;
+            if (code == CH_POW_L || code == CH_POW_R || code == CH_SAVE_LOAD || from == (uint32_t)KC_CHAIN_SRC_SAVED) return std::string();
+            const std::string e = step_expr(s, i, "in", suffix);
+            if (e.empty()) return std::string();
+            src += "        acc = " + e + ";\n";
+        }
+        std::snprintf(buf, sizeof buf, "        out%u = acc;\n    }\n", b);
+        src += buf;
+    }
+    if (s.sink == 2)
+        src += "    const unsigned int a0 = quant_u8(alpha.x) << 24, a1 = quant_u8(alpha.y) << 24, a2 = quant_u8(alpha.z) << 24, a3 = quant_u8(alpha.w) << 24;\n";
+    else
+        src += "    const unsigned int a0 = __builtin_bit_cast(unsigned int, P.start_c[3]) << 24, a1 = a0, a2 = a0, a3 = a0;\n";
+    src += "    u4 o;\n"
+           "    o.x = quant_u8(out0.lo.x) | (quant_u8(out1.lo.x) << 8) | (quant_u8(out2.lo.x) << 16) | a0;\n"
+           "    o.y = quant_u8(out0.lo.y) | (quant_u8(out1.lo.y) << 8) | (quant_u8(out2.lo.y) << 16) | a1;\n"
+           "    o.z = quant_u8(out0.hi.x) | (quant_u8(out1.hi.x) << 8) | (quant_u8(out2.hi.x) << 16) | a2;\n"
+           "    o.w = quant_u8(out0.hi.y) | (quant_u8(out1.hi.y) << 8) | (quant_u8(out2.hi.y) << 16) | a3;\n"
+           "    reinterpret_cast<u4 *>(P.out[3])[idx] = o;\n}\n";
+    return src;
+}
+
 std::string generate(const Signature &s)
 {
     if (s.up_taps) return generate_up(s);
+    if (s.rgba8() || s.u8_mask || s.lane_batch != 1) return generate_rgba8(s);
     const int SPEC_WG = spec_wg();
     bool pow = false;
     for (uint32_t i = 0; i < s.n_ops; ++i) pow |= (s.word[i] & 0xffu) == CH_POW_L || (s.word[i] & 0xffu) == CH_POW_R;
@@ -680,7 +773,8 @@
             std::fprintf(f, "{\"name\": \"%s\", \"n_in\": %u, \"start_src\": %d, \"flat\": %d, \"nt_mask\": %u, \"up_taps\": %u, \"up_wide\": %d, \"words\": [",
                          kernel_name(sig).c_str(), sig.n_in, sig.start_src, sig.flat ? 1 : 0, sig.nt_mask, sig.up_taps, sig.up_wide ? 1 : 0);
             for (uint32_t k = 0; k < sig.n_ops; ++k) std::fprintf(f, "%s%u", k ? ", " : "", sig.word[k]);
-            std::fprintf(f, "]}\n");
+            if (sig.rgba8()) std::fprintf(f, "], \"u8_mask\": %u, \"sink\": %u, \"lane_batch\": %u}\n", sig.u8_mask, sig.sink, sig.lane_batch);
+            else std::fprintf(f, "]}\n");
             std::fclose(f);
         }
     }
@@ -749,6 +843,9 @@
     mix(s.up_wide ? 1 : 0);
     mix(s.nt_mask);
     mix(s.quads);
+    mix(s.u8_mask);
+    mix(s.sink);
+    mix(s.lane_batch);
     for (uint32_t i = 0; i < s.n_ops; ++i) mix(s.word[i]);
     return h;
 }
@@ -756,7 +853,7 @@
 static bool same_signature(const Signature &a, const Signature &b)
 {
     return a.n_in == b.n_in && a.n_ops == b.n_ops && a.start_src == b.start_src && a.flat == b.flat && a.up_taps == b.up_taps &&
-           a.up_wide == b.up_wide && a.nt_mask == b.nt_mask && a.quads == b.quads &&
+           a.up_wide == b.up_wide && a.nt_mask == b.nt_mask && a.quads == b.quads && a.u8_mask == b.u8_mask && a.sink == b.sink && a.lane_batch == b.lane_batch &&
            std::memcmp(a.word, b.word, sizeof(uint32_t) * a.n_ops) == 0;
 }
 
@@ -847,6 +944,41 @@
         *launched = true;
         if (nt_mask) *nt_mask = sig.nt_mask;
         if (quads) *quads = sig.quads;
+        std::lock_guard<std::mutex> lk(spec().mu);
+        spec().launches++;
+    }
+    return e;
+}
+
+static Signature signature_rgba8(const ChainProgram &P, uint32_t u8_mask, int sink)
+{
+    Signature sig = signature_of(P);
+    if (!sink && !u8_mask) return sig;
+    sig.nt_mask &= ~0x100u;
+    for (uint32_t k = 0; k < P.n_in; ++k)
+        if (u8_mask >> k & 1u) sig.nt_mask &= ~KC_CHAIN_NT_BIT(k);
+    sig.quads = 1;
+    sig.u8_mask = u8_mask;
+    sig.sink = (uint32_t)sink;
+    sig.lane_batch = 3;
+    return sig;
+}
+
+hipError_t launch_chain_rgba8_specialized(const ChainProgram &P, uint32_t u8_mask, int sink, hipStream_t s, bool *launched)
+{
+    *launched = false;
+    if (P.n_ops < 1 || P.n_ops > (uint32_t)KC_CHAIN_MAX_OPS || P.n_in > (uint32_t)KC_CHAIN_MAX_IN || !u8_mask || (sink != 1 && sink != 2)) return hipSuccess;
+    const uint64_t total = (uint64_t)P.rows * P.row_units;
+    if (total == 0 || total > 0xFFFFFFFFull || !P.in[3][0] || !P.out[3] || (sink == 2 && !P.in[3][1])) return hipSuccess;
+    const Signature sig = signature_rgba8(P, u8_mask, sink);
+    hipFunction_t fn = spec_lookup(sig);
+    if (!fn) return hipSuccess;
+    size_t size = sizeof(ChainProgram);
+    void *extra[] = { HIP_LAUNCH_PARAM_BUFFER_POINTER, (void *)&P, HIP_LAUNCH_PARAM_BUFFER_SIZE, &size, HIP_LAUNCH_PARAM_END };
+    const unsigned gx = (unsigned)((total + 255) / 256);
+    hipError_t e = hipModuleLaunchKernel(fn, gx, 1, 1, 256, 1, 1, 0, s, nullptr, extra);
+    if (e == hipSuccess) {
+        *launched = true;
         std::lock_guard<std::mutex> lk(spec().mu);
         spec().launches++;
     }
@@ -946,6 +1078,23 @@
 
 std::string specialize_source(const ChainProgram &P, const UpsampleArgs *U) { return generate(signature_of(P, U)); }
 
+std::string specialize_source_sig(const ChainProgram &P, uint32_t u8_mask, int sink) { return generate(signature_rgba8(P, u8_mask, sink)); }
+
+int specialize_compile_only_sig(const ChainProgram &P, uint32_t u8_mask, int sink, std::string *log)
+{
+    if (!rtc().ok) {
+        *log = "libhiprtc not available";
+        return KC_ERR_UNSUPPORTED;
+    }
+    const std::string src = generate(signature_rgba8(P, u8_mask, sink));
+    if (src.empty()) {
+        *log = "not a program of that form";
+        return KC_ERR_GENERIC;
+    }
+    std::vector<char> code;
+    return rtc_compile(src, code, log) ? KC_OK : KC_ERR_GENERIC;
+}
+
 int specialize_compile_only(const ChainProgram &P, std::string *log, const UpsampleArgs *U)
 {
     if (!rtc().ok) {
@@ -1006,7 +1155,7 @@
 }
 
 int kernel_cache_precompile(const uint32_t *words, uint32_t n_ops, uint32_t n_in, int32_t start_src, bool flat, uint32_t nt_mask,
-                            uint32_t up_taps, bool up_wide, const char *dir, std::string *log)
+                            uint32_t up_taps, bool up_wide, const char *dir, std::string *log, uint32_t u8_mask, int sink)
 {
     if (!words || n_ops < 1 || n_ops > (uint32_t)KC_CHAIN_MAX_OPS || n_in > (uint32_t)KC_CHAIN_MAX_IN || !dir || !*dir) return KC_ERR_INVALID_ARG;
     Signature sig;
@@ -1019,6 +1168,15 @@
     sig.up_wide = up_wide;
     for (uint32_t i = 0; i < n_ops; ++i) sig.word[i] = words[i];
     sig.quads = chain_quads_for(sig, 0);
+    if (sink || u8_mask) {
+        sig.quads = 1;
+        sig.u8_mask = u8_mask;
+        sig.sink = (uint32_t)sink;
+        sig.lane_batch = 3;
+        sig.nt_mask &= ~0x100u;
+        for (uint32_t k = 0; k < n_in; ++k)
+            if (u8_mask >> k & 1u) sig.nt_mask &= ~KC_CHAIN_NT_BIT(k);
+    }
     const std::string src = generate(sig);
     if (src.empty()) {
         *log = "unknown step code";
diff --git a/kanter_core_amd/csrc/streaming.h b/kanter_core_amd/csrc/streaming.h
--- a/kanter_core_amd/csrc/streaming.h
+++ b/kanter_core_amd/csrc/streaming.h
@@ -19,15 +19,9 @@
     else *p = v;
 }
 
-static __device__ __forceinline__ uint32_t quant_u8(float v)
-{
-    float x = v;
-    if (x < 0.0f) x = 0.0f;
-    if (x > 1.0f) x = 1.0f;
-    x = x * 255.0f;
-    if (!(x <= 255.0f)) x = 255.0f;
-    return (uint32_t)x;
-}
+#define KC_QUANT_U8_TEXT(...) __VA_ARGS__
+#include "quant_u8.inc"
+#undef KC_QUANT_U8_TEXT
 
 #include "srgb_thresholds.inc"
 
diff --git a/kanter_core_amd/csrc/u8pipe.cpp b/kanter_core_amd/csrc/u8pipe.cpp
--- a/kanter_core_amd/csrc/u8pipe.cpp
+++ b/kanter_core_amd/csrc/u8pipe.cpp
@@ -13,15 +13,91 @@
         hipEvent_t packed = nullptr;
         hipEvent_t copied_out = nullptr;
         bool in_used = false, out_used = false;
+        kc::U8Source *src = nullptr;
     };
     std::vector<Slot> slots;
 };
 
 namespace kc {
 
+static std::atomic<int> g_u8_fuse{ 1 };
+int u8_set_fuse(int on)
+{
+    g_u8_fuse.store(on != 0);
+    return KC_OK;
+}
+int u8_get_fuse() { return g_u8_fuse.load(); }
+
+int u8_source_force(U8Source *src)
+{
+    if (!src || u8source_deferred_count(src) == 0) return KC_OK;
+    if (!src->base) {
+        set_error("internal: deferred u8 planes outlived their buffer");
+        return KC_ERR_GENERIC;
+    }
+    Context &c = ctx();
+    kc_plane *pl[4] = { nullptr, nullptr, nullptr, nullptr };
+    float *dp[4] = { nullptr, nullptr, nullptr, nullptr };
+    int st = KC_OK;
+    for (int i = 0; i < src->channels && st == KC_OK; ++i) {
+        st = plane_new_mem(src->w, src->h, &pl[i]);
+        if (st == KC_OK) dp[i] = pl[i]->dptr;
+    }
+    if (st == KC_OK) {
+        const uint64_t in_bytes = (uint64_t)src->w * src->h * src->channels;
+        hipError_t e = launch_from_u8(src->base, src->channels, src->w, src->h, dp, (uint32_t)(pl[0]->pitch / 4),
+                                      cache_policy_mask(in_bytes, in_bytes * 4, 1), c.stream);
+        if (e == hipSuccess && src->read_event) e = hipEventRecord((hipEvent_t)src->read_event, c.stream);
+        if (e != hipSuccess) st = hip_fail(e, "from_u8 of deferred planes");
+        else {
+            c.launches++;
+            c.alg_bytes += in_bytes * 5;
+        }
+    }
+    if (st == KC_OK) {
+        ++src->refs;
+        for (int i = 0; i < src->channels; ++i) {
+            kc_plane *q = static_cast<kc_plane *>(src->deferred[i]);
+            if (!q) continue;
+            q->kind = kc_plane::MEM;
+            q->dptr = pl[i]->dptr;
+            q->pitch = pl[i]->pitch;
+            q->bytes = pl[i]->bytes;
+            q->owned = true;
+            pl[i]->owned = false;
+            pl[i]->dptr = nullptr;
+            q->u8 = nullptr;
+            u8source_detach_plane(src, i, q);
+        }
+        u8source_release(src);
+    }
+    for (int i = 0; i < 4; ++i) plane_release(pl[i]);
+    return st;
+}
+
+int u8_planes_force(kc_plane *const *planes, int n)
+{
+    for (int i = 0; i < n; ++i)
+        if (planes[i] && planes[i]->kind == kc_plane::U8SRC) KC_TRY(u8_source_force(planes[i]->u8));
+    return KC_OK;
+}
+
+static int slot_retire_source(kc_u8_pipe::Slot &s)
+{
+    int st = KC_OK;
+    if (s.src) {
+        st = u8_source_force(s.src);
+        u8source_detach_buffer(s.src);
+        u8source_release(s.src);
+        s.src = nullptr;
+    }
+    return st;
+}
+
 int u8_pipe_free(kc_u8_pipe *p)
 {
     if (!p) return KC_OK;
+    for (auto &s : p->slots) (void)slot_retire_source(s);
     if (p->up) (void)hipStreamSynchronize(p->up);
     if (p->down) (void)hipStreamSynchronize(p->down);
     if (ctx().stream) (void)hipStreamSynchronize(ctx().stream);
@@ -102,6 +178,29 @@
     kc_plane *pl[4] = { nullptr, nullptr, nullptr, nullptr };
     float *dp[4] = { nullptr, nullptr, nullptr, nullptr };
     int st = KC_OK;
+    KC_TRY(slot_retire_source(*s));
+    if (p->channels == 4 && u8_get_fuse()) {
+        hipError_t e = hipSuccess;
+        if (s->in_used) e = hipStreamWaitEvent(p->up, s->converted, 0);
+        if (e == hipSuccess) e = hipMemcpyAsync(s->dev_in, s->host_in, p->in_bytes, hipMemcpyHostToDevice, p->up);
+        if (e == hipSuccess) e = hipEventRecord(s->copied_in, p->up);
+        if (e == hipSuccess) e = hipStreamWaitEvent(c.stream, s->copied_in, 0);
+        if (e != hipSuccess) return hip_fail(e, "kc_u8_pipe_upload");
+        s->in_used = true;
+        s->src = u8source_new(s->dev_in, 4, p->w, p->h, s->converted);
+        for (int i = 0; i < 4; ++i) {
+            pl[i] = new kc_plane();
+            pl[i]->w = p->w;
+            pl[i]->h = p->h;
+            pl[i]->kind = kc_plane::U8SRC;
+            pl[i]->u8 = s->src;
+            pl[i]->u8_ch = i;
+            u8source_attach(s->src, i, pl[i]);
+        }
+        *out = image_new(4, pl);
+        for (int i = 0; i < 4; ++i) plane_release(pl[i]);
+        return KC_OK;
+    }
     for (int i = 0; i < 4 && st == KC_OK; ++i) {
         if (i < p->channels) {
             st = plane_new_mem(p->w, p->h, &pl[i]);
@@ -141,6 +240,25 @@
         return KC_ERR_INVALID_ARG;
     }
     Context &c = ctx();
+    if (u8_get_fuse()) {
+        bool fused = false;
+        U8Source *read = nullptr;
+        hipError_t e = hipSuccess;
+        if (!srgb && s->out_used) e = hipStreamWaitEvent(c.stream, s->copied_out, 0);
+        if (e != hipSuccess) return hip_fail(e, "kc_u8_pipe_download");
+        if (!srgb) KC_TRY(chain_launch_rgba8(img, s->dev_out, &fused, &read));
+        if (fused) {
+            if (read->read_event) e = hipEventRecord((hipEvent_t)read->read_event, c.stream);
+            if (e == hipSuccess) e = hipEventRecord(s->packed, c.stream);
+            if (e == hipSuccess) e = hipStreamWaitEvent(p->down, s->packed, 0);
+            if (e == hipSuccess) e = hipMemcpyAsync(s->host_out, s->dev_out, p->out_bytes, hipMemcpyDeviceToHost, p->down);
+            if (e == hipSuccess) e = hipEventRecord(s->copied_out, p->down);
+            if (e != hipSuccess) return hip_fail(e, "kc_u8_pipe_download");
+            s->out_used = true;
+            return KC_OK;
+        }
+        c.counters["u8chain_fallbacks"]++;
+    }
     KC_TRY(image_force(img));
     Operand o[4];
     for (int i = 0; i < 4; ++i) o[i] = plane_operand(img->planes[img->is_rgba() ? i : 0]);
diff --git a/kanter_core_amd/csrc/u8source.h b/kanter_core_amd/csrc/u8source.h
--- /dev/null
+++ b/kanter_core_amd/csrc/u8source.h
@@ -0,0 +1,60 @@
+#pragma once
+
+namespace kc {
+
+struct U8Source {
+    int refs = 1;
+    const unsigned char *base = nullptr;
+    int channels = 0;
+    unsigned int w = 0, h = 0;
+    void *deferred[4] = { nullptr, nullptr, nullptr, nullptr };
+    void *read_event = nullptr;
+};
+
+inline U8Source *u8source_new(const unsigned char *base, int channels, unsigned int w, unsigned int h, void *read_event)
+{
+    U8Source *s = new U8Source();
+    s->base = base;
+    s->channels = channels;
+    s->w = w;
+    s->h = h;
+    s->read_event = read_event;
+    return s;
+}
+
+inline void u8source_release(U8Source *s)
+{
+    if (s && --s->refs == 0) delete s;
+}
+
+inline bool u8source_attach(U8Source *s, int c, void *plane)
+{
+    if (!s || c < 0 || c >= s->channels || c >= 4 || s->deferred[c]) return false;
+    s->deferred[c] = plane;
+    ++s->refs;
+    return true;
+}
+
+inline void u8source_detach_plane(U8Source *s, int c, void *plane)
+{
+    if (!s || c < 0 || c >= 4 || s->deferred[c] != plane) return;
+    s->deferred[c] = nullptr;
+    u8source_release(s);
+}
+
+inline int u8source_deferred_count(const U8Source *s)
+{
+    int n = 0;
+    if (s)
+        for (int c = 0; c < 4; ++c) n += s->deferred[c] != nullptr;
+    return n;
+}
+
+inline void u8source_detach_buffer(U8Source *s)
+{
+    if (!s) return;
+    s->base = nullptr;
+    s->read_event = nullptr;
+}
+
+}
```
